# dongzhuoyao/self-guided-diffusion-models

Measured on AMD Instinct MI355X. Metric: cfg_sampled_images_per_sec_64x64_1000step_ddpm, higher is better.
Workload: dtype f32 as 3xf16 split MFMA products, f32 accumulate; 1 GPU; IN64 unet_fast ch128 cluster-k5000 cond_scale=2 bs=40/GPU (UNet batch 80), 1000-step native DDPM; batch_per_gpu=40, unet_batch=80, precision_mode=f16x3, launch=hipGraph-captured step

## Files before the change

include/sgdm_hip.h:

```cpp
#ifndef SGDM_HIP_H
#define SGDM_HIP_H
#include <stdint.h>

#ifdef __cplusplus
extern "C" {
#endif

#define SGD_ABI_VERSION 22
int sgd_abi_version(void);
const char* sgd_build_id(void);

enum { SGD_MODE_FLAT = 0, SGD_MODE_CONV3 = 1 };
enum { SGD_RS_NONE = 0, SGD_RS_AVGPOOL2 = 1, SGD_RS_UP2 = 2,
       SGD_RS_ZEROUP2 = 3  };
enum { SGD_PRO_NONE = 0, SGD_PRO_AFFINE_NC = 1, SGD_PRO_LN_ROW = 2 };
enum { SGD_PREC_F32 = 0, SGD_PREC_F16X3 = 1, SGD_PREC_BF16X3 = 2 };

typedef struct sgd_igemm_args {
    const float* x0;
    const float* x1;
    int32_t c0, c1;
    int32_t mode;
    int32_t n, hi, wi;
    int32_t ho, wo;
    int32_t m;
    int32_t rows_per_n;
    int32_t stride;
    int32_t resample;
    int32_t pro;
    int32_t pro_silu;
    const float* pa;
    const float* pb;
    const float* pc;
    const void* w;
    int32_t cin_p, cout_p;
    const float* bias;
    const float* res;
    int32_t res_mode;
    float* y;
    int32_t cout;
    int32_t y_ld;
    int32_t orows_in, orows_out, orow_off;
    int32_t prec;
    float drop_p;
    uint32_t drop_seed;
    float* stats;
    const float* w_scale_inv;
    void* work;
    int64_t work_bytes;
    int32_t grid_cap;
    int32_t tune;
} sgd_igemm_args;
enum {
    SGD_TUNE_BN128 = 1,
    SGD_TUNE_BN256 = 2,
    SGD_TUNE_FLAT2 = 4,
    SGD_TUNE_DEFER = 8,
    SGD_TUNE_PLAIN_SCHEDULE = 16,
    SGD_TUNE_NO_SMALL = 64,
    SGD_TUNE_LN_PACKED = 32,
    SGD_TUNE_WGRAD_GENERIC_NARROW = 256,
    SGD_TUNE_WGRAD_NO_POOLED_PLANES = 512,
    SGD_TUNE_WGRAD_F32 = 1024,
    SGD_TUNE_WGRAD_NO_WS = 2048,
    SGD_TUNE_WGRAD_NO_PLANES = 4096,
    SGD_TUNE_WGRAD_NO_PIPE = 8192,
    SGD_TUNE_WGRAD_PLANES_ALWAYS = 16384
};
int64_t sgd_igemm_work_bytes(void);
int64_t sgd_igemm_work_status_offset(void);
int sgd_igemm_tail_layout(int32_t total_tiles, int32_t nchunks, int32_t taps, int32_t grid, int32_t* out);


int sgd_igemm(const sgd_igemm_args* args , void* stream);
int sgd_igemm_stats_parts(const sgd_igemm_args* args );

int64_t sgd_packed_weight_bytes(int32_t cout, int32_t cin, int32_t ksize, int32_t prec);
int sgd_pack_weight(const float* w_src, void* w_dst, int32_t cout, int32_t cin, int32_t ksize,
                    int32_t prec, int32_t* cin_p, int32_t* cout_p , void* stream);

int sgd_weight_amax(const float* w, int64_t count, uint32_t* amax_bits, void* stream);
int sgd_pack_weight_scaled(const float* w_src, void* w_dst, int32_t cout, int32_t cin, int32_t ksize, int32_t prec,
                           int32_t transpose ,
                           const uint32_t* amax_bits, float* scale_inv_out, int32_t* cin_p, int32_t* cout_p ,
                           void* stream);

typedef struct sgd_pack_job {
    const float* src;
    void* dst;
    uint32_t* amax_bits;
    float* scale_inv;
    int32_t cout, cin, ksize, transpose;
    int32_t own_amax, reserved0;
} sgd_pack_job;
int sgd_pack_job_blocks(int32_t cout, int32_t cin, int32_t ksize, int32_t prec, int32_t transpose, int32_t* amax_blocks,
                        int32_t* pack_blocks, int32_t* cin_p, int32_t* cout_p );
int sgd_pack_weights_batched(const sgd_pack_job* jobs, int32_t n_jobs, const int32_t* amax_block_job, const int32_t* amax_first,
                             int32_t n_amax_blocks, const int32_t* pack_block_job, const int32_t* pack_first,
                             int32_t n_pack_blocks, int32_t prec, void* stream);

int sgd_linear_splitk(const float* x, int32_t x_ld, const float* w, const float* bias, int32_t m, int32_t n, int32_t k,
                      float* work, int32_t ksplit, float* y, int32_t y_ld, void* stream);
int sgd_linear_splitk_t(const float* x, int32_t x_ld, const float* w, int32_t w_ld, int32_t m, int32_t n, int32_t k,
                        float* work, int32_t ksplit, float* y, int32_t y_ld, void* stream);

int sgd_chan_stats(const float* x, int32_t n, int32_t hw, int32_t c,
                   float* sums , int32_t c_total, int32_t c_off, void* stream);
int sgd_add_rows_nc(float* x, const float* e, int32_t e_ld, int32_t n, int64_t hw, int32_t c, void* stream);
int sgd_stats_reduce(const float* partial, int32_t n, int32_t parts, int32_t c,
                     float* sums , int32_t c_total, int32_t c_off, void* stream);
int sgd_gn_coef_parts(const float* partial0, int32_t parts0, int32_t c0, const float* partial1, int32_t parts1, int32_t c1,
                      float* sums, const float* gamma, const float* beta, const float* film, int32_t film_ld,
                      int32_t n, int32_t groups, int32_t hw, float eps, float* a, float* b, void* stream);
int sgd_gn_coef(const float* sums, const float* gamma, const float* beta,
                const float* film , int32_t film_ld,
                int32_t n, int32_t c, int32_t groups, int32_t hw, float eps,
                float* a, float* b, void* stream);

int sgd_ln_stats(const float* x, int32_t rows, int32_t c, float eps, float* stats , void* stream);
int sgd_ln_apply(const float* x, const float* gamma, const float* beta, const float* res,
                 int32_t rows, int32_t c, float eps, float* out, void* stream);

int sgd_attention(const float* q, int32_t q_ld, int32_t q_hs,
                  const float* k, const float* v, int32_t kv_ld, int32_t kv_hs,
                  int32_t batch, int32_t heads, int32_t tq, int32_t tk, int32_t d, float scale,
                  float* out, int32_t out_ld,
                  float* lse ,
                  void* stream);
int sgd_attention_split(const float* q, int32_t q_ld, int32_t q_hs,
                        const float* k, const float* v, int32_t kv_ld, int32_t kv_hs,
                        int32_t batch, int32_t heads, int32_t tq, int32_t tk, int32_t d, float scale,
                        float* out, int32_t out_ld, float* lse, void* stream);

int sgd_timestep_embedding(const int64_t* t, const float* freqs, int32_t n_src, int32_t n, int32_t dim,
                           float* out, void* stream);
int sgd_cond_select(const void* cond, int32_t is_i64, const uint8_t* mask, const float* null_row,
                    int32_t n_src, int32_t n, int32_t k, float* out, void* stream);
int sgd_pack_input(const float* x, const float* layout, const uint8_t* mask, const float* null_layout,
                   int32_t n_src, int32_t n, int32_t cx, int32_t cl, int32_t h, int32_t w,
                   float* out, void* stream);
int sgd_pack_input_compact(const float* x, const void* layout, int32_t layout_fmt, const uint8_t* mask,
                           const float* null_layout, int32_t n_src, int32_t n, int32_t cx, int32_t cl, int32_t h,
                           int32_t w, float* out, void* stream);
int sgd_labelmap_nhot(const uint8_t* labels, int32_t b, int32_t hw, int32_t k, float* out, void* stream);
int sgd_linear_gather(const int64_t* ids, const uint8_t* mask, const float* w, const float* bias, const float* nullproj,
                      int32_t n_src, int32_t n, int32_t nout, int32_t k, float* out, int32_t ldo, void* stream);
int sgd_linear_sparse_rows(const int64_t* cond, const uint8_t* mask, const float* w, const float* bias, const float* nullproj,
                           int32_t n_src, int32_t n, int32_t nout, int32_t k, float* out, int32_t ldo, void* stream);

int sgd_nhwc_to_nchw(const float* x, int32_t n, int32_t h, int32_t w, int32_t c, float* out, void* stream);
int sgd_fill_null_kv(const float* null_kv, int32_t batch, int32_t rows_per_b, int32_t row, int32_t d,
                     float* kv, void* stream);

int sgd_ddpm_step(const float* x, const float* eps_nhwc, const float* z, int32_t cfg_mode, float w,
                  const float* coef , int32_t clip, int32_t b, int32_t c, int32_t hw,
                  float* x_out, float* x0_out, void* stream);
int sgd_ddim_step(const float* x, const float* eps_nhwc, const float* z, int32_t cfg_mode, float w,
                  const float* coef , float temperature,
                  int32_t clip, int32_t b, int32_t c, int32_t hw, float* x_out, float* x0_out, void* stream);
int sgd_ddpm_step_dev(const float* x, const float* eps_nhwc, const float* z, int32_t cfg_mode, float w,
                      const float* coef_dev, int32_t clip, int32_t b, int32_t c, int32_t hw,
                      float* x_out, float* x0_out, void* stream);
int sgd_ddim_step_dev(const float* x, const float* eps_nhwc, const float* z, int32_t cfg_mode, float w,
                      const float* coef_dev, float temperature, int32_t clip, int32_t b, int32_t c, int32_t hw,
                      float* x_out, float* x0_out, void* stream);
#define SGD_PNDM_RK0 0
#define SGD_PNDM_RK12 1
#define SGD_PNDM_RK3 2
#define SGD_PNDM_PLMS 3
typedef struct sgd_pndm_row {
    float d, c1, c2, reserved;
    int32_t phase, slot1, slot2, slot3;
} sgd_pndm_row;
int sgd_pndm_step(const float* x, const float* eps_nhwc, int32_t cfg_mode, float w, const sgd_pndm_row* row_dev,
                  float* acc, float* base, float* ring, int32_t b, int32_t c, int32_t hw, float* x_out, void* stream);
int sgd_x0_quantile(int32_t kind, const float* x, const float* eps_nhwc, int32_t cfg_mode, float w,
                    const float* coef , int32_t b, int32_t c, int32_t hw, int32_t lo, int32_t hi, float frac,
                    float* s_out , void* stream);
int sgd_ddpm_step_dyn(const float* x, const float* eps_nhwc, const float* z, int32_t cfg_mode, float w,
                      const float* coef , const float* dyn_s, int32_t b, int32_t c, int32_t hw,
                      float* x_out, float* x0_out, void* stream);
int sgd_ddim_step_dyn(const float* x, const float* eps_nhwc, const float* z, int32_t cfg_mode, float w,
                      const float* coef , float temperature, const float* dyn_s, int32_t b, int32_t c,
                      int32_t hw, float* x_out, float* x0_out, void* stream);

int sgd_token_pool(const float* cond, int32_t n, int32_t tokens, int32_t c, int32_t cls, float* out, void* stream);

int sgd_geglu(const float* in, int64_t rows, int32_t inner, float* out, void* stream);

int sgd_to_uint8(const float* x, int64_t count, uint8_t* out, void* stream);
int sgd_cfg_combine(const float* eps_nhwc, int32_t cfg_mode, float w, int32_t b, int32_t c, int32_t hw,
                    float* out_nchw, void* stream);


int sgd_pack_weight_dgrad(const float* w_src, void* w_dst, int32_t cout_fwd, int32_t cin_fwd, int32_t ksize,
                          int32_t prec, int32_t* cin_p, int32_t* cout_p , void* stream);

int sgd_wgrad(const sgd_igemm_args* fwd , const float* gy, int32_t gy_ld, int32_t cout,
              float* slabs, int32_t ksplit, float* bias_slabs, void* stream);
int64_t sgd_wgrad_scratch_bytes(const sgd_igemm_args* fwd , int32_t cout);
int sgd_wgrad_bias_rows(const sgd_igemm_args* fwd , int32_t cout, int32_t gy_ld, int32_t ksplit,
                            int64_t scratch_bytes);
int sgd_wgrad_scratch(const sgd_igemm_args* fwd , const float* gy, int32_t gy_ld, int32_t cout,
                      float* slabs, int32_t ksplit, float* bias_slabs, void* scratch, int64_t scratch_bytes, void* stream);
int sgd_colsum_fold(const float* partial, int32_t chunks, int32_t c, float* out, int32_t accumulate, float scale,
                    void* stream);
int sgd_wgrad_reduce(const float* slabs, int32_t ksplit, int32_t taps, int32_t cout, int32_t cin,
                     float* dw, int32_t accumulate, float scale, void* stream);
int sgd_wgrad_reduce_bias(const float* slabs, int32_t ksplit, int32_t taps, int32_t cout, int32_t cin, float* dw,
                          int32_t accumulate, float scale, const float* bias_slabs, int32_t bias_rows, float* dbias,
                          void* stream);
int sgd_colsum_pair(const float* g1, const float* g2, int32_t rows, int32_t c, int32_t ld, float* out1, float* out2,
                    int32_t accumulate, float scale, void* stream);
int sgd_colsum(const float* g, int32_t rows, int32_t c, int32_t ld, float* out, int32_t accumulate, float scale,
               float* work, int32_t work_chunks, void* stream);

int sgd_gn_bwd_reduce(const float* x, int32_t n, int32_t h, int32_t w, int32_t c, int32_t c_total, int32_t c_off,
                      const float* a, const float* b, int32_t silu,
                      const float* gu, int32_t gu_ld, int32_t gu_mode, float drop_p, uint32_t drop_seed,
                      float* S, void* stream);
int sgd_gn_bwd_coef(const float* S, int32_t s_chunks, const float* sums, const float* gamma, const float* beta,
                    const float* film, int32_t film_ld, int32_t n, int32_t c, int32_t groups, int32_t hw, float eps,
                    float* A, float* B, float* Cc, float* dgamma_nc, float* dbeta_nc ,
                    float* dfilm, void* stream);
int sgd_gn_bwd_coef_fold(const float* S, int32_t s_chunks, const float* sums, const float* gamma, const float* beta, const float* film,
                         int32_t film_ld, int32_t n, int32_t c, int32_t groups, int32_t hw, float eps, float* A, float* B,
                         float* Cc, float* dfilm, float* dgamma, float* dbeta, int32_t accumulate, float scale, void* stream);
int sgd_gn_bwd_rows_chunks(int32_t n, int32_t h, int32_t w, int32_t c);
int sgd_gn_bwd_reduce_rows(const float* x, int32_t n, int32_t h, int32_t w, int32_t c, int32_t c_total, int32_t c_off,
                           const float* a, const float* b, int32_t silu, const float* gu, int32_t gu_ld, float drop_p,
                           uint32_t drop_seed, int32_t chunks, float* P, void* stream);
int sgd_gn_bwd_apply(const float* x, int32_t n, int32_t h, int32_t w, int32_t c, int32_t c_total, int32_t c_off,
                     const float* a, const float* b, int32_t silu,
                     const float* gu, int32_t gu_ld, int32_t gu_mode, float drop_p, uint32_t drop_seed,
                     const float* A, const float* B, const float* Cc,
                     const float* gres, int32_t gres_ld, int32_t gres_mode,
                     float* dst, int32_t dst_ld, int32_t dst_off, int32_t accumulate, void* stream);
int sgd_silu_bwd(const float* x, const float* g, int64_t count, float* gx, void* stream);

// ... 67 lines not shown
```

self-guided-diffusion-models_amd/csrc/igemm.hip:

```cpp
#include <type_traits>
#include <utility>

#include "igemm_shared.h"
#include "prologue.h"

namespace {

#ifdef SGDM_PROBE
#define DBG(bit) 0
#define SYNC() do { if (g.stamp) { const unsigned long long t0_ = __builtin_amdgcn_s_memtime(); __syncthreads(); \
                    const unsigned long long t1_ = __builtin_amdgcn_s_memtime(); \
                    if (g.trace && blockIdx.x < 16 && pr_nbar < 512 && (threadIdx.x & 63) == 0) { \
                        unsigned long long* tp_ = g.trace + (((size_t)blockIdx.x * (NTHREADS / 64) + (threadIdx.x >> 6)) * 512 + pr_nbar) * 2; \
                        tp_[0] = t0_; tp_[1] = t1_; } \
                    pr_bar += t1_ - t0_; ++pr_nbar; } else if (!DBG(64)) { __syncthreads(); } } while (0)
#define PROBE_BEGIN() unsigned long long pr_bar = 0, pr_nbar = 0, pr_epi = 0; const unsigned long long pr_t0 = __builtin_amdgcn_s_memtime()
#define PROBE_END(role) do { if (g.stamp && (threadIdx.x & 63) == 0) { \
        unsigned long long* sp_ = g.stamp + ((size_t)blockIdx.x * (NTHREADS / 64) + (threadIdx.x >> 6)) * 4; \
        sp_[0] = __builtin_amdgcn_s_memtime() - pr_t0; sp_[1] = pr_bar; sp_[2] = pr_nbar; sp_[3] = pr_epi; } } while (0)
#define PROBE_EPI(expr) do { if (g.stamp) { const unsigned long long t0_ = __builtin_amdgcn_s_memtime(); expr; pr_epi += __builtin_amdgcn_s_memtime() - t0_; } else { expr; } } while (0)
#else
#define DBG(bit) 0
#define SYNC() __syncthreads()
#define PROBE_BEGIN()
// ... 39 lines not shown

template <int PREC, int NT> struct Frag {
    typedef typename Split<PREC>::T T;
    typedef T T8 __attribute__((ext_vector_type(8)));
    static constexpr int NKS = KC / 16;
    static constexpr int NREADS = 2;
    static constexpr int NWLOADS = 2 * NT;
    static constexpr int NMMA = 3 * NT;
    struct AU {
        T8 h, l;
        __device__ __forceinline__ void load(const float* rowp, int ks, int lh) {
            const int goff = (ks * 2 + lh) * 8;
            h = *reinterpret_cast<const T8*>(rowp + goff);
            l = *reinterpret_cast<const T8*>(rowp + goff + 4);
        }
    };
    struct B {
        T8 h[NT], l[NT];
        __device__ __forceinline__ void load(const char* p, int ks) {
#pragma unroll
            for (int nt = 0; nt < NT; ++nt) {
                h[nt] = *reinterpret_cast<const T8*>(p + nt * WUNIT + ks * 2048);
                l[nt] = *reinterpret_cast<const T8*>(p + nt * WUNIT + ks * 2048 + 1024);
            }
        }
    };
    static __device__ __forceinline__ void mma(f32x16 (&acc)[NT], const AU& a, const B& b) {
#pragma unroll
        for (int nt = 0; nt < NT; ++nt) {
            if constexpr (PREC == SGD_PREC_F16X3) {
                acc[nt] = __builtin_amdgcn_mfma_f32_32x32x16_f16(b.h[nt], a.l, acc[nt], 0, 0, 0);
                acc[nt] = __builtin_amdgcn_mfma_f32_32x32x16_f16(b.l[nt], a.h, acc[nt], 0, 0, 0);
                acc[nt] = __builtin_amdgcn_mfma_f32_32x32x16_f16(b.h[nt], a.h, acc[nt], 0, 0, 0);
            } else {
                acc[nt] = __builtin_amdgcn_mfma_f32_32x32x16_bf16(b.h[nt], a.l, acc[nt], 0, 0, 0);
                acc[nt] = __builtin_amdgcn_mfma_f32_32x32x16_bf16(b.l[nt], a.h, acc[nt], 0, 0, 0);
                acc[nt] = __builtin_amdgcn_mfma_f32_32x32x16_bf16(b.h[nt], a.h, acc[nt], 0, 0, 0);
            }
        }
    }
};
template <int PREC, int NCB> struct Frag16 {
    typedef typename Split<PREC>::T T;
    typedef T T8 __attribute__((ext_vector_type(8)));
    static constexpr int NREADS = 2;
    static constexpr int NWLOADS = 2 * NCB;
    static constexpr int NMMA = 3 * NCB;
    struct AU {
        T8 h, l;
        __device__ __forceinline__ void load(const float* rowp, int kg) {
            h = *reinterpret_cast<const T8*>(rowp + kg * 8);
            l = *reinterpret_cast<const T8*>(rowp + kg * 8 + 4);
        }
    };
    struct B {
        T8 h[NCB], l[NCB];
        __device__ __forceinline__ void load(const char* p) {
#pragma unroll
            for (int cb = 0; cb < NCB; ++cb) {
                h[cb] = *reinterpret_cast<const T8*>(p + (cb >> 1) * WUNIT + (cb & 1) * 256);
                l[cb] = *reinterpret_cast<const T8*>(p + (cb >> 1) * WUNIT + (cb & 1) * 256 + 1024);
            }
        }
    };
    static __device__ __forceinline__ f32x4 mma1(f32x4 acc, const AU& a, const B& b) {
        if constexpr (PREC == SGD_PREC_F16X3) {
            acc = __builtin_amdgcn_mfma_f32_16x16x32_f16(b.h[0], a.l, acc, 0, 0, 0);
            acc = __builtin_amdgcn_mfma_f32_16x16x32_f16(b.l[0], a.h, acc, 0, 0, 0);
            acc = __builtin_amdgcn_mfma_f32_16x16x32_f16(b.h[0], a.h, acc, 0, 0, 0);
        } else {
            acc = __builtin_amdgcn_mfma_f32_16x16x32_bf16(b.h[0], a.l, acc, 0, 0, 0);
            acc = __builtin_amdgcn_mfma_f32_16x16x32_bf16(b.l[0], a.h, acc, 0, 0, 0);
            acc = __builtin_amdgcn_mfma_f32_16x16x32_bf16(b.h[0], a.h, acc, 0, 0, 0);
        }
        return acc;
    }
    static __device__ __forceinline__ void mma(f32x4 (&acc)[NCB], const AU& a, const B& b) {
#pragma unroll
        for (int cb = 0; cb < NCB; ++cb) {
            if constexpr (PREC == SGD_PREC_F16X3) {
                acc[cb] = __builtin_amdgcn_mfma_f32_16x16x32_f16(b.h[cb], a.l, acc[cb], 0, 0, 0);
                acc[cb] = __builtin_amdgcn_mfma_f32_16x16x32_f16(b.l[cb], a.h, acc[cb], 0, 0, 0);
                acc[cb] = __builtin_amdgcn_mfma_f32_16x16x32_f16(b.h[cb], a.h, acc[cb], 0, 0, 0);
            } else {
                acc[cb] = __builtin_amdgcn_mfma_f32_16x16x32_bf16(b.h[cb], a.l, acc[cb], 0, 0, 0);
                acc[cb] = __builtin_amdgcn_mfma_f32_16x16x32_bf16(b.l[cb], a.h, acc[cb], 0, 0, 0);
                acc[cb] = __builtin_amdgcn_mfma_f32_16x16x32_bf16(b.h[cb], a.h, acc[cb], 0, 0, 0);
            }
        }
    }
};
template <int NCB> struct Frag16<SGD_PREC_F32, NCB> {
    static constexpr int NREADS = 1, NWLOADS = 1, NMMA = 1;
    struct AU { __device__ __forceinline__ void load(const float*, int) {} };
    struct B { __device__ __forceinline__ void load(const char*) {} };
    static __device__ __forceinline__ void mma(f32x4 (&)[NCB], const AU&, const B&) {}
    static __device__ __forceinline__ f32x4 mma1(f32x4 acc, const AU&, const B&) { return acc; }
};
template <int NT> struct Frag<SGD_PREC_F32, NT> {
    static constexpr int NKS = KC / 8;
    static constexpr int NREADS = 1;
    static constexpr int NWLOADS = NT;
    static constexpr int NMMA = 4 * NT;
    struct AU {
        f32x4 v;
        __device__ __forceinline__ void load(const float* rowp, int ks, int lh) {
            v = *reinterpret_cast<const f32x4*>(rowp + ks * 8 + lh * 4);
        }
    };
    struct B {
        f32x4 v[NT];
        __device__ __forceinline__ void load(const char* p, int ks) {
#pragma unroll
            for (int nt = 0; nt < NT; ++nt) v[nt] = *reinterpret_cast<const f32x4*>(p + nt * WUNIT + ks * 1024);
        }
    };
    static __device__ __forceinline__ void mma(f32x16 (&acc)[NT], const AU& a, const B& b) {
#pragma unroll
        for (int j = 0; j < 4; ++j)
#pragma unroll
            for (int nt = 0; nt < NT; ++nt)
                acc[nt] = __builtin_amdgcn_mfma_f32_32x32x2f32(b.v[nt][j], a.v[j], acc[nt], 0, 0, 0);
    }
};

template <int CTRL, int ROWMASK> __device__ __forceinline__ float dpp_add(float v) {
    return v + __builtin_bit_cast(float, __builtin_amdgcn_update_dpp(0, __builtin_bit_cast(int, v), CTRL, ROWMASK, 0xF, true));
}
__device__ __forceinline__ float half_wave_sum_hi(float v) {
    v = dpp_add<0xB1, 0xF>(v);
    v = dpp_add<0x4E, 0xF>(v);
    v = dpp_add<0x141, 0xF>(v);
    v = dpp_add<0x140, 0xF>(v);
    return dpp_add<0x142, 0xA>(v);
}

template <class F, int... I> __device__ __forceinline__ void static_for_impl(F&& f, std::integer_sequence<int, I...>) {
    (f(std::integral_constant<int, I>()), ...);
}
template <int N, class F> __device__ __forceinline__ void static_for(F&& f) {
    static_for_impl(f, std::make_integer_sequence<int, N>());
}

__device__ __forceinline__ float row16_sum(float v) {
    v = dpp_add<0xB1, 0xF>(v);
    v = dpp_add<0x4E, 0xF>(v);
    v = dpp_add<0x141, 0xF>(v);
    return dpp_add<0x140, 0xF>(v);
}

struct Tile {
    int n0c;
    int img0, ty0, tx0;
    long m0;
};

__device__ __forceinline__ Tile tile_at(const Geo& g, int lin, int bn, int tw, int th) {
    Tile t;
    const int mtile = lin / g.nt, ntile = lin - mtile * g.nt;
    t.n0c = ntile * bn;
    const int per_img = g.tiles_x * g.tiles_y;
    const int it = mtile / per_img, rem = mtile - it * per_img;
    t.img0 = it * g.nb;
    t.ty0 = (rem / g.tiles_x) * th;
    t.tx0 = (rem % g.tiles_x) * tw;
    t.m0 = (long)mtile * BM;
    return t;
}


template <int BN, int PREC, bool VEC, int TAPS, bool DEFER>
struct IgemmBlock {
    static constexpr bool CONV = TAPS == 9;
    static constexpr int FG = CONV ? 1 : TAPS;
    static constexpr int KCC = KC * FG;
    static constexpr int NA = 3;
    static constexpr int WM = (BN >= 128) ? 128 : 32;
    static constexpr int WN = (BN >= 128) ? BN / 4 : 32;
    static constexpr int MT = WM / 32, NT = WN / 32;
    static constexpr int WAVES_N = BN / WN;
    typedef Frag<PREC, NT> FragT;
    static constexpr bool M16 = PREC != SGD_PREC_F32 && BN <= 128 && !DEFER;
    static constexpr int RB = M16 ? WM / 16 : MT, RBH = M16 ? 16 : 32;
    static constexpr int CBN = M16 ? WN / 16 : NT, CBW = M16 ? 16 : 32;
    static constexpr int QPB = M16 ? 1 : 4;
    typedef Frag16<PREC, CBN> Frag16T;
    typedef std::conditional_t<M16, f32x4, f32x16> AccV;
    static constexpr int NKS = FragT::NKS;

    static constexpr int STG_LD = BN + 4;
    static_assert(!DEFER || (BN == 128 && TAPS == 9 && VEC && !M16), "loader-side epilogue: 3x3, 128-column tiles");

    const sgd_igemm_args& a;
    const Geo& g;
    float* As;
    int2* pixtab;
    float* bias_s;
    float* stg;
    int a_floats;
    bool bias_lds;
    int tid, lane, wave;
    int total, xchunk, nloc, xcd, loc, xbeg, xend, cin, nchunks, xtiles, nfull, xrem, split;
    int ntiles, rem_lin, rem_part, last_c0, last_c1;
    int Q, S, s, TW, TH, M;

    __device__ __forceinline__ int lin_of(int k) const { return (rem_lin >= 0 && k == ntiles - 1) ? rem_lin : xbeg + loc + k * nloc; }
    __device__ __forceinline__ int cbeg(int k) const { return k == ntiles - 1 ? last_c0 : 0; }
    __device__ __forceinline__ int cend(int k) const { return k == ntiles - 1 ? last_c1 : nchunks; }

    __device__ __forceinline__ bool init(float* smem) {
        a_floats = g.pix * LDA;
        As = smem;
        pixtab = reinterpret_cast<int2*>(smem + (size_t)NA * a_floats);
        bias_s = smem + (size_t)NA * a_floats + (size_t)g.pix * 8;
        bias_lds = a.cout_p <= BIAS_LDS_MAX;
        stg = bias_s + a.cout_p;

        tid = threadIdx.x; lane = tid & 63;
        wave = __builtin_amdgcn_readfirstlane(tid >> 6);

        total = g.mt * g.nt;
        xchunk = (total + 7) >> 3;
        nloc = gridDim.x >> 3;
        xcd = blockIdx.x & 7; loc = blockIdx.x >> 3;
        xbeg = xcd * xchunk; xend = (xbeg + xchunk < total) ? xbeg + xchunk : total;
        cin = a.c0 + a.c1;
        nchunks = (cin + KCC - 1) / KCC;
        xtiles = xend > xbeg ? xend - xbeg : 0;
        nfull = xtiles / nloc; xrem = xtiles - nfull * nloc;
        split = (a.work && !ABL(2048)) ? tail_split(xrem, nloc, nchunks, TAPS) : 0;
        rem_lin = -1; rem_part = 0; last_c0 = 0; last_c1 = nchunks;
        if (!split) {
            ntiles = loc < xtiles ? (xtiles - loc + nloc - 1) / nloc : 0;
        } else {
            ntiles = nfull;
            if (loc < xrem * split) {
                rem_lin = xbeg + nfull * nloc + loc / split;
                rem_part = loc % split;
                last_c0 = rem_part * nchunks / split;
                last_c1 = (rem_part + 1) * nchunks / split;
                ++ntiles;
            }
        }
        if (ntiles == 0) return false;

        Q = (ntiles - 1) * nchunks + (last_c1 - last_c0);
        S = Q * TAPS;
        s = CONV ? a.stride : 1;
        TW = 1 << g.tw_l2; TH = 1 << g.th_l2;
        M = CONV ? a.n * a.ho * a.wo : a.m;

        return true;
    }

    __device__ __forceinline__ void build_pixtab(int k, int t0, int nthr) const {
        if (k >= ntiles) return;
        const Tile T = tile_at(g, lin_of(k), BN, TW, TH);
        int2* tab = pixtab + (size_t)(k & 3) * g.pix;
        for (int pix = t0; pix < g.pix; pix += nthr) {
            int2 e;
            e.x = -1;
            e.y = 0;
            if (CONV) {
                int hx = pix % g.hw, t = pix / g.hw;
                int hy = t % g.hh, nb = t / g.hh;
                int n = T.img0 + nb, y = T.ty0 * s - 1 + hy, x = T.tx0 * s - 1 + hx;
                if (n < a.n && y >= 0 && y < g.hc && x >= 0 && x < g.wc) {
                    if (a.resample == SGD_RS_UP2) e.x = (n * a.hi + (y >> 1)) * a.wi + (x >> 1);
                    else if (a.resample == SGD_RS_AVGPOOL2) e.x = (n * a.hi + 2 * y) * a.wi + 2 * x;
                    else if (a.resample == SGD_RS_ZEROUP2) e.x = ((y | x) & 1) ? -1 : (n * a.hi + (y >> 1)) * a.wi + (x >> 1);
                    else e.x = (n * a.hi + y) * a.wi + x;
                    e.y = n;
                }
            } else {
                long row = T.m0 + pix;
                if (row < M) {
                    e.x = (int)row;
                    e.y = (a.pro == SGD_PRO_AFFINE_NC) ? (int)(row / a.rows_per_n) : 0;
                }
            }
            tab[pix] = e;
        }
    }

    static constexpr size_t SLAB = (size_t)RB * CBN * QPB * NCOMP * 16;
    static __device__ __forceinline__ f32x4 accq(const AccV (&acc)[RB][CBN], int mt, int nt, int q) {
        f32x4 v;
#pragma unroll
        for (int j = 0; j < 4; ++j) v[j] = acc[mt][nt][(M16 ? 0 : q * 4) + j];
        return v;
    }
    __device__ __forceinline__ int pixel_of_lane(int ln) const {
    const int l5 = ln & 31;
        int px = l5;
        if (CONV && g.tw_l2 == 4 && s == 1) {
            if (l5 < 4) px = l5;
            else if (l5 < 12) px = l5 + 4;
            else if (l5 < 16) px = l5 - 8;
            else if (l5 < 20) px = l5;
            else if (l5 < 28) px = l5 + 2;
            else px = l5 < 30 ? l5 - 8 : l5;
        }
        if constexpr (M16) {
            const int i16 = ln & 15;
            px = i16 < 4 ? 2 * i16 : (i16 < 12 ? 2 * (i16 - 4) + 1 : 2 * i16 - 16);
        }
        return px;
    }
    template <int RES, bool PART>
    __device__ __forceinline__ void epilogue(const AccV (&acc)[RB][CBN], const Tile& T, int wm, int wn, int lane_e, int cb, float wsk,
                                             const char* part_base, int nparts) const;
    __device__ __forceinline__ void loader_role();
    __device__ __forceinline__ void compute_role();
};

template <int BN, int PREC, bool VEC, int TAPS, bool DEFER>
__device__ __forceinline__ void IgemmBlock<BN, PREC, VEC, TAPS, DEFER>::loader_role() {
    PROBE_BEGIN();
    __builtin_amdgcn_s_setprio(2);
    const int dlt = tid - NCOMP;
    const int dcq = (dlt >> 6) * 8 + (dlt & 7), drg = (dlt & 63) >> 3;
    int dk = 0, dqs = 0, dnck = cend(0) - cbeg(0);
    Tile dT = tile_at(g, lin_of(0), BN, TW, TH);
    int dcol = 0;
    unsigned dsoff = 0xFFFFFFFFu;
    f32x4 dres[8], ds1 = {0.f, 0.f, 0.f, 0.f}, ds2 = ds1;
    unsigned dyoff[8];
    int di0 = 0;
#pragma unroll
    for (int j = 0; j < 8; ++j) { dres[j] = f32x4{0.f, 0.f, 0.f, 0.f}; dyoff[j] = 0xFFFFFFFFu; }
    const float dwsi = (DEFER && a.w_scale_inv) ? *a.w_scale_inv : 1.f;
    const long drows = (long)a.n * a.ho * a.wo;
    const __amdgpu_buffer_rsrc_t dy_rs = __builtin_amdgcn_make_buffer_rsrc(a.y, 0, (int)(drows * a.y_ld * 4), 0x00020000);
    const __amdgpu_buffer_rsrc_t dr_rs = __builtin_amdgcn_make_buffer_rsrc(a.res ? const_cast<float*>(a.res) : a.y, 0,
                                                                           a.res ? (int)(drows * a.cout * 4) : 0, 0x00020000);
    const __amdgpu_buffer_rsrc_t ds_rs = __builtin_amdgcn_make_buffer_rsrc(a.stats ? a.stats : a.y, 0,
                                             a.stats ? (int)((long)a.n * g.sparts * 2 * a.cout * 4) : 0, 0x00020000);
    const int dnq = !DEFER ? 0 : (nchunks - 1 >= 8 && cend(ntiles - 1) - cbeg(ntiles - 1) - 1 >= 8) ? 2
                               : (nchunks - 1 >= 4 && cend(ntiles - 1) - cbeg(ntiles - 1) - 1 >= 4) ? 4 : 8;
    auto with_nq = [&](auto&& f) __attribute__((always_inline)) {
        if (dnq == 2) f(std::integral_constant<int, 2>());
        else if (dnq == 4) f(std::integral_constant<int, 4>());
        else if (dnq == 8) f(std::integral_constant<int, 8>());
        else f(std::integral_constant<int, 0>());
    };
    auto drain = [&](int q, auto nqc) __attribute__((always_inline)) {
        constexpr int NQ = decltype(nqc)::value;
        if constexpr (DEFER && NQ > 0) {
            if (q >= dqs + dnck) {
                dqs += dnck;
                ++dk;
                dnck = cend(dk) - cbeg(dk);
            }
            const int j = q - dqs, nsl = dnck - 1;
            const f32x4 bq = *reinterpret_cast<const f32x4*>(bias_s + (dcol < a.cout_p ? dcol : 0));
#pragma unroll
            for (int jj = 0; jj < NQ; ++jj) {
                const int frow = drg + 8 * (di0 + jj < 16 ? di0 + jj : 15);
                f32x4 v = *reinterpret_cast<const f32x4*>(stg + (size_t)frow * STG_LD + dcq * 4);
                v = v * dwsi + bq + dres[jj];
                __builtin_amdgcn_raw_buffer_store_b128(__builtin_bit_cast(u32x4_t, v), dy_rs, dyoff[jj], 0, 0);
                if (dyoff[jj] != 0xFFFFFFFFu) {
                    ds1 += v;
                    ds2 += v * v;
                }
            }
            const bool last = dk > 0 && j == nsl;
            f32x4 t1 = ds1, t2 = ds2;
            if (last) {
#pragma unroll
                for (int o = 8; o < 64; o <<= 1)
#pragma unroll
                    for (int e = 0; e < 4; ++e) {
                        t1[e] += __shfl_xor(t1[e], o, 64);
                        t2[e] += __shfl_xor(t2[e], o, 64);
                    }
                ds1 = ds2 = f32x4{0.f, 0.f, 0.f, 0.f};
            }
            const unsigned so = (last && drg == 0) ? dsoff : 0xFFFFFFFFu;
            __builtin_amdgcn_raw_buffer_store_b128(__builtin_bit_cast(u32x4_t, t1), ds_rs, so, 0, 0);
            __builtin_amdgcn_raw_buffer_store_b128(__builtin_bit_cast(u32x4_t, t2), ds_rs,
                                                   so == 0xFFFFFFFFu ? so : so + (unsigned)a.cout * 4u, 0, 0);
            const bool req = dk > 0 && j < nsl;
            int i0 = 0, i1 = 0;
            if (req) { i0 = (16 * j) / nsl; i1 = (16 * (j + 1)) / nsl; }
            di0 = i0;
            if (dk > 0 && j == 0) {
                dT = tile_at(g, lin_of(dk - 1), BN, TW, TH);
                const Tile& T = dT;
                dcol = T.n0c + dcq * 4;
                const int part = (T.ty0 >> g.th_l2) * g.tiles_x + (T.tx0 >> g.tw_l2);
                dsoff = (a.stats && dcol < a.cout) ? (unsigned)((((long)T.img0 * g.sparts + part) * 2 * a.cout + dcol) * 4) : 0xFFFFFFFFu;
            }
            const Tile& T = dT;
#pragma unroll
            for (int jj = 0; jj < NQ; ++jj) {
                const int i = i0 + jj;
                const int row = drg + 8 * (i < 16 ? i : 15);
                const int tx = row & (TW - 1), ty = (row >> g.tw_l2) & (TH - 1), nb = row >> (g.tw_l2 + g.th_l2);
                const int n = T.img0 + nb;
                const bool ok = i < i1 && nb < g.nb && n < a.n && dcol < a.cout;
                const int orow = (n * a.ho + T.ty0 + ty) * a.wo + T.tx0 + tx;
                dyoff[jj] = ok ? (unsigned)(((long)orow * a.y_ld + dcol) * 4) : 0xFFFFFFFFu;
                const unsigned ro = ok ? (unsigned)(((long)orow * a.cout + dcol) * 4) : 0xFFFFFFFFu;
                dres[jj] = __builtin_bit_cast(f32x4, __builtin_amdgcn_raw_buffer_load_b128(dr_rs, ro, 0, 0));
            }
        }
        (void)q;
    };
    if constexpr (CONV) {
        const bool uni_rt = VEC && g.nb == 1 && a.pro == SGD_PRO_AFFINE_NC;
        const bool drop_rt = a.drop_p > 0.f;
        const bool lean2 = g.fast_a && VEC && ((uni_rt && a.pro_silu) || (a.pro == SGD_PRO_NONE && !a.pro_silu))
                           && (!drop_rt || (uni_rt && a.pro_silu && a.resample != SGD_RS_AVGPOOL2))
                           && cin % KC == 0 && (a.c1 == 0 || a.c0 % KC == 0) && !DBG(3);
        if (lean2) {
            constexpr int LT = A_THREADS;
            constexpr int AJ = (FAST_PIX * 8 + LT - 1) / LT;
            const int lt = tid - NCOMP;
            const int c4 = lt & 7;
            const int items = g.pix * 8;
            auto go = [&](auto unic, auto poolc, auto dropc) __attribute__((always_inline)) {
                constexpr bool uni = decltype(unic)::value;
                constexpr bool DROP = decltype(dropc)::value;
                constexpr bool LATE = false;
                constexpr int NS = decltype(poolc)::value ? 4 : 1;
                constexpr int T0 = LATE ? 5 : 1;
                typedef std::integral_constant<int, 0> R0;
                typedef std::integral_constant<int, 1> R1;
                typedef std::integral_constant<int, 2> R2;
                int pixj[AJ], rows2[AJ];
                bool live[AJ];
#pragma unroll
                for (int j = 0; j < AJ; ++j) {
                    const int idx = lt + j * LT;
                    live[j] = idx < items;
                    pixj[j] = (live[j] ? idx : items - 1) >> 3;
                }
                unsigned valid1 = 0, valid2 = 0;
                auto load_rows = [&](int k) __attribute__((always_inline)) {
                    const int2* tab = pixtab + (size_t)(k & 3) * g.pix;
                    valid2 = 0;
#pragma unroll
                    for (int j = 0; j < AJ; ++j) {
                        const int ex = tab[pixj[j]].x;
                        rows2[j] = ex < 0 ? 0 : ex;
                        if (ex >= 0) valid2 |= 1u << j;
                    }
                };
                struct S { int k, chunk, img0; const float* src; int stride; const float* ka; const float* kb; };
                auto fill = [&](S& c) __attribute__((always_inline)) {
                    const int ch = c.chunk * KC;
                    if (ch < a.c0) { c.src = a.x0 + ch; c.stride = a.c0; }
                    else { c.src = a.x1 + (ch - a.c0); c.stride = a.c1; }
                    const long ko = (long)c.img0 * cin + ch;
                    c.ka = uni ? a.pa + ko : a.x0;
                    c.kb = uni ? a.pb + ko : a.x0;
                };
                auto advance = [&](S c) __attribute__((always_inline)) {
                    if (++c.chunk == cend(c.k)) {
                        if (c.k + 1 < ntiles) {
                            ++c.k; c.chunk = cbeg(c.k);
                            c.img0 = tile_at(g, lin_of(c.k), BN, TW, TH).img0;
                        }
                        else c.chunk = cend(c.k) - 1;
                    }
                    fill(c);
                    return c;
                };
                f32x4 araw[AJ][NS];
                Coef kq;
                auto transform = [&](f32x4 v, bool ok) __attribute__((always_inline)) {
                    if (ABL(256)) return v;
                    if constexpr (uni) {
                        const float den = ok ? 1.0f : __builtin_inff();
                        v = v * kq.p + kq.q;
#pragma unroll
                        for (int e = 0; e < 4; ++e) v[e] = v[e] * __builtin_amdgcn_rcpf(den + __expf(-v[e]));
                    } else {
                        if (!ok) v = f32x4{0.f, 0.f, 0.f, 0.f};
                    }
                    return v;
                };
                auto issue_item = [&](const S& c, int j) __attribute__((always_inline)) {
                    const float* p0 = c.src + (long)rows2[j] * c.stride + c4 * 4;
                    if (ABL(512)) { KEEP_LIVE(p0); return; }
                    araw[j][0] = ld4(p0);
                    if constexpr (NS == 4) {
                        araw[j][1] = ld4(p0 + c.stride);
                        araw[j][2] = ld4(p0 + (long)a.wi * c.stride);
                        araw[j][3] = ld4(p0 + (long)(a.wi + 1) * c.stride);
                    }
                };
                auto issue_coef = [&](const S& c) __attribute__((always_inline)) {
                    if constexpr (uni) { kq.p = ld4(c.ka + c4 * 4); kq.q = ld4(c.kb + c4 * 4); }
                };
                S s2;
                auto finish = [&](int slot, int j) __attribute__((always_inline)) {
                    const bool ok = (valid1 >> j) & 1u;
                    f32x4 v = transform(araw[j][0], ok);
                    if constexpr (NS == 4)
                        v = 0.25f * (v + transform(araw[j][1], ok) + transform(araw[j][2], ok) + transform(araw[j][3], ok));
                    if constexpr (DROP)
                        v = sgd_drop4(v, a.drop_p, a.drop_seed, (long)rows2[j] * cin + s2.chunk * KC + c4 * 4);
                    if (!ABL(1024)) lds_store_act<PREC>(As + (size_t)(slot % NA) * a_floats + (size_t)pixj[j] * LDA, c4, v);
                    else KEEP_LIVE(v);
                };
                auto stage = [&](int slot) __attribute__((always_inline)) {
                    valid1 = valid2;
                    auto finish_all = [&]() {
#pragma unroll
                        for (int j = 0; j < AJ; ++j) finish(slot, j);
                    };
                    PROBE_EPI(finish_all());
                    const int kprev = s2.k;
                    s2 = advance(s2);
                    if (s2.k != kprev) load_rows(s2.k);
                    issue_coef(s2);
#pragma unroll
                    for (int j = 0; j < AJ; ++j) issue_item(s2, j);
                };
                s2.k = 0; s2.chunk = cbeg(0); s2.img0 = tile_at(g, lin_of(0), BN, TW, TH).img0; fill(s2);
                load_rows(0);
                issue_coef(s2);
#pragma unroll
                for (int j = 0; j < AJ; ++j) issue_item(s2, j);
                stage(0);
                stage(1);
                SYNC();
                auto periods = [&](auto nqc) __attribute__((always_inline)) {
                    for (int q = 0; q < Q; ++q) {
                        drain(q, nqc);
                        stage((q + 2) % NA);
                        if (q + 4 < Q && (q + 4) % nchunks == 0) build_pixtab((q + 4) / nchunks, lt, LT);
                        SYNC();
                    }
                };
                if constexpr (NS == 4) periods(std::integral_constant<int, 0>());
                else with_nq(periods);
            };
            if (uni_rt) {
                if (a.resample == SGD_RS_AVGPOOL2) go(std::true_type(), std::true_type(), std::false_type());
                else if (drop_rt) go(std::true_type(), std::false_type(), std::true_type());
                else go(std::true_type(), std::false_type(), std::false_type());
            } else {
                if (a.resample == SGD_RS_AVGPOOL2) go(std::false_type(), std::true_type(), std::false_type());
                else go(std::false_type(), std::false_type(), std::false_type());
            }
            PROBE_END(1);
            return;
        }
    } else {
        const bool tile_uni_rt = a.pro == SGD_PRO_AFFINE_NC && a.rows_per_n % BM == 0;
        const bool ln_rt = a.pro == SGD_PRO_LN_ROW;
        const bool leanf = VEC && (a.pro == SGD_PRO_NONE || tile_uni_rt || ln_rt) && a.drop_p == 0.f && cin % KC == 0
                           && (a.c1 == 0 || a.c0 % KC == 0) && !DBG(3);
        auto flat_loader = [&](auto modec, auto siluc) {
            constexpr int MODE = decltype(modec)::value;
            constexpr bool SILU = decltype(siluc)::value;
            constexpr bool tile_uni = MODE == 1, ln = MODE == 2;
            constexpr int AI = BM * 8 / A_THREADS;
            constexpr int AROWS = A_THREADS / 8;
            const int lt = tid - NCOMP;
            const int c4 = lt & 7;
            const int arow = lt >> 3;
            typedef std::integral_constant<int, 0> R0;
            typedef std::integral_constant<int, 1> R1;
            typedef std::integral_constant<int, 2> R2;
            f32x4 araw[NB_RING][AI];
            Coef kq[NB_RING];
            float2 rst[NB_RING][AI];
            struct Cur { int k, chunk; int m0; const float* ka; const float* kb; };
            auto open_tile = [&](Cur& c) {
                const Tile T = tile_at(g, lin_of(c.k), BN, TW, TH);
                c.m0 = (int)T.m0;
                const long ko = tile_uni ? (long)(c.m0 / a.rows_per_n) * cin : 0;
                c.ka = tile_uni ? a.pa + ko + c4 * 4 : (ln ? a.pb + c4 * 4 : a.x0);
                c.kb = tile_uni ? a.pb + ko + c4 * 4 : ((ln && a.pc) ? a.pc + c4 * 4 : a.x0);
            };
            auto advance = [&](Cur& c) {
                if (++c.chunk == cend(c.k) * FG) {
                    if (c.k + 1 < ntiles) { ++c.k; c.chunk = cbeg(c.k) * FG; open_tile(c); }
                    else c.chunk = cend(c.k) * FG - 1;
                }
            };
            Cur ci, cf;
            ci.k = 0; ci.chunk = cbeg(0) * FG; open_tile(ci);
            cf = ci;
            auto issue = [&](auto rc) {
                constexpr int R = decltype(rc)::value;
                const int ch = ci.chunk * KC;
                const float* src;
                int stride;
                if (ch < a.c0) { src = a.x0 + ch; stride = a.c0; }
                else { src = a.x1 + (ch - a.c0); stride = a.c1; }
                if constexpr (MODE != 0) {
                    kq[R].p = ld4(ci.ka + ch);
                    kq[R].q = ld4(ci.kb + ((tile_uni || a.pc) ? ch : 0));
                }
#pragma unroll
                for (int j = 0; j < AI; ++j) {
                    int row = ci.m0 + arow + j * AROWS;
                    row = row < M ? row : M - 1;
                    araw[R][j] = ld4(src + (long)row * stride + c4 * 4);
                    if constexpr (ln) rst[R][j] = *reinterpret_cast<const float2*>(a.pa + (long)row * 2);
                }
                advance(ci);
            };
            auto finish = [&](int slot, auto rc, int sub = 0) {
                constexpr int R = decltype(rc)::value;
#pragma unroll
                for (int j = 0; j < AI; ++j) {
                    f32x4 v = araw[R][j];
                    if constexpr (tile_uni) v = v * kq[R].p + kq[R].q;
                    if constexpr (ln) {
                        v = (v - rst[R][j].x) * rst[R][j].y * kq[R].p;
                        if (a.pc) v += kq[R].q;
                    }
                    if constexpr (SILU) {
#pragma unroll
                        for (int e = 0; e < 4; ++e) v[e] = sgd_silu(v[e]);
                    }
                    if (cf.m0 + arow + j * AROWS >= M) v = f32x4{0.f, 0.f, 0.f, 0.f};
                    lds_store_act<PREC>(As + (size_t)slot * a_floats + (size_t)(sub * BM + arow + j * AROWS) * LDA, c4, v);
                }
                advance(cf);
            };
            if constexpr (FG == 1) {
                issue(R0());
                issue(R1());
                finish(0, R0());
                finish(1, R1());
                issue(R2());
                issue(R0());
                issue(R1());
                SYNC();
                auto body = [&](int slot, auto rc) {
                    finish(slot, rc);
                    issue(rc);
                    SYNC();
                };
                int step = 0;
                for (; step + 3 <= S; step += 3) {
                    body(2, R2());
                    body(0, R0());
                    body(1, R1());
                }
                if (step < S) {
                    body(2, R2());
                    if (step + 1 < S) body(0, R0());
                }
            } else {
                static_assert(FG <= 2, "two planes per chunk");
                issue(R0());
                issue(R1());
                issue(R2());
                finish(0, R0(), 0); issue(R0());
                finish(0, R1(), 1); issue(R1());
                finish(1, R2(), 0); issue(R2());
                finish(1, R0(), 1); issue(R0());
                SYNC();
                auto period = [&](int slot, auto ra, auto rb) {
                    finish(slot, ra, 0); issue(ra);
                    finish(slot, rb, 1); issue(rb);
                    SYNC();
                };
                int q = 0;
                for (; q + 3 <= Q; q += 3) {
                    period(2, R1(), R2());
                    period(0, R0(), R1());
                    period(1, R2(), R0());
                }
                if (q < Q) {
                    period(2, R1(), R2());
                    if (q + 1 < Q) period(0, R0(), R1());
                }
            }
        };
        if (FG > 1 && !leanf) __builtin_trap();
        if (leanf) {
            typedef std::integral_constant<int, 0> M0;
            typedef std::integral_constant<int, 1> M1;
            typedef std::integral_constant<int, 2> M2;
            if (tile_uni_rt) { if (a.pro_silu) flat_loader(M1(), std::true_type()); else flat_loader(M1(), std::false_type()); }
            else if (ln_rt) { if (a.pro_silu) flat_loader(M2(), std::true_type()); else flat_loader(M2(), std::false_type()); }
            else { if (a.pro_silu) flat_loader(M0(), std::true_type()); else flat_loader(M0(), std::false_type()); }
            PROBE_END(1);
            return;
        }
    }
    const int lt = tid - NCOMP;
    const int c4 = lt & 7;
    const int items = g.pix * 8;
    struct TabRef { const int2* tab; long m0; };
    auto tabref = [&](int k) {
        TabRef t;
        t.tab = pixtab + (size_t)(k & 3) * g.pix;
        t.m0 = CONV ? 0 : tile_at(g, lin_of(k), BN, TW, TH).m0;
        return t;
    };
    auto entry = [&](const TabRef& t, int pix) -> int2 {
        if (CONV) return t.tab[pix];
        int2 e;
        const long row = t.m0 + pix;
        e.x = row < M ? (int)row : -1;
        e.y = (a.pro == SGD_PRO_AFFINE_NC) ? (int)(row / a.rows_per_n) : 0;
        return e;
    };
    auto item_sync = [&](float* abuf, const TabRef& tab, int idx, int kc0) {
        const int pix = idx >> 3;
        const int c = kc0 + c4 * 4;
        const int2 e = entry(tab, pix);
        f32x4 v = {0.f, 0.f, 0.f, 0.f};
        if (e.x >= 0 && c < cin) {
            if (CONV && a.resample == SGD_RS_AVGPOOL2) {
#pragma unroll
                for (int dy = 0; dy < 2; ++dy)
#pragma unroll
                    for (int dx = 0; dx < 2; ++dx) {
                        long r = (long)e.x + dy * a.wi + dx;
                        v += apply_pro(a, load_raw<VEC>(a, r, c), load_coef<VEC>(a, e.y, r, c), c, r);
                    }
                v = v * 0.25f;
            } else {
                v = apply_pro(a, load_raw<VEC>(a, e.x, c), load_coef<VEC>(a, e.y, e.x, c), c, e.x);
            }
        }
        lds_store_act<PREC>(abuf + (size_t)pix * LDA, c4, v);
    };
    auto stage_A_sync = [&](int slot, int q) __attribute__((always_inline)) {
        q = q < Q ? q : Q - 1;
        const int k = q / nchunks, chunk = q - k * nchunks + cbeg(k);
        float* abuf = As + (size_t)(slot % NA) * a_floats;
        const TabRef tab = tabref(k);
        for (int idx = lt; idx < items; idx += A_THREADS) item_sync(abuf, tab, idx, chunk * KC);
    };
    auto finish_item = [&](int slot, const TabRef& tab, int chunk, int idx, f32x4 raw, bool kuse, const Coef& kuni) __attribute__((always_inline)) {
        float* abuf = As + (size_t)(slot % NA) * a_floats;
        const int c = chunk * KC + c4 * 4;
        if (idx < items) {
            const int pix = idx >> 3;
            const int2 e = entry(tab, pix);
            f32x4 v = {0.f, 0.f, 0.f, 0.f};
            if (c < cin && e.x >= 0) v = apply_pro(a, raw, kuse ? kuni : load_coef<VEC>(a, e.y, e.x, c), c, e.x);
            lds_store_act<PREC>(abuf + (size_t)pix * LDA, c4, v);
        }
    };
    auto raw_item = [&](const TabRef& tab, int idx, int c) -> f32x4 {
        const int ii = idx < items ? idx : items - 1;
        const int2 e = entry(tab, ii >> 3);
        return load_raw<VEC>(a, e.x >= 0 ? e.x : 0, c < cin ? c : 0);
    };

    if (CONV) {
        constexpr int AJ = (FAST_PIX * 8 + A_THREADS - 1) / A_THREADS;
        stage_A_sync(0, 0);
        if (DBG(1)) {
            for (int q = 0; q <= Q; ++q) SYNC();
        } else if (g.fast_a && a.resample != SGD_RS_AVGPOOL2) {
            const bool uni = VEC && g.nb == 1 && a.pro == SGD_PRO_AFFINE_NC;
            const bool kshared = uni || a.pro == SGD_PRO_NONE;
            f32x4 araw[AJ];
            Coef kq;
            struct Ctx { const int2* tab; int c; int chunk; long ko; };
            auto ctx_of = [&](int q) {
                q = q < Q ? q : Q - 1;
                Ctx cx;
                const int k = q / nchunks;
                cx.chunk = q - k * nchunks + cbeg(k);
                cx.tab = pixtab + (size_t)(k & 3) * g.pix;
                cx.c = cx.chunk * KC + c4 * 4;
                cx.ko = (long)tile_at(g, lin_of(k), BN, TW, TH).img0 * cin + (cx.c < cin ? cx.c : 0);
                return cx;
            };
            Ctx cx = ctx_of(1);
            auto request = [&]() __attribute__((always_inline)) {
                TabRef tr;
                tr.tab = cx.tab;
                tr.m0 = 0;
                kq.p = ld4(uni ? a.pa + cx.ko : a.x0);
                kq.q = ld4(uni ? a.pb + cx.ko : a.x0);
#pragma unroll
                for (int j = 0; j < AJ; ++j) araw[j] = raw_item(tr, lt + j * A_THREADS, cx.c);
            };
            auto stage = [&](int slot, int qnext) __attribute__((always_inline)) {
                TabRef tr;
                tr.tab = cx.tab;
                tr.m0 = 0;
#pragma unroll
                for (int j = 0; j < AJ; ++j)
                    finish_item(slot, tr, cx.chunk, lt + j * A_THREADS, araw[j], kshared, kq);
                cx = ctx_of(qnext);
                request();
            };
            request();
            stage(1, 2);
            SYNC();
            with_nq([&](auto nqc) __attribute__((always_inline)) {
                for (int q = 0; q < Q; ++q) {
                    drain(q, nqc);
                    stage(q + 2, q + 3);
                    if (q + 4 < Q && (q + 4) % nchunks == 0) build_pixtab((q + 4) / nchunks, lt, A_THREADS);
                    SYNC();
                }
            });
        } else {
            stage_A_sync(1, 1);
            SYNC();
            with_nq([&](auto nqc) __attribute__((always_inline)) {
                for (int q = 0; q < Q; ++q) {
                    drain(q, nqc);
                    stage_A_sync(q + 2, q + 2);
                    if (q + 4 < Q && (q + 4) % nchunks == 0) build_pixtab((q + 4) / nchunks, lt, A_THREADS);
                    SYNC();
                }
            });
        }
        PROBE_END(1);
        return;
    } else {
        constexpr int AJ = (BM * 8 + A_THREADS - 1) / A_THREADS;
        f32x4 araw[NB_RING][AJ];
        stage_A_sync(0, 0);
        if (Q > 1) stage_A_sync(1, 1);
        auto issue = [&](int q, auto rc) {
            constexpr int R = decltype(rc)::value;
            q = q < Q ? q : Q - 1;
            const int k = q / nchunks, chunk = q - k * nchunks + cbeg(k);
            const TabRef tab = tabref(k);
            const int c = chunk * KC + c4 * 4;
#pragma unroll
            for (int j = 0; j < AJ; ++j) araw[R][j] = raw_item(tab, lt + j * A_THREADS, c);
        };
        auto finish = [&](int slot, auto rc) {
            constexpr int R = decltype(rc)::value;
            const int q = slot < Q ? slot : Q - 1;
            const int k = q / nchunks, chunk = q - k * nchunks + cbeg(k);
            const TabRef tab = tabref(k);
            Coef knone;
            knone.p = f32x4{0.f, 0.f, 0.f, 0.f};
            knone.q = knone.p;
#pragma unroll
            for (int j = 0; j < AJ; ++j)
                finish_item(slot, tab, chunk, lt + j * A_THREADS, araw[R][j], a.pro == SGD_PRO_NONE, knone);
        };
        typedef std::integral_constant<int, 0> R0;
        typedef std::integral_constant<int, 1> R1;
        typedef std::integral_constant<int, 2> R2;
        issue(2, R2());
        issue(3, R0());
        issue(4, R1());
        SYNC();
        auto body = [&](int step, auto rc) {
            finish(step + 2, rc);
            issue(step + 5, rc);
            SYNC();
        };
        int step = 0;
        for (; step + 3 <= S; step += 3) {
            body(step, R2());
            body(step + 1, R0());
            body(step + 2, R1());
        }
        if (step < S) {
            body(step, R2());
            if (step + 1 < S) body(step + 1, R0());
        }
        PROBE_END(1);
        return;
    }
}

template <int BN, int PREC, bool VEC, int TAPS, bool DEFER>
template <int RES, bool PART>
__device__ __forceinline__ void IgemmBlock<BN, PREC, VEC, TAPS, DEFER>::epilogue(const AccV (&acc)[RB][CBN], const Tile& T, int wm, int wn,
                                                                                 int lane_e, int cb, float wsk, const char* part_base,
                                                                                 int nparts) const {
    const int li = lane & 31;
    bool okm[RB];
    int orw[RB], rrw[RB];
    const int plie = pixel_of_lane(lane_e);
#pragma unroll
    for (int mt = 0; mt < RB; ++mt) {
        const int row = wm * WM + mt * RBH + plie;
        int orow, n = 0, oy = 0, ox = 0;
        if (CONV) {
            const int tx = row & (TW - 1), ty = (row >> g.tw_l2) & (TH - 1), nb = row >> (g.tw_l2 + g.th_l2);
            n = T.img0 + nb; oy = T.ty0 + ty; ox = T.tx0 + tx;
            okm[mt] = nb < g.nb && n < a.n;
            orow = (n * a.ho + oy) * a.wo + ox;
        } else {
            orow = (int)T.m0 + row;
            okm[mt] = orow < M;
        }
        if (!okm[mt]) orow = 0;
        int rrow = orow;
        if (RES == 2) rrow = (n * a.ho * 2 + 2 * oy) * (a.wo * 2) + 2 * ox;
        if (RES == 3) rrow = (n * (a.ho >> 1) + (oy >> 1)) * (a.wo >> 1) + (ox >> 1);
        if (!okm[mt]) rrow = 0;
        if (!CONV && a.orows_in > 0)
            orow = (int)((unsigned)orow / (unsigned)a.orows_in) * a.orows_out + a.orow_off
                   + (int)((unsigned)orow % (unsigned)a.orows_in);
        orw[mt] = orow;
        rrw[mt] = rrow;
    }
    const bool vec = ((a.cout | a.y_ld) & 3) == 0;
    if (vec) {
        float* sp = nullptr;
        if (a.stats) {
            int n_img, part;
            if (CONV) {
                n_img = T.img0;
                part = ((T.ty0 >> g.th_l2) * g.tiles_x + (T.tx0 >> g.tw_l2)) * (BM / WM) + wm;
            } else {
                n_img = (int)(T.m0 / a.rows_per_n);
                part = (int)((T.m0 % a.rows_per_n) / BM) * (BM / WM) + wm;
            }
            sp = a.stats + ((long)n_img * g.sparts + part) * 2 * a.cout;
        }
        {
            constexpr int CS = CBN * QPB;
            constexpr int QB = M16 ? ((RES == 2 || PART) ? 1 : (CBN > 2 ? 2 : CBN)) : ((RES == 2 || NT > 1) ? 1 : 2);
            constexpr int RBB = M16 ? (RES == 2 || RB < 4 ? 2 : ((PART || CBN > 2) ? 4 : RB)) : RB;
            static_assert(RB % RBB == 0 && CS % QB == 0, "batches must tile the wave's rows and columns");
#pragma unroll
            for (int q0 = 0; q0 < CS; q0 += QB) {
            f32x4 s1[QB], s2[QB];
#pragma unroll
            for (int i = 0; i < QB; ++i) s1[i] = s2[i] = f32x4{0.f, 0.f, 0.f, 0.f};
#pragma unroll
            for (int mb0 = 0; mb0 < RB; mb0 += RBB) {
#pragma unroll
            for (int mt = mb0; mt < mb0 + RBB; ++mt) asm volatile("" : "+v"(orw[mt]), "+v"(rrw[mt]));
            f32x4 rv[QB][RBB];
            f32x4 pv[QB][RBB];
            if constexpr (PART) {
#pragma unroll
                for (int cs = q0; cs < q0 + QB; ++cs)
#pragma unroll
                    for (int mt = mb0; mt < mb0 + RBB; ++mt) {
                        const char* pp = part_base + (size_t)((mt * CS + cs) * NCOMP) * 16;
                        f32x4 sum = *reinterpret_cast<const f32x4*>(pp);
                        for (int pi = 1; pi < nparts; ++pi) sum += *reinterpret_cast<const f32x4*>(pp + pi * SLAB);
                        pv[cs - q0][mt - mb0] = sum;
                    }
            }
#pragma unroll
            for (int cs = q0; cs < q0 + QB; ++cs) {
                const int c = cb + (cs / QPB) * CBW + (cs % QPB) * 8;
                const int cl = c < a.cout ? c : 0;
                f32x4 bv = {0.f, 0.f, 0.f, 0.f};
                if (bias_lds) bv = *reinterpret_cast<const f32x4*>(bias_s + cl);
                else if (a.bias && !ABL(2)) bv = ld4(a.bias + cl);
#pragma unroll
                for (int mt = mb0; mt < mb0 + RBB; ++mt) {
                    f32x4& r = rv[cs - q0][mt - mb0];
                    r = bv;
                    if ((RES == 1 || RES == 3) && !ABL(2)) r += ld4(a.res + (long)rrw[mt] * a.cout + cl);
                    if (RES == 2 && !ABL(2)) {
                        const long rw = (long)a.wo * 2 * a.cout;
                        const float* rp = a.res + (long)rrw[mt] * a.cout;
                        r += 0.25f * (ld4(rp + cl) + ld4(rp + a.cout + cl) + ld4(rp + rw + cl) + ld4(rp + rw + a.cout + cl));
                    }
                }
            }
#pragma unroll
            for (int cs = q0; cs < q0 + QB; ++cs) {
                const int c = cb + (cs / QPB) * CBW + (cs % QPB) * 8;
                if (c >= a.cout) continue;
#pragma unroll
                for (int mt = mb0; mt < mb0 + RBB; ++mt) {
                    f32x4 v = accq(acc, mt, cs / QPB, cs % QPB);
                    if constexpr (PART) v += pv[cs - q0][mt - mb0];
                    v = v * wsk + rv[cs - q0][mt - mb0];
                    if (okm[mt]) {
                        if (!(DBG(8)) && !ABL(1)) *reinterpret_cast<f32x4*>(a.y + (long)orw[mt] * a.y_ld + c) = v;
                        else KEEP_LIVE(v);
                        s1[cs - q0] += v;
                        s2[cs - q0] += v * v;
                    }
                }
            }
            }
            if (sp && !DBG(256) && !ABL(4)) {
#pragma unroll
                for (int cs = q0; cs < q0 + QB; ++cs) {
                    const int c = cb + (cs / QPB) * CBW + (cs % QPB) * 8;
                    if (c >= a.cout) continue;
                    f32x4 t1 = s1[cs - q0], t2 = s2[cs - q0];
#pragma unroll
                    for (int j = 0; j < 4; ++j) {
                        t1[j] = M16 ? row16_sum(t1[j]) : half_wave_sum_hi(t1[j]);
                        t2[j] = M16 ? row16_sum(t2[j]) : half_wave_sum_hi(t2[j]);
                    }
                    if (M16 ? (lane & 15) == 0 : li == 16) {
                        *reinterpret_cast<f32x4*>(sp + c) = t1;
                        *reinterpret_cast<f32x4*>(sp + a.cout + c) = t2;
                    }
                }
            }
            }
        }
    } else {
#pragma unroll
        for (int mt = 0; mt < RB; ++mt) {
            if (!okm[mt]) continue;
            float* yp = a.y + (long)orw[mt] * a.y_ld;
            const float* rp = RES ? a.res + (long)rrw[mt] * a.cout : nullptr;
#pragma unroll
            for (int nt = 0; nt < CBN; ++nt)
#pragma unroll
                for (int gq = 0; gq < QPB; ++gq)
#pragma unroll
                    for (int j = 0; j < 4; ++j) {
                        const int c = cb + nt * CBW + gq * 8 + j;
                        if (c >= a.cout) continue;
                        float x = acc[mt][nt][(M16 ? 0 : gq * 4) + j];
                        if constexpr (PART) {
                            const float* pp = reinterpret_cast<const float*>(part_base + (size_t)(((mt * CBN + nt) * QPB + gq) * NCOMP) * 16) + j;
                            for (int pi = 0; pi < nparts; ++pi) x += pp[pi * (SLAB / 4)];
                        }
                        x = x * wsk + (bias_lds ? bias_s[c] : (a.bias ? a.bias[c] : 0.f));
                        if (RES == 1 || RES == 3) x += rp[c];
                        if (RES == 2) {
                            const long rw = (long)a.wo * 2 * a.cout;
                            x += 0.25f * (rp[c] + rp[a.cout + c] + rp[rw + c] + rp[rw + a.cout + c]);
                        }
                        yp[c] = x;
                    }
        }
    }
}

template <int BN, int PREC, bool VEC, int TAPS, bool DEFER>
__device__ __forceinline__ void IgemmBlock<BN, PREC, VEC, TAPS, DEFER>::compute_role() {
    PROBE_BEGIN();
    const int li = lane & 31, lh = lane >> 5;
    const int wm = wave / WAVES_N, wn = wave % WAVES_N;

    const int pli = pixel_of_lane(lane);
    int aoff[RB];
#pragma unroll
    for (int mt = 0; mt < RB; ++mt) {
        int r = wm * WM + mt * RBH + pli;
        int p;
        if (CONV) {
            int tx = r & (TW - 1), ty = (r >> g.tw_l2) & (TH - 1), nb = r >> (g.tw_l2 + g.th_l2);
            p = (nb * g.hh + ty * s) * g.hw + tx * s;
        } else {
            p = r;
        }
        aoff[mt] = p * LDA;
    }
    const size_t wstep = (size_t)(a.cout_p >> 5) * WUNIT;
    auto wtile_of = [&](int k) __attribute__((always_inline)) {
        int l;
        asm volatile("v_mbcnt_lo_u32_b32 %0, -1, 0\n\tv_mbcnt_hi_u32_b32 %0, -1, %0" : "=v"(l));
        const int loff = M16 ? (l >> 5) * 2048 + (((l >> 4) & 1) * 32 + (l & 15)) * 16 : l * 16;
        return reinterpret_cast<const char*>(a.w) + (size_t)(wn * NT + (tile_at(g, lin_of(k), BN, TW, TH).n0c >> 5)) * WUNIT + loff;
    };

    AccV acc[RB][CBN];
    const float wsi = __builtin_bit_cast(float, __builtin_amdgcn_readfirstlane(
        __builtin_bit_cast(int, a.w_scale_inv ? *a.w_scale_inv : 1.f)));

    constexpr int STAGES = M16 ? RB * CBN : NKS * MT;
    constexpr int RING = M16 ? RB : (STAGES >= 4 ? 4 : 2);
    constexpr int DEPTH = RING - 1;
    static_assert(STAGES % RING == 0, "ring position must be a compile-time constant inside a K step");
    std::conditional_t<M16, typename Frag16<PREC, 1>::AU, typename FragT::AU> ring[RING];
    typename FragT::B fb[NKS];
    typename Frag16<PREC, 1>::B fb16[CBN];
    const int rowstep = g.hw * LDA;

    auto tap_off = [&](int tap) { return CONV ? (tap / 3) * rowstep + (tap % 3) * LDA : tap * (BM * LDA); };
    auto do_step = [&](const float* acur, const float* anext, auto tapc, auto parc, const char* wnext) {
        constexpr int tap = decltype(tapc)::value;
        constexpr int PAR = decltype(parc)::value;
        constexpr bool seam = tap + 1 == TAPS;
        static_for<STAGES>([&](auto stc) {
            constexpr int st = decltype(stc)::value;
            constexpr int ks = M16 ? 0 : st / MT, mt = M16 ? st % RB : st % MT;
            constexpr int pst = (st + DEPTH) % STAGES;
            constexpr bool wrap = st + DEPTH >= STAGES;
            const float* pbase = (wrap && seam) ? anext : acur;
            constexpr int ptap = wrap ? (seam ? 0 : tap + 1) : tap;
            if constexpr (M16) {
                constexpr int cbi = st / RB;
                const float* nbase = seam ? anext : acur;
                constexpr int ntap = seam ? 0 : tap + 1;
                if (!ABL(16)) acc[mt][cbi] = Frag16<PREC, 1>::mma1(acc[mt][cbi], ring[mt], fb16[cbi]);
                if (cbi == CBN - 1 && !ABL(64)) ring[mt].load(nbase + tap_off(ntap) + aoff[mt], lane >> 4);
                if (mt == RB - 1 && !ABL(32)) fb16[cbi].load(wnext + (cbi >> 1) * WUNIT + (cbi & 1) * 256);
                (void)pbase; (void)ptap; (void)pst; (void)wrap;
            } else {
                if (!ABL(64)) ring[(st + DEPTH) % RING].load(pbase + tap_off(ptap) + aoff[pst % MT], pst / MT, lh);
                if (!ABL(16)) FragT::mma(acc[mt], ring[st % RING], fb[ks]);
                if (mt == MT - 1 && !ABL(32)) fb[ks].load(wnext, ks);
            }
            {
                constexpr int NM = M16 ? 3 : FragT::NMMA;
                constexpr int NR = M16 ? (st / RB == CBN - 1 ? 2 : 0) : FragT::NREADS;
                constexpr int P1 = NR < NM ? NR : NM;
                constexpr int nw = M16 ? (st % RB == RB - 1 ? 2 : 0) : ((mt == MT - 1) ? FragT::NWLOADS : 0);
                constexpr int P2 = nw < NM - P1 ? nw : NM - P1;
#pragma unroll
                for (int i = 0; i < P1; ++i) {
                    __builtin_amdgcn_sched_group_barrier(0x008, 1, 0);
                    __builtin_amdgcn_sched_group_barrier(0x100, 1, 0);
                }
#pragma unroll
                for (int i = 0; i < P2; ++i) {
                    __builtin_amdgcn_sched_group_barrier(0x008, 1, 0);
                    __builtin_amdgcn_sched_group_barrier(0x020, 1, 0);
                }
                if constexpr (NM - P1 - P2 > 0) __builtin_amdgcn_sched_group_barrier(0x008, NM - P1 - P2, 0);
            }
            __builtin_amdgcn_sched_barrier(0);
        });
        if constexpr (seam) SYNC();
    };

    auto wstart_of = [&](int k) { return wtile_of(k) + (size_t)cbeg(k) * TAPS * wstep; };
    const char* wp = wstart_of(0);
    if constexpr (M16) {
#pragma unroll
        for (int cb = 0; cb < CBN; ++cb) fb16[cb].load(wp + (cb >> 1) * WUNIT + (cb & 1) * 256);
    } else {
#pragma unroll
        for (int ks = 0; ks < NKS; ++ks) fb[ks].load(wp, ks);
    }
    SYNC();
#pragma unroll
    for (int st = 0; st < (M16 ? RB : DEPTH); ++st) {
        if constexpr (M16) ring[st].load(As + aoff[st % RB], lane >> 4);
        else ring[st].load(As + aoff[st % MT], st / MT, lh);
    }
    int aslot = 0;
    for (int k = 0; k < ntiles; ++k) {
#pragma unroll
        for (int i = 0; i < RB; ++i)
#pragma unroll
            for (int j = 0; j < CBN; ++j)
#pragma unroll
                for (int r = 0; r < (M16 ? 4 : 16); ++r) acc[i][j][r] = 0.f;
        const char* const wseam = k + 1 < ntiles ? wstart_of(k + 1) : nullptr;
        const int c_end = cend(k);
        for (int chunk = cbeg(k); chunk < c_end; ++chunk) {
            const int naslot = aslot + 1 == NA ? 0 : aslot + 1;
            const float* acur = As + (size_t)aslot * a_floats;
            const float* anext = As + (size_t)naslot * a_floats;
            const char* const wlast = chunk + 1 == c_end ? (wseam ? wseam : wp + (TAPS - 1) * wstep) : nullptr;
            static_for<TAPS>([&](auto tapc) {
                constexpr int tap = decltype(tapc)::value;
                const char* wnext = wp + wstep;
                if (tap + 1 == TAPS && wlast) wnext = wlast;
                do_step(acur, anext, tapc, std::integral_constant<int, tap & 1>(), wnext);
                wp = wnext;
            });
            aslot = naslot;
        }
        if constexpr (DEFER) {
            if (k + 1 < ntiles) {
                int plie = pli;
                asm volatile("" : "+v"(plie));
#pragma unroll
                for (int mt = 0; mt < RB; ++mt) {
                    float* sp = stg + (size_t)(wm * WM + mt * RBH + plie) * STG_LD + wn * WN + 4 * lh;
#pragma unroll
                    for (int q = 0; q < QPB; ++q) {
                        f32x4 v;
#pragma unroll
                        for (int j = 0; j < 4; ++j) v[j] = acc[mt][0][q * 4 + j];
                        *reinterpret_cast<f32x4*>(sp + q * 8) = v;
                    }
                }
                continue;
            }
        }

        const char* part_base = nullptr;
        int nparts = 0;
        float wsk = wsi;
        int* part_cnt = nullptr;
        if (rem_lin >= 0 && k == ntiles - 1) {
            const int gi = tail_counter(xcd, loc, nloc, split);
            int* const cnt = reinterpret_cast<int*>(a.work) + gi * 2;
            char* const slab0 = reinterpret_cast<char*>(a.work) + WORK_HEAD + (size_t)tail_slab(xcd, loc, nloc, split) * SLAB;
            if (rem_part + 1 < split) {
                __amdgpu_buffer_rsrc_t rs = __builtin_amdgcn_make_buffer_rsrc(slab0 + (size_t)rem_part * SLAB, 0, (int)SLAB, 0x00020000);
#pragma unroll
                for (int mt = 0; mt < RB; ++mt)
#pragma unroll
                    for (int nt = 0; nt < CBN; ++nt)
#pragma unroll
                        for (int q = 0; q < QPB; ++q)
                            __builtin_amdgcn_raw_buffer_store_b128(__builtin_bit_cast(u32x4_t, accq(acc, mt, nt, q)), rs,
                                                                   (((mt * CBN + nt) * QPB + q) * NCOMP + tid) * 16, 0, 16 );
                asm volatile("s_waitcnt vmcnt(0)" ::: "memory");
                if (lane == 0) __hip_atomic_fetch_add(cnt, 1, __ATOMIC_RELAXED, __HIP_MEMORY_SCOPE_AGENT);
                break;
            }
            int late = 0;
            if (lane == 0) {
                const int need = (split - 1) * (NCOMP / 64);
                int polls = 0;
                while (__hip_atomic_load(cnt, __ATOMIC_RELAXED, __HIP_MEMORY_SCOPE_AGENT) < need) {
                    __builtin_amdgcn_s_sleep(16);
                    if (++polls >= FINISH_POLL_MAX) { late = 1; break; }
                }
                int* const status = reinterpret_cast<int*>(a.work) + WORK_STATUS_INT;
                if (late) __hip_atomic_store(status, 1, __ATOMIC_RELAXED, __HIP_MEMORY_SCOPE_AGENT);
                else if (__hip_atomic_load(status, __ATOMIC_RELAXED, __HIP_MEMORY_SCOPE_AGENT) != 0) late = 2;
            }
            if (__builtin_amdgcn_readfirstlane(late)) wsk = __builtin_nanf("");
            __builtin_amdgcn_fence(__ATOMIC_ACQUIRE, "agent");
            asm volatile("s_waitcnt vmcnt(0)" ::: "memory");
            {
                int lane_p;
                asm volatile("v_mbcnt_lo_u32_b32 %0, -1, 0\n\tv_mbcnt_hi_u32_b32 %0, -1, %0" : "=v"(lane_p));
                part_base = slab0 + (size_t)(wave * 64 + lane_p) * 16;
            }
            nparts = split - 1;
            part_cnt = cnt;
        }

        const Tile T = tile_at(g, lin_of(k), BN, TW, TH);
        int lane_e;
        asm volatile("v_mbcnt_lo_u32_b32 %0, -1, 0\n\tv_mbcnt_hi_u32_b32 %0, -1, %0" : "=v"(lane_e));
        const int cb = T.n0c + wn * WN + 4 * (M16 ? lane_e >> 4 : lane_e >> 5);
        auto keep_acc = [&]() {
#pragma unroll
            for (int i = 0; i < RB; ++i)
#pragma unroll
                for (int j = 0; j < CBN; ++j) KEEP_LIVE(acc[i][j]);
        };
        auto run_epilogue = [&](auto partc) {
            constexpr bool PARTV = decltype(partc)::value;
            if (DBG(16) || ABL(8)) keep_acc();
            else if (!a.res) epilogue<0, PARTV>(acc, T, wm, wn, lane_e, cb, wsk, part_base, nparts);
            else if (a.res_mode == SGD_RS_NONE) epilogue<1, PARTV>(acc, T, wm, wn, lane_e, cb, wsk, part_base, nparts);
            else if (NT > 1) __builtin_trap();
            else if (a.res_mode == SGD_RS_AVGPOOL2) epilogue<2, PARTV>(acc, T, wm, wn, lane_e, cb, wsk, part_base, nparts);
            else epilogue<3, PARTV>(acc, T, wm, wn, lane_e, cb, wsk, part_base, nparts);
        };
        if (nparts) {
            run_epilogue(std::true_type());
            if (lane == 0) {
                if (__hip_atomic_fetch_add(part_cnt + 1, 1, __ATOMIC_RELAXED, __HIP_MEMORY_SCOPE_AGENT) == NCOMP / 64 - 1) {
                    __hip_atomic_store(part_cnt, 0, __ATOMIC_RELAXED, __HIP_MEMORY_SCOPE_AGENT);
                    __hip_atomic_store(part_cnt + 1, 0, __ATOMIC_RELAXED, __HIP_MEMORY_SCOPE_AGENT);
                }
            }
        } else {
            PROBE_EPI(run_epilogue(std::false_type()));
        }
        if constexpr (NT > 1 || M16) {
            if (k + 1 < ntiles) {
                const float* a0 = As + (size_t)aslot * a_floats;
                if constexpr (M16) {
#pragma unroll
                    for (int st = 0; st < RB; ++st) ring[st].load(a0 + aoff[st % RB], lane >> 4);
                } else {
#pragma unroll
                    for (int ks = 0; ks < NKS; ++ks) fb[ks].load(wp, ks);
#pragma unroll
                    for (int st = 0; st < DEPTH; ++st) ring[st].load(a0 + aoff[st % MT], st / MT, lh);
                }
            }
        }
    }
    PROBE_END(0);
}

template <int BN, int PREC, bool VEC, int TAPS, bool DEFER = false>
__global__ __launch_bounds__(NTHREADS) void igemm_kernel(const KArgs ka) {
    extern __shared__ __attribute__((aligned(16))) float smem[];
    IgemmBlock<BN, PREC, VEC, TAPS, DEFER> blk{ka.a, ka.g};
    if (!blk.init(smem)) return;
    blk.build_pixtab(0, blk.tid, NTHREADS);
    blk.build_pixtab(1, blk.tid, NTHREADS);
    blk.build_pixtab(2, blk.tid, NTHREADS);
    blk.build_pixtab(3, blk.tid, NTHREADS);
    if (blk.bias_lds)
        for (int i = blk.tid; i < ka.a.cout_p; i += NTHREADS) blk.bias_s[i] = (ka.a.bias && i < ka.a.cout && !ABL(2)) ? ka.a.bias[i] : 0.f;
    __syncthreads();
    if (blk.tid >= NCOMP) blk.loader_role();
    else blk.compute_role();
}

template <int BN, int PREC, bool VEC, int TAPS, bool DEFER = false>
int launch1(const KArgs& ka, size_t smem, hipStream_t st) {
    static bool attr = false;
    if (!attr) {
        (void)hipFuncSetAttribute((const void*)igemm_kernel<BN, PREC, VEC, TAPS, DEFER>,
                                  hipFuncAttributeMaxDynamicSharedMemorySize, 160 * 1024);
        attr = true;
    }
    const int total = ka.g.mt * ka.g.nt;
    int full = device_cus();
    if (ka.a.grid_cap > 0 && ka.a.grid_cap < full) full = ka.a.grid_cap >= 8 ? (ka.a.grid_cap & ~7) : 8;
    int grid = ((total + 7) / 8) * 8;
    if (grid > full) grid = full;
    if (ka.a.work && total >= 8) grid = full;
    hipLaunchKernelGGL((igemm_kernel<BN, PREC, VEC, TAPS, DEFER>), dim3(grid), dim3(NTHREADS), smem, st, ka);
    const int rc = sgd_check_launch();
    if (rc != SGD_OK && ka.a.work) (void)hipMemsetAsync(ka.a.work, 0, WORK_HEAD, st);
    return rc;
}

template <int BN, int PREC>
int launch(const KArgs& ka, int vec, int taps, size_t smem, hipStream_t st) {
    const bool conv = taps == 9;
#ifdef SGDM_IGEMM_NOPK
    if (conv) return SGD_ERR_ARG;
    if constexpr (BN == 256) {
        return taps == 2 ? launch1<BN, PREC, true, 2>(ka, smem, st) : launch1<BN, PREC, true, 1>(ka, smem, st);
    } else {
        if constexpr (BN == 128) {
            if (taps == 2) return launch1<BN, PREC, true, 2>(ka, smem, st);
        }
        return vec ? launch1<BN, PREC, true, 1>(ka, smem, st) : launch1<BN, PREC, false, 1>(ka, smem, st);
    }
#else
    if constexpr (BN == 256) {
        if (conv) return launch1<BN, PREC, true, 9>(ka, smem, st);
        return taps == 2 ? launch1<BN, PREC, true, 2>(ka, smem, st) : launch1<BN, PREC, true, 1>(ka, smem, st);
    } else {
        if constexpr (BN == 128 && PREC != SGD_PREC_F32) {
            if (conv && vec == 2) return launch1<BN, PREC, true, 9, true>(ka, smem, st);
        }
        if (conv) return vec ? launch1<BN, PREC, true, 9>(ka, smem, st) : launch1<BN, PREC, false, 9>(ka, smem, st);
        if constexpr (BN == 128) {
            if (taps == 2) return launch1<BN, PREC, true, 2>(ka, smem, st);
        }
        return vec ? launch1<BN, PREC, true, 1>(ka, smem, st) : launch1<BN, PREC, false, 1>(ka, smem, st);
    }
#endif
}

}

#ifndef SGDM_IGEMM_PREC
#error "igemm.hip is compiled once per arithmetic mode: -DSGDM_IGEMM_PREC=0|1|2 (build.py); geometry and entry points: igemm_host.hip"
#endif
#ifdef SGDM_DEV_ONE
#define SGD_DISPATCH_BODY(P)                                                                                        \
    const KArgs& ka = *reinterpret_cast<const KArgs*>(kap); (void)bn; (void)vec; (void)taps;                         \
    return launch1<SGDM_DEV_BN, P, true, SGDM_DEV_ONE, SGDM_DEV_DEFER>(ka, smem, st);
#else
#define SGD_DISPATCH_BODY(P)                                                                                        \
    const KArgs& ka = *reinterpret_cast<const KArgs*>(kap);                                                         \
    return bn == 256 ? launch<256, P>(ka, 1, taps, smem, st)                                                         \
                     : (bn == 128 ? launch<128, P>(ka, vec, taps, smem, st) : launch<32, P>(ka, vec, taps, smem, st));
#endif
#if SGDM_IGEMM_PREC == 0
int sgd_igemm_dispatch_f32(const void* kap, int bn, int vec, int taps, size_t smem, hipStream_t st) { SGD_DISPATCH_BODY(SGD_PREC_F32) }
#elif SGDM_IGEMM_PREC == 1 && defined(SGDM_IGEMM_NOPK)
int sgd_igemm_dispatch_f16x3_nopk(const void* kap, int bn, int vec, int taps, size_t smem, hipStream_t st) { SGD_DISPATCH_BODY(SGD_PREC_F16X3) }
#elif SGDM_IGEMM_PREC == 1
int sgd_igemm_dispatch_f16x3(const void* kap, int bn, int vec, int taps, size_t smem, hipStream_t st) { SGD_DISPATCH_BODY(SGD_PREC_F16X3) }
#elif defined(SGDM_IGEMM_NOPK)
int sgd_igemm_dispatch_bf16x3_nopk(const void* kap, int bn, int vec, int taps, size_t smem, hipStream_t st) { SGD_DISPATCH_BODY(SGD_PREC_BF16X3) }
#else
int sgd_igemm_dispatch_bf16x3(const void* kap, int bn, int vec, int taps, size_t smem, hipStream_t st) { SGD_DISPATCH_BODY(SGD_PREC_BF16X3) }
#endif
```

self-guided-diffusion-models_amd/csrc/igemm_host.hip:

```cpp
#include <stdint.h>

#include "igemm_shared.h"

extern "C" int sgd_abi_version(void) { return SGD_ABI_VERSION; }

static inline int pick_bn(int cout) { return (cout % 128 == 0) ? 128 : 32; }

static inline int column_tile(const sgd_igemm_args& a) {
    const int bn = pick_bn(a.cout);
    if (bn != 128 || (a.tune & (SGD_TUNE_NO_SMALL | SGD_TUNE_BN128 | SGD_TUNE_BN256))) return bn;
    const long rows = a.mode == SGD_MODE_CONV3 ? (long)a.n * a.ho * a.wo : (long)a.m;
    const long t128 = ((rows + BM - 1) / BM) * ((a.cout + 127) / 128);
    return t128 * 4 <= device_cus() ? 32 : 128;
}

static int make_geo(const sgd_igemm_args& a, Geo& g, int bn, int& na, int fg = 1) {
    if (a.c0 <= 0 || a.c1 < 0 || a.cout <= 0 || a.y_ld < a.cout) return SGD_ERR_ARG;
    if (a.mode == SGD_MODE_CONV3) {
        if (a.n <= 0 || a.hi <= 0 || a.wi <= 0 || (a.stride != 1 && a.stride != 2)) return SGD_ERR_ARG;
        if (a.stride == 2 && a.resample != SGD_RS_NONE) return SGD_ERR_ARG;
        const bool up = a.resample == SGD_RS_UP2 || a.resample == SGD_RS_ZEROUP2;
        g.hc = a.resample == SGD_RS_AVGPOOL2 ? a.hi / 2 : (up ? a.hi * 2 : a.hi);
        g.wc = a.resample == SGD_RS_AVGPOOL2 ? a.wi / 2 : (up ? a.wi * 2 : a.wi);
        if (a.resample == SGD_RS_AVGPOOL2 && ((a.hi | a.wi) & 1)) return SGD_ERR_ARG;
        const int ho = a.stride == 2 ? (g.hc + 1) / 2 : g.hc, wo = a.stride == 2 ? (g.wc + 1) / 2 : g.wc;
        if (a.ho != ho || a.wo != wo) return SGD_ERR_ARG;
        if (!is_pow2(a.ho) || !is_pow2(a.wo) || a.ho < 2 || a.wo < 2) return SGD_ERR_ARG;
        if (a.res && a.res_mode == SGD_RS_UP2 && ((a.ho | a.wo) & 1)) return SGD_ERR_ARG;
        if ((long)a.n * a.hi * a.wi >= (1L << 31)) return SGD_ERR_ARG;
        int tw = a.wo < 16 ? a.wo : 16;
        int th = BM / tw; if (th > a.ho) th = a.ho;
        while (th * tw > BM) th >>= 1;
        if (a.stride == 2) { if (tw > 8) tw = 8; if (th > 8) th = 8; }
        int nb = BM / (th * tw);
        g.hh = a.stride == 2 ? 2 * th + 1 : th + 2;
        g.hw = a.stride == 2 ? 2 * tw + 1 : tw + 2;
        while (nb > 1 && 3 * (size_t)nb * g.hh * g.hw * LDA * 4 + (size_t)nb * g.hh * g.hw * 32 > 150 * 1024)
            nb >>= 1;
        g.tw_l2 = ilog2(tw); g.th_l2 = ilog2(th); g.nb = nb;
        g.tiles_x = a.wo / tw; g.tiles_y = a.ho / th;
        g.pix = nb * g.hh * g.hw;
        g.mt = ((a.n + nb - 1) / nb) * g.tiles_x * g.tiles_y;
        g.fast_a = g.pix <= FAST_PIX ? 1 : 0;
        na = 3;
    } else if (a.mode == SGD_MODE_FLAT) {
        if (a.m <= 0) return SGD_ERR_ARG;
        if (a.pro == SGD_PRO_AFFINE_NC && a.rows_per_n <= 0) return SGD_ERR_ARG;
        if (a.res && a.res_mode != SGD_RS_NONE) return SGD_ERR_ARG;
        g.tw_l2 = g.th_l2 = 0; g.nb = 1; g.tiles_x = g.tiles_y = 1; g.hh = g.hw = 1; g.hc = g.wc = 1;
        g.pix = BM * fg;
        g.mt = (a.m + BM - 1) / BM;
        g.fast_a = 1;
        na = 3;
    } else {
        return SGD_ERR_ARG;
    }
    g.sparts = 0;
    const int ppt = bn >= 128 ? 1 : 4;
    if (((a.cout | a.y_ld) & 3) == 0 && a.orows_in == 0) {
        if (a.mode == SGD_MODE_CONV3) {
            if (g.nb == 1 && (1 << (g.tw_l2 + g.th_l2)) == BM) g.sparts = g.tiles_x * g.tiles_y * ppt;
        } else if (a.rows_per_n > 0 && a.rows_per_n % BM == 0 && a.m % a.rows_per_n == 0) {
            g.sparts = a.rows_per_n / BM * ppt;
        }
    }
    return SGD_OK;
}

static bool want_bn256(const sgd_igemm_args& a) {
    if (a.tune & SGD_TUNE_BN128) return false;
    if (a.tune & SGD_TUNE_BN256) return true;
    const long rows = a.mode == SGD_MODE_CONV3 ? (long)a.n * a.ho * a.wo : (long)a.m;
    const long mt = (rows + BM - 1) / BM;
    const long t256 = mt * (a.cout_p / 256), t128 = mt * (a.cout_p / 128);
    if (a.mode == SGD_MODE_CONV3 && a.prec != SGD_PREC_F32) return t128 <= 256 && a.ho * a.wo <= 64 && a.c0 + a.c1 >= 512;
    if (t256 <= 256 && t128 > 256) return true;
    const long r256 = (t256 + 255) / 256, r128 = (t128 + 255) / 256;
    return r256 * 2.0 < r128 * 1.07;
}

extern "C" int sgd_igemm_tail_layout(int32_t total_tiles, int32_t nchunks, int32_t taps, int32_t grid, int32_t* out) {
    if (!out || grid < 8 || (grid & 7) || total_tiles < 0) return SGD_ERR_ARG;
    const int xchunk = (total_tiles + 7) >> 3, nloc = grid >> 3;
    for (int b = 0; b < grid; ++b) {
        const int xcd = b & 7, loc = b >> 3;
        const int xbeg = xcd * xchunk, xend = (xbeg + xchunk < total_tiles) ? xbeg + xchunk : total_tiles;
        const int xtiles = xend > xbeg ? xend - xbeg : 0;
        const int nfull = xtiles / nloc, xrem = xtiles - nfull * nloc;
        const int split = tail_split(xrem, nloc, nchunks, taps);
        int32_t* o = out + 4 * b;
        o[0] = o[1] = o[2] = o[3] = 0;
        if (split && loc < xrem * split) {
            o[0] = split;
            o[1] = tail_counter(xcd, loc, nloc, split);
            o[2] = tail_slab(xcd, loc, nloc, split);
            o[3] = split - 1;
        }
    }
    return SGD_OK;
}

extern "C" int64_t sgd_igemm_work_bytes(void) {
    return (int64_t)WORK_HEAD + 192 * (int64_t)(BM * 256 * 4);
}

extern "C" int64_t sgd_igemm_work_status_offset(void) { return (int64_t)WORK_STATUS_INT * 4; }

extern "C" int sgd_igemm_stats_parts(const sgd_igemm_args* args) {
    if (!args) return 0;
    Geo g;
    int na;
    if (make_geo(*args, g, column_tile(*args), na) != SGD_OK) return 0;
    return g.sparts;
}

extern "C" int sgd_igemm(const sgd_igemm_args* args, void* stream) {
    SGD_CLEAR_ERR();
    if (!args) return SGD_ERR_ARG;
    KArgs ka;
    ka.a = *args;
    sgd_igemm_args& a = ka.a;
    Geo& g = ka.g;
    if (!a.x0 || !a.w || !a.y || a.c0 <= 0 || a.c1 < 0 || a.cout <= 0) return SGD_ERR_ARG;
    if (a.c1 > 0 && (!a.x1 || a.c0 % KC != 0)) return SGD_ERR_ARG;
    if (a.y_ld < a.cout) return SGD_ERR_ARG;
    if (a.pro != SGD_PRO_NONE && (!a.pa || !a.pb)) return SGD_ERR_ARG;
    const int cin = a.c0 + a.c1;
    int bn = column_tile(a);
    if (a.cout_p % pick_bn(a.cout) != 0 || a.cout_p < a.cout || a.cin_p % KC != 0 || a.cin_p < cin) return SGD_ERR_ARG;
    const bool vec = (a.c0 % 4 == 0) && (a.c1 % 4 == 0);
    if (bn == 128 && a.cout_p % 256 == 0 && vec && (!a.res || a.res_mode == SGD_RS_NONE) && want_bn256(a)) bn = 256;
    int na;
    const bool conv = a.mode == SGD_MODE_CONV3;
    int taps = conv ? 9 : 1;
    const bool ln_nopk = !conv && a.pro == SGD_PRO_LN_ROW && a.prec != SGD_PREC_F32 && !(a.tune & SGD_TUNE_LN_PACKED);
    const bool ln_any = !conv && a.pro == SGD_PRO_LN_ROW && (ln_nopk || (a.tune & SGD_TUNE_LN_PACKED));
    if (!conv && vec && bn >= 128 && a.drop_p == 0.f && cin % (2 * KC) == 0 && (a.c1 == 0 || a.c0 % KC == 0)
        && (a.pro == SGD_PRO_NONE || (a.pro == SGD_PRO_AFFINE_NC && a.rows_per_n > 0 && a.rows_per_n % BM == 0) || ln_any)
        && (a.tune & SGD_TUNE_FLAT2))
        taps = 2;
    {
        const int rc = make_geo(a, g, bn, na, conv ? 1 : taps);
        if (rc != SGD_OK) return rc;
    }
    if (a.stats && g.sparts == 0) return SGD_ERR_ARG;
    g.nt = a.cout_p / bn;
    if ((a.work && a.work_bytes < sgd_igemm_work_bytes()) || (a.tune & SGD_TUNE_PLAIN_SCHEDULE)) a.work = nullptr;
    {
        const long rows_out = a.mode == SGD_MODE_CONV3 ? (long)a.n * a.ho * a.wo : (long)a.m;
        const long rows_res = a.res_mode == SGD_RS_AVGPOOL2 ? rows_out * 4 : rows_out;
        if (rows_out >= (1L << 31) || rows_res >= (1L << 31)) return SGD_ERR_ARG;
    }
#ifdef SGDM_PROBE
    {
        const char* e = getenv("SGDM_DBG");
        g.dbg = e ? atoi(e) : 0;
        const char* sp = getenv("SGDM_STAMP_PTR");
        g.stamp = sp ? reinterpret_cast<unsigned long long*>(strtoull(sp, nullptr, 0)) : nullptr;
        const char* tp = getenv("SGDM_TRACE_PTR");
        g.trace = tp ? reinterpret_cast<unsigned long long*>(strtoull(tp, nullptr, 0)) : nullptr;
    }
#endif
    const size_t smem = (size_t)na * g.pix * LDA * sizeof(float) + (size_t)g.pix * 32
                        + (a.cout_p <= BIAS_LDS_MAX ? (size_t)a.cout_p * sizeof(float) : 0);
    if (smem > 160 * 1024) return SGD_ERR_ARG;
    hipStream_t st = (hipStream_t)stream;
    int variant = vec ? 1 : 0;
    size_t smem_launch = smem;
    {
        const int nchunks = (cin + KC - 1) / KC;
        const long rows_out = (long)a.n * a.ho * a.wo;
        const size_t smem_defer = smem + (size_t)BM * (128 + 4) * sizeof(float);
        if (conv && vec && bn == 128 && a.prec != SGD_PREC_F32 && ((a.cout | a.y_ld) & 3) == 0
            && (!a.res || a.res_mode == SGD_RS_NONE) && a.resample != SGD_RS_AVGPOOL2 && a.cout_p <= BIAS_LDS_MAX && nchunks >= 3
            && rows_out * a.y_ld * 4 < (1L << 32) && (!a.stats || (long)a.n * g.sparts * 2 * a.cout * 4 < (1L << 32))
            && smem_defer <= 160 * 1024 && (a.tune & SGD_TUNE_DEFER)) {
            variant = 2;
            smem_launch = smem_defer;
        }
    }
    switch (a.prec) {
        case SGD_PREC_F32: return sgd_igemm_dispatch_f32(&ka, bn, variant, taps, smem_launch, st);
        case SGD_PREC_F16X3: return ln_nopk ? sgd_igemm_dispatch_f16x3_nopk(&ka, bn, variant, taps, smem_launch, st)
                                            : sgd_igemm_dispatch_f16x3(&ka, bn, variant, taps, smem_launch, st);
        case SGD_PREC_BF16X3: return ln_nopk ? sgd_igemm_dispatch_bf16x3_nopk(&ka, bn, variant, taps, smem_launch, st)
                                             : sgd_igemm_dispatch_bf16x3(&ka, bn, variant, taps, smem_launch, st);
        default: return SGD_ERR_ARG;
    }
}
```

self-guided-diffusion-models_amd/csrc/pack.hip:

```cpp
#include "igemm_shared.h"
#include "prologue.h"

namespace {

__device__ __forceinline__ float pow2_scale_of(uint32_t amax_bits) {
    const float amax = __uint_as_float(amax_bits);
    if (!(amax >= 1.17549435e-38f) || !(amax < 3.0e38f)) return 1.f;
    int e;
    frexpf(amax, &e);
    return ldexpf(1.f, 1 - e);
}

__device__ __forceinline__ void weight_amax_body(const float* __restrict__ w, long count, uint32_t* __restrict__ amax_bits, int vec,
                                                 int blk, int nblk) {
    float m = 0.f;
    if (vec) {
        const long nq = count >> 2;
        const long q0 = (blk * (long)blockDim.x + threadIdx.x) * 4;
        const long step = (long)nblk * blockDim.x * 4;
        for (long q = q0; q < nq; q += step) {
            f32x4 v[4];
#pragma unroll
            for (int j = 0; j < 4; ++j) {
                const long qq = q + j < nq ? q + j : nq - 1;
                v[j] = *reinterpret_cast<const f32x4*>(w + qq * 4);
            }
#pragma unroll
            for (int j = 0; j < 4; ++j)
#pragma unroll
                for (int e = 0; e < 4; ++e) m = fmaxf(m, fabsf(v[j][e]));
        }
        for (long i = (nq << 2) + blk * (long)blockDim.x + threadIdx.x; i < count; i += (long)nblk * blockDim.x)
            m = fmaxf(m, fabsf(w[i]));
    } else {
        for (long i = blk * (long)blockDim.x + threadIdx.x; i < count; i += (long)nblk * blockDim.x) m = fmaxf(m, fabsf(w[i]));
    }
    m = wave_max(m);
    __shared__ float wm[4];
    if ((threadIdx.x & 63) == 0) wm[threadIdx.x >> 6] = m;
    __syncthreads();
    if (threadIdx.x == 0) atomicMax(amax_bits, __float_as_uint(fmaxf(fmaxf(wm[0], wm[1]), fmaxf(wm[2], wm[3]))));
}
__global__ void weight_amax_kernel(const float* __restrict__ w, long count, uint32_t* __restrict__ amax_bits, int vec) {
    weight_amax_body(w, count, amax_bits, vec, blockIdx.x, gridDim.x);
}

template <int PREC>
__device__ __forceinline__ void pack_weight_body(const float* __restrict__ src, float* __restrict__ dst, int cout, int cin,
                                                 int ks, int cout_p, int cin_p, int transpose, const uint32_t* __restrict__ amax_bits,
                                                 float* __restrict__ scale_inv_out, int blk, int grid_blocks) {
    const float wscale = amax_bits ? pow2_scale_of(*amax_bits) : 1.f;
    if (scale_inv_out && blk == 0 && threadIdx.x == 0) *scale_inv_out = 1.f / wscale;
    constexpr int NKS = PREC == SGD_PREC_F32 ? 4 : 2;
    constexpr int CPL = PREC == SGD_PREC_F32 ? 4 : 8;
    const int kk = ks * ks, nblk = cout_p >> 5;
    const long total = (long)(cin_p >> 5) * kk * nblk * NKS * 64;
    for (long i = blk * (long)blockDim.x + threadIdx.x; i < total; i += (long)grid_blocks * blockDim.x) {
        const int lane = i & 63;
        long t = i >> 6;
        const int sub = t % NKS; t /= NKS;
        const long unit = t;
        const int nb = t % nblk; t /= nblk;
        const int tap = t % kk;
        const int chunk = t / kk;
        const int co = nb * 32 + (lane & 31);
        const int ci0 = chunk * 32 + sub * (2 * CPL) + (lane >> 5) * CPL;
        float v[CPL];
#pragma unroll
        for (int j = 0; j < CPL; ++j) {
            const int ci = ci0 + j;
            float x = 0.f;
            if (ci < cin && co < cout) {
                if (!transpose) x = src[((long)co * cin + ci) * kk + tap];
                else x = src[((long)ci * cout + co) * kk + (kk - 1 - tap)];
            }
            v[j] = x * wscale;
        }
        if constexpr (PREC == SGD_PREC_F32) {
            *reinterpret_cast<f32x4*>(dst + unit * 1024 + sub * 256 + lane * 4) = f32x4{v[0], v[1], v[2], v[3]};
        } else {
            typedef typename Split<PREC>::T T;
            typedef T T8 __attribute__((ext_vector_type(8)));
            T8 h, l;
#pragma unroll
            for (int j = 0; j < 8; ++j) {
                T hj, lj;
                Split<PREC>::split(v[j], hj, lj);
                h[j] = hj;
                l[j] = lj;
            }
            T* up = reinterpret_cast<T*>(dst + unit * 1024) + sub * 1024 + lane * 8;
            *reinterpret_cast<T8*>(up) = h;
            *reinterpret_cast<T8*>(up + 512) = l;
        }
    }
}
template <int PREC>
__global__ void pack_weight_kernel(const float* __restrict__ src, float* __restrict__ dst, int cout, int cin,
                                   int ks, int cout_p, int cin_p, int transpose, const uint32_t* __restrict__ amax_bits,
                                   float* __restrict__ scale_inv_out) {
    pack_weight_body<PREC>(src, dst, cout, cin, ks, cout_p, cin_p, transpose, amax_bits, scale_inv_out, blockIdx.x, gridDim.x);
}

__global__ void pack_zero_amax_kernel(const sgd_pack_job* __restrict__ jobs, int n) {
    const int i = blockIdx.x * blockDim.x + threadIdx.x;
    if (i < n && jobs[i].own_amax && jobs[i].amax_bits) *jobs[i].amax_bits = 0u;
}
__global__ void weight_amax_batched_kernel(const sgd_pack_job* __restrict__ jobs, const int32_t* __restrict__ block_job,
                                           const int32_t* __restrict__ first) {
    const int j = block_job[blockIdx.x];
    const sgd_pack_job jb = jobs[j];
    const long count = (long)jb.cout * jb.cin * jb.ksize * jb.ksize;
    weight_amax_body(jb.src, count, jb.amax_bits, (((uintptr_t)jb.src) & 15) == 0 && count >= 4, blockIdx.x - first[j], first[j + 1] - first[j]);
}
template <int PREC>
__global__ void pack_weight_batched_kernel(const sgd_pack_job* __restrict__ jobs, const int32_t* __restrict__ block_job,
                                           const int32_t* __restrict__ first) {
    const int j = block_job[blockIdx.x];
    const sgd_pack_job jb = jobs[j];
    const int co = jb.transpose ? jb.cin : jb.cout, ci = jb.transpose ? jb.cout : jb.cin;
    const int bn = (co % 128 == 0) ? 128 : 32;
    const int cout_p = ((co + bn - 1) / bn) * bn, cin_p = ((ci + KC - 1) / KC) * KC;
    pack_weight_body<PREC>(jb.src, reinterpret_cast<float*>(jb.dst), co, ci, jb.ksize, cout_p, cin_p, jb.transpose, jb.amax_bits,
                           jb.scale_inv, blockIdx.x - first[j], first[j + 1] - first[j]);
}

}

static inline int pick_bn(int cout) { return (cout % 128 == 0) ? 128 : 32; }

extern "C" int64_t sgd_packed_weight_bytes(int32_t cout, int32_t cin, int32_t ksize, int32_t prec) {
    (void)prec;
    const int bn = pick_bn(cout);
    const int64_t cout_p = (int64_t)((cout + bn - 1) / bn) * bn;
    const int64_t cin_p = (int64_t)((cin + KC - 1) / KC) * KC;
    return (int64_t)ksize * ksize * cout_p * cin_p * 4;
}

static int pack_weight_impl(const float* w_src, void* w_dst, int32_t cout, int32_t cin, int32_t ksize, int32_t prec,
                            int32_t* cin_p_out, int32_t* cout_p_out, int transpose, void* stream,
                            const uint32_t* amax_bits = nullptr, float* scale_inv_out = nullptr) {
    SGD_CLEAR_ERR();
    if (!w_src || !w_dst || cout <= 0 || cin <= 0 || (ksize != 1 && ksize != 3)) return SGD_ERR_ARG;
    const int bn = pick_bn(cout);
    const int cout_p = ((cout + bn - 1) / bn) * bn;
    const int cin_p = ((cin + KC - 1) / KC) * KC;
    if (cin_p_out) *cin_p_out = cin_p;
    if (cout_p_out) *cout_p_out = cout_p;
    const long total = (long)ksize * ksize * cout_p * cin_p / (prec == SGD_PREC_F32 ? 4 : 8);
    int grid = (int)((total + 255) / 256);
    if (grid > 4096) grid = 4096;
    hipStream_t st = (hipStream_t)stream;
    float* dst = reinterpret_cast<float*>(w_dst);
    if (prec == SGD_PREC_F32) hipLaunchKernelGGL((pack_weight_kernel<SGD_PREC_F32>), dim3(grid), dim3(256), 0, st, w_src, dst, cout, cin, ksize, cout_p, cin_p, transpose, amax_bits, scale_inv_out);
    else if (prec == SGD_PREC_F16X3) hipLaunchKernelGGL((pack_weight_kernel<SGD_PREC_F16X3>), dim3(grid), dim3(256), 0, st, w_src, dst, cout, cin, ksize, cout_p, cin_p, transpose, amax_bits, scale_inv_out);
    else if (prec == SGD_PREC_BF16X3) hipLaunchKernelGGL((pack_weight_kernel<SGD_PREC_BF16X3>), dim3(grid), dim3(256), 0, st, w_src, dst, cout, cin, ksize, cout_p, cin_p, transpose, amax_bits, scale_inv_out);
    else return SGD_ERR_ARG;
    return sgd_check_launch();
}

extern "C" int sgd_pack_weight(const float* w_src, void* w_dst, int32_t cout, int32_t cin, int32_t ksize,
                               int32_t prec, int32_t* cin_p_out, int32_t* cout_p_out, void* stream) {
    return pack_weight_impl(w_src, w_dst, cout, cin, ksize, prec, cin_p_out, cout_p_out, 0, stream);
}

extern "C" int sgd_pack_weight_dgrad(const float* w_src, void* w_dst, int32_t cout_fwd, int32_t cin_fwd, int32_t ksize,
                                     int32_t prec, int32_t* cin_p_out, int32_t* cout_p_out, void* stream) {
    return pack_weight_impl(w_src, w_dst, cin_fwd, cout_fwd, ksize, prec, cin_p_out, cout_p_out, 1, stream);
}

extern "C" int sgd_weight_amax(const float* w, int64_t count, uint32_t* amax_bits, void* stream) {
    SGD_CLEAR_ERR();
    if (!w || !amax_bits || count <= 0) return SGD_ERR_ARG;
    const int vec = (((uintptr_t)w) & 15) == 0 && count >= 4;
    long grid = vec ? (count + 4095) / 4096 : (count + 1023) / 1024;
    if (grid > 256) grid = 256;
    hipLaunchKernelGGL(weight_amax_kernel, dim3((unsigned)grid), dim3(256), 0, (hipStream_t)stream, w, (long)count, amax_bits, vec);
    return sgd_check_launch();
}

extern "C" int sgd_pack_weight_scaled(const float* w_src, void* w_dst, int32_t cout, int32_t cin, int32_t ksize, int32_t prec,
                                      int32_t transpose, const uint32_t* amax_bits, float* scale_inv_out, int32_t* cin_p_out,
                                      int32_t* cout_p_out, void* stream) {
    if (!amax_bits || !scale_inv_out) return SGD_ERR_ARG;
    if (transpose) return pack_weight_impl(w_src, w_dst, cin, cout, ksize, prec, cin_p_out, cout_p_out, 1, stream, amax_bits, scale_inv_out);
    return pack_weight_impl(w_src, w_dst, cout, cin, ksize, prec, cin_p_out, cout_p_out, 0, stream, amax_bits, scale_inv_out);
}

extern "C" int sgd_pack_job_blocks(int32_t cout, int32_t cin, int32_t ksize, int32_t prec, int32_t transpose, int32_t* amax_blocks,
                                   int32_t* pack_blocks, int32_t* cin_p_out, int32_t* cout_p_out) {
    if (cout <= 0 || cin <= 0 || (ksize != 1 && ksize != 3)) return SGD_ERR_ARG;
    const int co = transpose ? cin : cout, ci = transpose ? cout : cin;
    const int bn = pick_bn(co);
    const int cout_p = ((co + bn - 1) / bn) * bn, cin_p = ((ci + KC - 1) / KC) * KC;
    const long count = (long)cout * cin * ksize * ksize;
    long ab = (count + 4095) / 4096;
    if (ab > 256) ab = 256;
    const long total = (long)ksize * ksize * cout_p * cin_p / (prec == SGD_PREC_F32 ? 4 : 8);
    long pb = (total + 255) / 256;
    if (pb > 4096) pb = 4096;
    if (amax_blocks) *amax_blocks = (int32_t)ab;
    if (pack_blocks) *pack_blocks = (int32_t)pb;
    if (cin_p_out) *cin_p_out = cin_p;
    if (cout_p_out) *cout_p_out = cout_p;
    return SGD_OK;
}

extern "C" int sgd_pack_weights_batched(const sgd_pack_job* jobs, int32_t n_jobs, const int32_t* amax_block_job,
                                        const int32_t* amax_first, int32_t n_amax_blocks, const int32_t* pack_block_job,
                                        const int32_t* pack_first, int32_t n_pack_blocks, int32_t prec, void* stream) {
    SGD_CLEAR_ERR();
    if (!jobs || n_jobs <= 0 || !pack_block_job || !pack_first || n_pack_blocks <= 0) return SGD_ERR_ARG;
    hipStream_t st = (hipStream_t)stream;
    if (prec != SGD_PREC_F32 && n_amax_blocks > 0) {
        if (!amax_block_job || !amax_first) return SGD_ERR_ARG;
        hipLaunchKernelGGL(pack_zero_amax_kernel, dim3((n_jobs + 255) / 256), dim3(256), 0, st, jobs, n_jobs);
        hipLaunchKernelGGL(weight_amax_batched_kernel, dim3(n_amax_blocks), dim3(256), 0, st, jobs, amax_block_job, amax_first);
    }
    if (prec == SGD_PREC_F32) hipLaunchKernelGGL((pack_weight_batched_kernel<SGD_PREC_F32>), dim3(n_pack_blocks), dim3(256), 0, st, jobs, pack_block_job, pack_first);
    else if (prec == SGD_PREC_F16X3) hipLaunchKernelGGL((pack_weight_batched_kernel<SGD_PREC_F16X3>), dim3(n_pack_blocks), dim3(256), 0, st, jobs, pack_block_job, pack_first);
    else if (prec == SGD_PREC_BF16X3) hipLaunchKernelGGL((pack_weight_batched_kernel<SGD_PREC_BF16X3>), dim3(n_pack_blocks), dim3(256), 0, st, jobs, pack_block_job, pack_first);
    else return SGD_ERR_ARG;
    return sgd_check_launch();
}
```

self-guided-diffusion-models_amd/sgdm_amd/_lib.py:

```python
import ctypes as C
import os

import torch

_HERE = os.path.dirname(os.path.abspath(__file__))
LIB_PATH = os.environ.get("SGDM_LIB_PATH") or os.path.join(_HERE, "lib", "libsgdm_hip.so")

MODE_FLAT, MODE_CONV3 = 0, 1
RS_NONE, RS_AVGPOOL2, RS_UP2, RS_ZEROUP2 = 0, 1, 2, 3
PRO_NONE, PRO_AFFINE_NC, PRO_LN_ROW = 0, 1, 2
PREC_F32, PREC_F16X3, PREC_BF16X3 = 0, 1, 2
PREC_BY_NAME = {"f32": PREC_F32, "f16x3": PREC_F16X3, "bf16x3": PREC_BF16X3}
ABI_VERSION = 22

TUNE_BN128, TUNE_BN256, TUNE_FLAT2, TUNE_DEFER, TUNE_PLAIN_SCHEDULE, TUNE_LN_PACKED, TUNE_NO_SMALL = 1, 2, 4, 8, 16, 32, 64
TUNE_WGRAD_GENERIC_NARROW, TUNE_WGRAD_NO_POOLED_PLANES, TUNE_WGRAD_F32 = 256, 512, 1024
TUNE_WGRAD_NO_WS, TUNE_WGRAD_NO_PLANES, TUNE_WGRAD_NO_PIPE, TUNE_WGRAD_PLANES_ALWAYS = 2048, 4096, 8192, 16384

vp, i32, i64, f32 = C.c_void_p, C.c_int32, C.c_int64, C.c_float


class IgemmArgs(C.Structure):
    _fields_ = [
        ("x0", vp), ("x1", vp), ("c0", i32), ("c1", i32), ("mode", i32),
        ("n", i32), ("hi", i32), ("wi", i32), ("ho", i32), ("wo", i32), ("m", i32),
        ("rows_per_n", i32), ("stride", i32), ("resample", i32), ("pro", i32), ("pro_silu", i32),
        ("pa", vp), ("pb", vp), ("pc", vp), ("w", vp), ("cin_p", i32), ("cout_p", i32),
        ("bias", vp), ("res", vp), ("res_mode", i32), ("y", vp), ("cout", i32), ("y_ld", i32),
        ("orows_in", i32), ("orows_out", i32), ("orow_off", i32), ("prec", i32),
        ("drop_p", f32), ("drop_seed", C.c_uint32), ("stats", vp), ("w_scale_inv", vp),
        ("work", vp), ("work_bytes", i64), ("grid_cap", i32), ("tune", i32),
    ]


class PackJob(C.Structure):
    _fields_ = [("src", vp), ("dst", vp), ("amax_bits", vp), ("scale_inv", vp), ("cout", i32), ("cin", i32), ("ksize", i32),
                ("transpose", i32), ("own_amax", i32), ("reserved0", i32)]


SIGNATURES = {
    "sgd_abi_version": (i32, []),
    "sgd_build_id": (C.c_char_p, []),
    "sgd_igemm": (i32, [C.POINTER(IgemmArgs), vp]),
    "sgd_igemm_stats_parts": (i32, [C.POINTER(IgemmArgs)]),
    "sgd_igemm_work_bytes": (i64, []),
    "sgd_igemm_work_status_offset": (i64, []),
    "sgd_igemm_tail_layout": (i32, [i32, i32, i32, i32, C.POINTER(i32)]),
    "sgd_stats_reduce": (i32, [vp, i32, i32, i32, vp, i32, i32, vp]),
    "sgd_packed_weight_bytes": (i64, [i32, i32, i32, i32]),
    "sgd_pack_weight": (i32, [vp, vp, i32, i32, i32, i32, C.POINTER(i32), C.POINTER(i32), vp]),
    "sgd_weight_amax": (i32, [vp, i64, vp, vp]),
    "sgd_pack_weight_scaled": (i32, [vp, vp, i32, i32, i32, i32, i32, vp, vp, C.POINTER(i32), C.POINTER(i32), vp]),
    "sgd_pack_job_blocks": (i32, [i32, i32, i32, i32, i32, C.POINTER(i32), C.POINTER(i32), C.POINTER(i32), C.POINTER(i32)]),
    "sgd_pack_weights_batched": (i32, [vp, i32, vp, vp, i32, vp, vp, i32, i32, vp]),
    "sgd_linear_splitk": (i32, [vp, i32, vp, vp, i32, i32, i32, vp, i32, vp, i32, vp]),
    "sgd_linear_splitk_t": (i32, [vp, i32, vp, i32, i32, i32, i32, vp, i32, vp, i32, vp]),
    "sgd_conv3_narrow_in_parts": (i32, [i32, i32]),
    "sgd_conv3_narrow_in": (i32, [vp, vp, vp, vp, vp, i32, i32, i32, i32, i32, i32, i32, vp]),
    "sgd_conv3_narrow_out": (i32, [vp, vp, vp, i32, vp, vp, vp, i32, i32, i32, i32, i32, i32, vp]),
    "sgd_chan_stats": (i32, [vp, i32, i32, i32, vp, i32, i32, vp]),
    "sgd_gn_coef_parts": (i32, [vp, i32, i32, vp, i32, i32, vp, vp, vp, vp, i32, i32, i32, i32, f32, vp, vp, vp]),
    "sgd_gn_coef": (i32, [vp, vp, vp, vp, i32, i32, i32, i32, i32, f32, vp, vp, vp]),
    "sgd_add_rows_nc": (i32, [vp, vp, i32, i32, i64, i32, vp]),
    "sgd_ln_stats": (i32, [vp, i32, i32, f32, vp, vp]),
    "sgd_ln_apply": (i32, [vp, vp, vp, vp, i32, i32, f32, vp, vp]),
    "sgd_attention": (i32, [vp, i32, i32, vp, vp, i32, i32, i32, i32, i32, i32, i32, f32, vp, i32, vp, vp]),
    "sgd_attention_split": (i32, [vp, i32, i32, vp, vp, i32, i32, i32, i32, i32, i32, i32, f32, vp, i32, vp, vp]),
    "sgd_attention_masked": (i32, [vp, i32, i32, vp, vp, i32, i32, vp, i32, i32, i32, i32, i32, f32, vp, i32, vp, vp]),
    "sgd_linear_attention": (i32, [vp, i32, i32, vp, vp, i32, i32, vp, i32, i32, i32, i32, i32, f32, vp, i32, vp]),
    "sgd_attention_bwd": (i32, [vp, i32, i32, vp, vp, i32, i32, vp, i32, vp, i32, vp, vp, i32, i32, i32, i32, i32, f32,
                              vp, vp, vp, vp]),
    "sgd_attention_bwd_split": (i32, [vp, i32, i32, vp, vp, i32, i32, vp, i32, vp, i32, vp, vp, i32, i32, i32, i32, i32, f32,
                                    vp, vp, vp, vp]),
    "sgd_attention_masked_bwd": (i32, [vp, i32, i32, vp, vp, i32, i32, vp, vp, i32, vp, i32, vp, vp, i32, i32, i32, i32, i32,
                                     f32, vp, vp, vp, vp]),
    "sgd_linear_attention_bwd": (i32, [vp, i32, i32, vp, vp, i32, i32, vp, vp, i32, i32, i32, i32, i32, i32, f32, vp, vp, vp,
                                     vp]),
    "sgd_pack_weight_dgrad": (i32, [vp, vp, i32, i32, i32, i32, C.POINTER(i32), C.POINTER(i32), vp]),
    "sgd_wgrad": (i32, [C.POINTER(IgemmArgs), vp, i32, i32, vp, i32, vp, vp]),
    "sgd_wgrad_scratch_bytes": (i64, [C.POINTER(IgemmArgs), i32]),
    "sgd_wgrad_scratch": (i32, [C.POINTER(IgemmArgs), vp, i32, i32, vp, i32, vp, vp, i64, vp]),
    "sgd_colsum_fold": (i32, [vp, i32, i32, vp, i32, f32, vp]),
    "sgd_wgrad_reduce": (i32, [vp, i32, i32, i32, i32, vp, i32, f32, vp]),
    "sgd_wgrad_reduce_bias": (i32, [vp, i32, i32, i32, i32, vp, i32, f32, vp, i32, vp, vp]),
    "sgd_wgrad_bias_rows": (i32, [C.POINTER(IgemmArgs), i32, i32, i32, i64]),
    "sgd_colsum_pair": (i32, [vp, vp, i32, i32, i32, vp, vp, i32, f32, vp]),
    "sgd_colsum": (i32, [vp, i32, i32, i32, vp, i32, f32, vp, i32, vp]),
    "sgd_gn_bwd_reduce": (i32, [vp, i32, i32, i32, i32, i32, i32, vp, vp, i32, vp, i32, i32, f32, C.c_uint32, vp, vp]),
    "sgd_gn_bwd_coef": (i32, [vp, i32, vp, vp, vp, vp, i32, i32, i32, i32, i32, f32, vp, vp, vp, vp, vp, vp, vp]),
    "sgd_gn_bwd_coef_fold": (i32, [vp, i32, vp, vp, vp, vp, i32, i32, i32, i32, i32, f32, vp, vp, vp, vp, vp, vp, i32, f32, vp]),
    "sgd_gn_bwd_rows_chunks": (i32, [i32, i32, i32, i32]),
    "sgd_gn_bwd_reduce_rows": (i32, [vp, i32, i32, i32, i32, i32, i32, vp, vp, i32, vp, i32, f32, C.c_uint32, i32, vp, vp]),
    "sgd_gn_bwd_apply": (i32, [vp, i32, i32, i32, i32, i32, i32, vp, vp, i32, vp, i32, i32, f32, C.c_uint32, vp, vp, vp, vp, i32, i32,
                             vp, i32, i32, i32, vp]),
    "sgd_silu_bwd": (i32, [vp, vp, i64, vp, vp]),
    "sgd_ln_bwd": (i32, [vp, vp, vp, i32, i32, f32, vp, i32, vp, vp, vp]),
    "sgd_resample_bwd": (i32, [vp, i32, i32, i32, i32, i32, vp, i32, vp]),
    "sgd_q_sample": (i32, [vp, vp, vp, vp, vp, i32, i64, vp, vp]),
    "sgd_mse_loss": (i32, [vp, vp, i32, i32, i32, vp, vp, vp]),
    "sgd_adamw_ema_step": (i32, [vp, vp, i32, i32, f32, f32, f32, f32, f32, f32, f32, f32, f32, vp, vp]),
    "sgd_exchange_bind": (i32, [C.c_char_p]),
    "sgd_allreduce_bucket": (i32, [vp, vp, i64, vp]),
    "sgd_timestep_embedding": (i32, [vp, vp, i32, i32, i32, vp, vp]),
    "sgd_cond_select": (i32, [vp, i32, vp, vp, i32, i32, i32, vp, vp]),
    "sgd_pack_input": (i32, [vp, vp, vp, vp, i32, i32, i32, i32, i32, i32, vp, vp]),
    "sgd_pack_input_compact": (i32, [vp, vp, i32, vp, vp, i32, i32, i32, i32, i32, i32, vp, vp]),
    "sgd_labelmap_nhot": (i32, [vp, i32, i32, i32, vp, vp]),
    "sgd_linear_gather": (i32, [vp, vp, vp, vp, vp, i32, i32, i32, i32, vp, i32, vp]),
    "sgd_linear_sparse_rows": (i32, [vp, vp, vp, vp, vp, i32, i32, i32, i32, vp, i32, vp]),
    "sgd_nhwc_to_nchw": (i32, [vp, i32, i32, i32, i32, vp, vp]),
    "sgd_fill_null_kv": (i32, [vp, i32, i32, i32, i32, vp, vp]),
    "sgd_ddpm_step": (i32, [vp, vp, vp, i32, f32, C.POINTER(f32), i32, i32, i32, i32, vp, vp, vp]),
    "sgd_ddim_step": (i32, [vp, vp, vp, i32, f32, C.POINTER(f32), f32, i32, i32, i32, i32, vp, vp, vp]),
    "sgd_ddpm_step_dev": (i32, [vp, vp, vp, i32, f32, vp, i32, i32, i32, i32, vp, vp, vp]),
    "sgd_ddim_step_dev": (i32, [vp, vp, vp, i32, f32, vp, f32, i32, i32, i32, i32, vp, vp, vp]),
    "sgd_x0_quantile": (i32, [i32, vp, vp, i32, f32, C.POINTER(f32), i32, i32, i32, i32, i32, f32, vp, vp]),
    "sgd_ddpm_step_dyn": (i32, [vp, vp, vp, i32, f32, C.POINTER(f32), vp, i32, i32, i32, vp, vp, vp]),
    "sgd_ddim_step_dyn": (i32, [vp, vp, vp, i32, f32, C.POINTER(f32), f32, vp, i32, i32, i32, vp, vp, vp]),
    "sgd_token_pool": (i32, [vp, i32, i32, i32, i32, vp, vp]),
    "sgd_geglu": (i32, [vp, i64, i32, vp, vp]),
    "sgd_to_uint8": (i32, [vp, i64, vp, vp]),
    "sgd_cfg_combine": (i32, [vp, i32, f32, i32, i32, i32, vp, vp]),
    "sgd_pndm_step": (i32, [vp, vp, i32, f32, vp, vp, vp, vp, i32, i32, i32, vp, vp]),
}

TOOLS_LIB_PATH = os.path.join(_HERE, "lib", "libsgdm_hip_tools.so")
TOOLS_SIGNATURES = {
    "sgd_debug_occupy": (i32, [i32, f32, vp]),
    "sgd_debug_mfma_probe": (i32, [i32, i64, C.c_uint32, i32, vp, vp]),
    "sgd_debug_mfma_probe_flops": (i64, [i32, i64, i32]),
    "sgd_debug_copy_probe": (i32, [vp, vp, i64, i32, i32, vp]),
    "sgd_debug_mfma_lds_probe": (i32, [i32, i64, C.c_uint32, i32, i32, vp, vp]),
    "sgd_debug_mfma_stream_probe": (i32, [i32, i64, C.c_uint32, i32, vp, vp, i64, vp, vp]),
}

_lib = None
_tools = None


class HipLibraryError(RuntimeError):
    pass


def load():
    global _lib
    if _lib is not None:
        return _lib
    if not os.path.exists(LIB_PATH):
        raise HipLibraryError(
            f"{LIB_PATH} not found: the HIP extension is not built "
            "(run `python self-guided-diffusion-models_amd/build.py`). There is no CPU fallback.")
    lib = C.CDLL(LIB_PATH)
    for name, (res, args) in SIGNATURES.items():
        try:
            fn = getattr(lib, name)
        except AttributeError as e:
            raise HipLibraryError(f"{LIB_PATH} does not export {name}") from e
        fn.restype = res
        fn.argtypes = args
    if lib.sgd_abi_version() != ABI_VERSION:
        raise HipLibraryError(f"ABI mismatch: library {lib.sgd_abi_version()} != binding {ABI_VERSION}")
    _lib = lib
    return lib


def load_tools():
    global _tools
    if _tools is not None:
        return _tools
    if not os.path.exists(TOOLS_LIB_PATH):
        raise HipLibraryError(f"{TOOLS_LIB_PATH} not found (run `python self-guided-diffusion-models_amd/build.py`)")
    lib = C.CDLL(TOOLS_LIB_PATH)
    for name, (res, args) in TOOLS_SIGNATURES.items():
        try:
            fn = getattr(lib, name)
        except AttributeError as e:
            raise HipLibraryError(f"{TOOLS_LIB_PATH} does not export {name}") from e
        fn.restype = res
        fn.argtypes = args
    _tools = lib
    return lib


def check(rc, what):
    if rc != 0:
        raise RuntimeError(f"{what} failed with code {rc} "
                           f"({'invalid argument' if rc == 1 else 'launch failure'})")
```

self-guided-diffusion-models_amd/sgdm_amd/unet.py:

```python
import ctypes as C
import weakref
import math
import os

import torch
import torch.nn as nn

from . import _lib as L

GN_GROUPS, GN_EPS, LN_EPS = 32, 1e-5, 1e-5
NUM_TIME_TOKENS = NUM_COND_TOKENS = 8


def _ptr(t):
    return C.c_void_p(t.data_ptr()) if t is not None else C.c_void_p(0)


def timestep_freqs(dim, max_period=10000):
    half = dim // 2
    return torch.exp(-math.log(max_period) * torch.arange(start=0, end=half, dtype=torch.float32) / half)


def default_precision():
    return os.environ.get("SGDM_PREC", "f32")


class _Node(nn.Module):
    pass


def _register(root, name, shape, kind, init):
    parts = name.split(".")
    node = root
    for p in parts[:-1]:
        if p not in node._modules:
            node.add_module(p, _Node())
        node = node._modules[p]
    t = init(shape)
    if kind == "buffer":
        node.register_buffer(parts[-1], t)
    else:
        node.register_parameter(parts[-1], nn.Parameter(t, requires_grad=(kind == "param")))


def _get(root, name):
    obj = root
    for p in name.split("."):
        obj = getattr(obj, p) if not p.isdigit() else obj._modules[p]
    return obj


def _init_weight(shape):
    w = torch.empty(shape)
    nn.init.kaiming_uniform_(w, a=math.sqrt(5))
    return w


def _init_bias_for(fan_in):
    def f(shape):
        b = torch.empty(shape)
        bound = 1 / math.sqrt(fan_in) if fan_in > 0 else 0
        nn.init.uniform_(b, -bound, bound)
        return b
    return f


_zeros = lambda s: torch.zeros(s)
_ones = lambda s: torch.ones(s)
_randn = lambda s: torch.randn(s)


class _Spec:

    def __init__(self):
        self.items = []

    def linear(self, p, i, o, bias=True, zero=False):
        self.items.append((p + ".weight", (o, i), "param", _zeros if zero else _init_weight))
        if bias:
            self.items.append((p + ".bias", (o,), "param", _zeros if zero else _init_bias_for(i)))

    def conv(self, p, i, o, k, dims=2, zero=False):
        self.items.append((p + ".weight", (o, i) + (k,) * dims, "param", _zeros if zero else _init_weight))
        self.items.append((p + ".bias", (o,), "param", _zeros if zero else _init_bias_for(i * k ** dims)))

    def norm(self, p, c):
        self.items.append((p + ".weight", (c,), "param", _ones))
        self.items.append((p + ".bias", (c,), "param", _zeros))


AMAX_OF = {}


HEAD_DIMS = (16, 32, 64, 128)


def padded_head_dim(d):
    for dp in HEAD_DIMS:
        if dp >= d:
            return dp
    raise ValueError(f"attention head width {d} > {HEAD_DIMS[-1]} is not supported")


class _Pad:

    def __init__(self, rows=None, n_rows=None, cols=None, n_cols=None):
        self.rows = None if rows is None else torch.as_tensor(rows, dtype=torch.int64)
        self.cols = None if cols is None else torch.as_tensor(cols, dtype=torch.int64)
        self.n_rows, self.n_cols = n_rows, n_cols

    def _idx(self, dev):
        if self.rows is not None and self.rows.device != dev:
            self.rows = self.rows.to(dev)
        if self.cols is not None and self.cols.device != dev:
            self.cols = self.cols.to(dev)

    def apply(self, w):
        self._idx(w.device)
        w2 = w.reshape(w.shape[0], -1)
        out = w2.new_zeros(self.n_rows if self.rows is not None else w2.shape[0],
                           self.n_cols if self.cols is not None else w2.shape[1])
        if self.rows is not None and self.cols is not None:
            out[self.rows[:, None], self.cols[None, :]] = w2
        elif self.rows is not None:
            out[self.rows] = w2
        else:
            out[:, self.cols] = w2
        return out

    def gather(self, wp):
        self._idx(wp.device)
        if self.rows is not None:
            wp = wp[self.rows]
        if self.cols is not None:
            wp = wp[:, self.cols]
        return wp


class _Packed:

    def __init__(self, srcs, ksize, prec, pad=None):
        self.srcs = srcs
        self.ksize = ksize
        self.prec = prec
        self.pad = pad
        self.cout = sum(s.shape[0] for s in srcs)
        self.cin = srcs[0].shape[1]
        if pad is not None:
            assert ksize == 1
            self.cout = pad.n_rows if pad.rows is not None else self.cout
            self.cin = pad.n_cols if pad.cols is not None else self.cin
        lib = L.load()
        nbytes = lib.sgd_packed_weight_bytes(self.cout, self.cin, ksize, prec)
        self.buf = torch.empty(nbytes // 4, dtype=torch.float32, device=srcs[0].device)
        self.cin_p = self.cout_p = 0
        self.sig = None
        self.scaled = prec != L.PREC_F32
        if self.scaled:
            self.amax = torch.zeros(1, dtype=torch.int32, device=srcs[0].device)
            self.scale_inv = torch.ones(1, dtype=torch.float32, device=srcs[0].device)

    @property
    def scale_ptr(self):
        return self.scale_inv.data_ptr() if self.scaled else 0

    def refresh(self, stream):
        sig = tuple((s.data_ptr(), s._version) for s in self.srcs)
        if sig == self.sig:
            return
        lib = L.load()
        src = self.srcs[0].detach() if len(self.srcs) == 1 else torch.cat([s.detach() for s in self.srcs], 0)
        src = src.contiguous().float()
        if self.pad is not None:
            src = self.pad.apply(src).contiguous()
        cin_p, cout_p = C.c_int32(0), C.c_int32(0)
        if self.scaled:
            self.amax.zero_()
            L.check(lib.sgd_weight_amax(_ptr(src), src.numel(), _ptr(self.amax), stream), "sgd_weight_amax")
            if len(self.srcs) == 1 and self.pad is None:
                AMAX_OF[self.srcs[0].data_ptr()] = (self.srcs[0]._version, self.amax, weakref.ref(self.srcs[0]))
            L.check(lib.sgd_pack_weight_scaled(_ptr(src), _ptr(self.buf), self.cout, self.cin, self.ksize, self.prec, 0,
                                               _ptr(self.amax), _ptr(self.scale_inv), C.byref(cin_p), C.byref(cout_p),
                                               stream), "sgd_pack_weight_scaled")
        else:
            L.check(lib.sgd_pack_weight(_ptr(src), _ptr(self.buf), self.cout, self.cin, self.ksize, self.prec,
                                        C.byref(cin_p), C.byref(cout_p), stream), "sgd_pack_weight")
        self.cin_p, self.cout_p = cin_p.value, cout_p.value
        self._keep = src
        self.sig = sig


class _PackBatch:

    MIN_STALE = 8

    def __init__(self, packs, prec, dev):
        self.packs, self.prec, self.dev = list(packs), prec, dev
        self.lib = L.load()
        self.members, self.table_sig = None, None

    @staticmethod
    def _source(pk):
        if hasattr(pk, "srcs"):
            if len(pk.srcs) != 1 or pk.pad is not None:
                return None
            p, t = pk.srcs[0], 0
            cout, cin = pk.cout, pk.cin
        else:
            if len(pk.deps) != 1:
                return None
            p, t = pk.deps[0], 1
            src = pk.src_fn()
            if src.data_ptr() != p.data_ptr() or src.numel() != p.numel():
                return None
            cout, cin = pk.cout_fwd, pk.cin_fwd
        if p.dtype != torch.float32 or not p.is_contiguous() or p.numel() != cout * cin * pk.ksize * pk.ksize:
            return None
        return p, cout, cin, t

    def _build(self):
        members, jobs = [], []
        ab, pb = C.c_int32(), C.c_int32()
        cp, op = C.c_int32(), C.c_int32()
        a_job, a_first, p_job, p_first = [], [0], [], [0]
        scaled = self.prec != L.PREC_F32
        for pk in self.packs:
            srcd = self._source(pk)
            if srcd is None:
                continue
            p, cout, cin, t = srcd
            L.check(self.lib.sgd_pack_job_blocks(cout, cin, pk.ksize, self.prec, t, C.byref(ab), C.byref(pb), C.byref(cp),
                                                 C.byref(op)), "sgd_pack_job_blocks")
            j = len(members)
            jobs.append(L.PackJob(src=p.data_ptr(), dst=pk.buf.data_ptr(), amax_bits=pk.amax.data_ptr() if scaled else 0,
                                  scale_inv=pk.scale_inv.data_ptr() if scaled else 0, cout=cout, cin=cin, ksize=pk.ksize,
                                  transpose=t, own_amax=1 if scaled else 0))
            members.append((pk, p, cp.value, op.value))
            a_job += [j] * (ab.value if scaled else 0)
            a_first.append(len(a_job))
            p_job += [j] * pb.value
            p_first.append(len(p_job))
        self.members = members
        self.table_sig = tuple(p.data_ptr() for _, p, _, _ in members)
        if not members:
            return
        arr = (L.PackJob * len(jobs))(*jobs)
        self.jobs = torch.frombuffer(bytearray(C.string_at(C.addressof(arr), C.sizeof(arr))), dtype=torch.uint8).to(self.dev)
        i32t = lambda v: torch.tensor(v if v else [0], dtype=torch.int32, device=self.dev)
        self.a_job, self.a_first, self.p_job, self.p_first = i32t(a_job), i32t(a_first), i32t(p_job), i32t(p_first)
        self.n_a, self.n_p = len(a_job), len(p_job)
        self.batched = {id(pk) for pk, _, _, _ in members}

    def refresh(self, stream):
        if self.members is None or self.table_sig != tuple(p.data_ptr() for _, p, _, _ in self.members):
            self._build()
        stale = [(pk, p, cp, op) for pk, p, cp, op in self.members if pk.sig != ((p.data_ptr(), p._version),)]
        if len(stale) >= self.MIN_STALE and os.environ.get("SGDM_BATCHED_PACK", "1") != "0":
            L.check(self.lib.sgd_pack_weights_batched(_ptr(self.jobs), len(self.members), _ptr(self.a_job), _ptr(self.a_first),
                                                      self.n_a, _ptr(self.p_job), _ptr(self.p_first), self.n_p, self.prec,
                                                      stream), "sgd_pack_weights_batched")
            for pk, p, cp, op in self.members:
                pk.cin_p, pk.cout_p = cp, op
                pk.sig = ((p.data_ptr(), p._version),)
                if hasattr(pk, "srcs") and pk.scaled:
                    AMAX_OF[p.data_ptr()] = (p._version, pk.amax, weakref.ref(p))
        for pk in self.packs:
            pk.refresh(stream)


class _Program:
    def __init__(self):
        self.ops = []
        self.meta = []
        self.keep = []

    def add(self, name, fn, *args, flops=0.0, nbytes=0.0):
        self.ops.append((name, fn, args))
        self.meta.append((getattr(fn, "__name__", "op"), flops, nbytes))

    def run(self, stream):
        for name, fn, args in self.ops:
            rc = fn(*args, stream)
            if rc:
                L.check(rc, name)

    def run_profiled(self, stream):
        evs = []
        for name, fn, args in self.ops:
            e0, e1 = torch.cuda.Event(enable_timing=True), torch.cuda.Event(enable_timing=True)
            e0.record()
            rc = fn(*args, stream)
            e1.record()
            if rc:
                L.check(rc, name)
            evs.append((e0, e1))
        torch.cuda.synchronize()
        return [(op[0], mt[0], e0.elapsed_time(e1), mt[1], mt[2])
                for op, mt, (e0, e1) in zip(self.ops, self.meta, evs)]


class UNetModelBase(nn.Module):
    KIND = None

    def _setup(self, image_size, in_channels, model_channels, out_channels, num_res_blocks,
               attention_resolutions, dropout, channel_mult, conv_resample, dims, use_checkpoint, use_fp16,
               num_heads, num_head_channels, num_heads_upsample, use_scale_shift_norm, resblock_updown,
               cond_dim, condition, condition_method):
        if dims != 2:
            raise NotImplementedError("HIP path implements dims=2 only")
        if use_fp16:
            raise NotImplementedError("use_fp16=True is not supported (reference configs use fp32)")
        if num_heads == -1 and num_head_channels == -1:
            raise AssertionError("Either num_heads or num_head_channels has to be set")
        if not conv_resample:
            raise NotImplementedError("HIP path implements conv_resample=True (ctor default)")
        self.image_size = image_size
        self.in_channels = in_channels
        self.model_channels = model_channels
        self.out_channels = out_channels
        self.num_res_blocks = num_res_blocks
        self.attention_resolutions = tuple(attention_resolutions)
        self.dropout = dropout
        self.channel_mult = tuple(channel_mult)
        self.conv_resample = conv_resample
        self.use_checkpoint = use_checkpoint
        self.dtype = torch.float32
        self.num_heads = num_heads
        self.num_head_channels = num_head_channels
        self.num_heads_upsample = num_heads if num_heads_upsample == -1 else num_heads_upsample
        self.use_scale_shift_norm = use_scale_shift_norm
        self._film_mult = 2 if use_scale_shift_norm else 1
        self.resblock_updown = resblock_updown
        self.cond_dim = 0 if cond_dim is None else cond_dim
        self.condition = condition
        self.condition_method = condition_method
        self.hip_precision = default_precision()
        self._engines = {}

    def _heads_for(self, ch, up=False):
        if self.num_head_channels == -1:
            return self.num_heads_upsample if up else self.num_heads
        return ch // self.num_head_channels

    def _walk(self):
        mc, cm, nrb = self.model_channels, self.channel_mult, self.num_res_blocks
        inp = [[("conv", self._in_ch_total, mc)]]
        chans = [mc]
        ch, ds = mc, 1
        for level, mult in enumerate(cm):
            for _ in range(nrb):
                layers = [("res", ch, mult * mc, None)]
                ch = mult * mc
                if ds in self.attention_resolutions:
                    layers.append(("attn", ch, self._heads_for(ch)))
                inp.append(layers)
                chans.append(ch)
            if level != len(cm) - 1:
                inp.append([("res", ch, ch, "down")] if self.resblock_updown else [("down", ch)])
                chans.append(ch)
                ds *= 2
        mid = [("res", ch, ch, None), ("attn", ch, self._heads_for(ch)), ("res", ch, ch, None)]
        out = []
        for level, mult in list(enumerate(cm))[::-1]:
            for i in range(nrb + 1):
                ich = chans.pop()
                layers = [("res", ch + ich, mc * mult, None)]
                ch = mc * mult
                if ds in self.attention_resolutions:
                    layers.append(("attn", ch, self._heads_for(ch, up=True)))
                if level and i == nrb:
                    layers.append(("res", ch, ch, "up") if self.resblock_updown else ("up", ch))
                    ds //= 2
                out.append(layers)
        return inp, mid, out

    def _layer_spec(self, sp, p, layer):
        kind = layer[0]
        if kind == "conv":
            sp.conv(p, layer[1], layer[2], 3)
        elif kind == "res":
            _, cin, cout, _ud = layer
            sp.norm(p + ".in_layers.0", cin)
            sp.conv(p + ".in_layers.2", cin, cout, 3)
            sp.linear(p + ".emb_layers.1", self._emb_ch, self._film_mult * cout)
            sp.norm(p + ".out_layers.0", cout)
            sp.conv(p + ".out_layers.3", cout, cout, 3, zero=True)
            if cin != cout:
                sp.conv(p + ".skip_connection", cin, cout, 1)
        elif kind == "attn":
            self._attn_spec(sp, p, layer[1], layer[2])
        elif kind == "down":
            sp.conv(p + ".op", layer[1], layer[1], 3)
        elif kind == "up":
            sp.conv(p + ".conv", layer[1], layer[1], 3)

    def _register_all(self, sp_head):
        sp = sp_head
        inp, mid, out = self._walk()
        self._plan = (inp, mid, out)
        for i, blk in enumerate(inp):
            for j, layer in enumerate(blk):
                self._layer_spec(sp, f"input_blocks.{i}.{j}", layer)
        for j, layer in enumerate(mid):
            self._layer_spec(sp, f"middle_block.{j}", layer)
        for i, blk in enumerate(out):
            for j, layer in enumerate(blk):
                self._layer_spec(sp, f"output_blocks.{i}.{j}", layer)
        sp.norm("out.0", self.model_channels)
        sp.conv("out.2", self.model_channels, self.out_channels, 3, zero=True)
        for name, shape, kind, init in sp.items:
            _register(self, name, shape, kind, init)
        self._manifest = [(n, tuple(s), k) for n, s, k, _ in sp.items]

    def P(self, name):
        return _get(self, name)

    def get_guided_score(self, z, zc, w):
        st = self.condition["scale_type"] if isinstance(self.condition, dict) else self.condition.scale_type
        if st == "imagen":
            return (1 - w) * z + w * zc
        elif st == "cfg":
            return (1 + w) * zc - w * z
        raise ValueError(st)

    def _scale_mode(self):
        st = self.condition["scale_type"] if isinstance(self.condition, dict) else self.condition.scale_type
        if st == "imagen":
            return 1
        if st == "cfg":
            return 2
        raise ValueError(st)

    def convert_to_fp16(self):
        pass

    def convert_to_fp32(self):
        pass

    def _engine(self, n, h, w, prec):
        dev = self._device()
        sig = tuple(p.data_ptr() for p in self._all_tensors())
        key = (n, h, w, prec)
        eng = self._engines.get(key)
        if eng is None or eng.sig != sig:
            eng = _Engine(self, n, h, w, prec, dev)
            eng.sig = sig
            self._engines[key] = eng
        return eng

    def _all_tensors(self):
        if not hasattr(self, "_tensor_list") or self._tensor_list_n != len(self._manifest):
            self._tensor_list = [self.P(n) for n, _, _ in self._manifest]
            self._tensor_list_n = len(self._manifest)
        return self._tensor_list

    def _device(self):
        return self.P(self._manifest[-1][0]).device

    def _check_runnable(self, x):
        if x.device.type != "cuda":
            raise RuntimeError("sgdm_amd UNet runs on the MI355X HIP path only (inputs must be on a cuda "
                               "device); there is no CPU fallback")
        L.load()

    def _draw_mask(self, n, cond_drop_prob, device):
        return torch.zeros((n,), device=device).float().uniform_(0, 1) < cond_drop_prob

    def _run(self, x, t, cond, layout, mask, n):
        self._check_runnable(x)
        if torch.is_grad_enabled() and self.training and any(p.requires_grad for p in self.parameters()):
            from .train import forward_train
            return forward_train(self, x, t, cond, layout, mask, n)
        B, cx, H, W = x.shape
        assert cx == self.in_channels
        prec = L.PREC_BY_NAME[self.hip_precision]
        eng = self._engine(n, H, W, prec)
        eng.run(x, t, cond, layout, mask)
        return eng

    def _to_nchw(self, eng):
        lib = L.load()
        n, H, W = eng.n, eng.h, eng.w
        out = torch.empty(n, self.out_channels, H, W, device=eng.dev, dtype=torch.float32)
        L.check(lib.sgd_nhwc_to_nchw(_ptr(eng.eps_nhwc), n, H, W, self.out_channels, _ptr(out),
                                     torch.cuda.current_stream().cuda_stream), "sgd_nhwc_to_nchw")
        return out

    def _cfg_combine(self, eng, w, B):
        lib = L.load()
        out = torch.empty(B, self.out_channels, eng.h, eng.w, device=eng.dev, dtype=torch.float32)
        L.check(lib.sgd_cfg_combine(_ptr(eng.eps_nhwc), self._scale_mode(), float(w), B, self.out_channels,
                                    eng.h * eng.w, _ptr(out), torch.cuda.current_stream().cuda_stream),
                "sgd_cfg_combine")
        return out


def device_cus(dev):
    return int(torch.cuda.get_device_properties(dev).multi_processor_count)


_GRAD_HEALTH = {}


def grad_health(dev):
    dev = torch.device(dev)
    key = (dev.type, dev.index if dev.index is not None else (torch.cuda.current_device() if dev.type == "cuda" else 0))
    if key not in _GRAD_HEALTH:
        _GRAD_HEALTH[key] = torch.zeros(1, dtype=torch.float32, device=dev)
    return _GRAD_HEALTH[key]


class _Engine:

    def __init__(self, model, n, h, w, prec, dev):
        self.m, self.n, self.h, self.w, self.prec, self.dev = model, n, h, w, prec, dev
        self.lib = L.load()
        self.prog = _Program()
        self.packed = []
        self.bufs = []
        self.tape = []
        self.drops = []
        self.lse = {}
        self.stats_of = {}
        self._p_drop = 0.0
        self._grid_cap = 0
        self.refresh_hooks = []
        self.work_bytes = int(self.lib.sgd_igemm_work_bytes()) if os.environ.get("SGDM_BALANCE", "1") != "0" else 0
        self.work = torch.zeros(max(1, self.work_bytes // 4), dtype=torch.float32, device=dev)
        self._build()

    def buf(self, *shape, dtype=torch.float32):
        t = torch.empty(*shape, dtype=dtype, device=self.dev)
        self.bufs.append(t)
        return t

    def attention_fn(self):
        return self.lib.sgd_attention_split if self.prec == L.PREC_F16X3 else self.lib.sgd_attention

    def pack(self, names, ksize, pad=None):
        pk = _Packed([self.m.P(nm) for nm in names], ksize, self.prec, pad)
        self.packed.append(pk)
        return pk

    def padded(self, name, pad):
        src = self.m.P(name)
        buf = self.buf(*pad.apply(src.detach().reshape(-1, src.shape[-1]) if src.dim() > 1 else src.detach().reshape(1, -1)).shape)
        box = dict(sig=None)

        def hook(stream):
            sig = (src.data_ptr(), src._version)
            if sig != box["sig"]:
                v = src.detach().float()
                buf.copy_(pad.apply(v.reshape(-1, v.shape[-1]) if v.dim() > 1 else v.reshape(1, -1)))
                box["sig"] = sig
        self.refresh_hooks.append(hook)
        return buf

    def igemm(self, tag, x0, c0, y, cout, pk, *, x1=None, c1=0, conv=None, m=0, rows_per_n=0,
              pro=L.PRO_NONE, silu=0, pa=None, pb=None, pc=None, bias=None, res=None, res_mode=L.RS_NONE,
              y_ld=None, y_off=0, orows=(0, 0, 0), stats=False, launch=True):
        a = L.IgemmArgs()
        a.x0, a.x1, a.c0, a.c1 = x0.data_ptr(), (x1.data_ptr() if x1 is not None else 0), c0, c1
        rows_n = conv[0] if conv is not None else (m // rows_per_n if rows_per_n else 0)
        if conv is not None:
            nimg, hi, wi, ho, wo, stride, resample = conv
            a.mode, a.n, a.hi, a.wi, a.ho, a.wo, a.stride, a.resample = L.MODE_CONV3, nimg, hi, wi, ho, wo, stride, resample
        else:
            a.mode, a.m, a.rows_per_n, a.stride = L.MODE_FLAT, m, rows_per_n, 1
        a.pro, a.pro_silu = pro, silu
        a.pa = pa.data_ptr() if pa is not None else 0
        a.pb = pb.data_ptr() if pb is not None else 0
        a.pc = pc.data_ptr() if pc is not None else 0
        a.w = pk.buf.data_ptr()
        a.w_scale_inv = pk.scale_ptr
        a.bias = bias.data_ptr() if bias is not None else 0
        a.res = res.data_ptr() if res is not None else 0
        a.res_mode = res_mode
        a.y = y.data_ptr() + 4 * y_off
        a.cout = cout
        a.y_ld = y_ld if y_ld is not None else cout
        a.orows_in, a.orows_out, a.orow_off = orows
        a.prec = self.prec
        if self.work_bytes:
            a.work, a.work_bytes = self.work.data_ptr(), self.work_bytes
        narrow = (conv is not None and launch and c1 == 0 and c0 in (3, 4) and pro == L.PRO_NONE and not silu and res is None
                  and conv[5] == 1 and conv[6] == 0 and cout % 4 == 0 and cout <= 1024 and y_off == 0 and orows == (0, 0, 0)
                  and len(pk.srcs) == 1 and pk.pad is None and pk.srcs[0].dtype == torch.float32 and pk.srcs[0].is_contiguous()
                  and os.environ.get("SGDM_NARROW_CONV", "1") != "0")
        narrow_out = (conv is not None and launch and not narrow and c1 == 0 and cout in (3, 4) and c0 % 32 == 0 and res is None
                      and pro in (L.PRO_NONE, L.PRO_AFFINE_NC) and conv[5] == 1 and conv[6] == 0 and y_off == 0
                      and orows == (0, 0, 0) and not stats and len(pk.srcs) == 1 and pk.pad is None
                      and pk.srcs[0].dtype == torch.float32 and os.environ.get("SGDM_NARROW_CONV", "1") != "0")
        if stats and os.environ.get("SGDM_FUSED_STATS", "1") != "0":
            parts = self.lib.sgd_conv3_narrow_in_parts(conv[3], conv[4]) if narrow else self.lib.sgd_igemm_stats_parts(C.byref(a))
            if parts > 0:
                sbuf = self.buf(rows_n, parts, 2, cout)
                a.stats = sbuf.data_ptr()
                self.stats_of[y.data_ptr()] = (sbuf, parts, cout)
        self.prog.keep.append((a, pk))
        self._late.append((a, pk))
        rows = conv[0] * conv[3] * conv[4] if conv is not None else m
        rows_in = conv[0] * conv[1] * conv[2] if conv is not None else m
        taps = 9 if conv is not None else 1
        cin = c0 + c1
        flops = 2.0 * rows * cout * taps * cin
        nbytes = 4.0 * (rows_in * cin + rows * cout * (2 if res is not None else 1) + taps * cin * cout)
        if narrow:
            wsrc, fn = pk.srcs[0], self.lib.sgd_conv3_narrow_in
            x_p, b_p, y_p, s_p = _ptr(x0), C.c_void_p(a.bias or 0), C.c_void_p(a.y), C.c_void_p(a.stats or 0)
            nimg, ho, wo, y_ld = conv[0], conv[3], conv[4], a.y_ld

            def sgd_conv3_narrow_in(stream):
                return fn(x_p, C.c_void_p(wsrc.data_ptr()), b_p, y_p, s_p, nimg, ho, wo, c0, cout, y_ld, 0, stream)
            self.prog.add(tag, sgd_conv3_narrow_in, flops=flops, nbytes=nbytes)
        elif narrow_out:
            wsrc, fn = pk.srcs[0], self.lib.sgd_conv3_narrow_out
            w9 = self.buf(9, cout, c0)
            box = dict(sig=None)

            def refresh_w9(stream, w9=w9, wsrc=wsrc, box=box):
                sig = (wsrc.data_ptr(), wsrc._version)
                if sig != box["sig"]:
                    w9.copy_(wsrc.detach().float().permute(2, 3, 0, 1).reshape(9, cout, c0))
                    box["sig"] = sig
            self.refresh_hooks.append(refresh_w9)
            x_p, y_p, b_p, w_p = _ptr(x0), C.c_void_p(a.y), C.c_void_p(a.bias or 0), _ptr(w9)
            pa_p, pb_p = C.c_void_p(a.pa or 0), C.c_void_p(a.pb or 0)
            nimg, ho, wo, y_ld = conv[0], conv[3], conv[4], a.y_ld

            def sgd_conv3_narrow_out(stream):
                return fn(x_p, pa_p, pb_p, int(silu), w_p, b_p, y_p, nimg, ho, wo, c0, cout, y_ld, stream)
            self.prog.add(tag, sgd_conv3_narrow_out, flops=flops, nbytes=nbytes)
        elif launch:
            self.prog.add(tag, self.lib.sgd_igemm, C.byref(a), flops=flops, nbytes=nbytes)
        return a

    def gn(self, tag, srcs, hw, gname, film=None, film_ld=0, eps=GN_EPS):
        n = self.n
        ct = sum(c for _, c in srcs)
        sums = self.buf(n, ct, 2)
        off = 0
        parts = []
        for t, c in srcs:
            st = self.stats_of.get(t.data_ptr())
            if st is not None and st[2] == c:
                parts.append((st[0], st[1], c))
            else:
                self.prog.add(tag + ".stats", self.lib.sgd_chan_stats, _ptr(t), n, hw, c, _ptr(sums), ct, off)
                parts.append((None, 0, c))
            off += c
        a, b = self.buf(n, ct), self.buf(n, ct)
        self._last_sums = sums
        gw, gb = self.m.P(gname + ".weight"), self.m.P(gname + ".bias")
        if len(parts) <= 2 and any(p[1] > 0 for p in parts):
            (p0, n0, c0), (p1, n1, c1) = parts[0], (parts[1] if len(parts) == 2 else (None, 0, 0))
            self.prog.add(tag + ".coef", self.lib.sgd_gn_coef_parts, _ptr(p0) if p0 is not None else None, n0, c0,
                          _ptr(p1) if p1 is not None else None, n1, c1, _ptr(sums), _ptr(gw), _ptr(gb),
                          C.c_void_p(film or 0), film_ld, n, GN_GROUPS, hw, eps, _ptr(a), _ptr(b))
        else:
            self.prog.add(tag + ".coef", self.lib.sgd_gn_coef, _ptr(sums), _ptr(gw), _ptr(gb), C.c_void_p(film or 0),
                          film_ld, n, ct, GN_GROUPS, hw, eps, _ptr(a), _ptr(b))
        return a, b

    def _build(self):
        m, n, H, W = self.m, self.n, self.h, self.w
        self._late = []
        mc = m.model_channels
        ted = 4 * mc
        P = m.P
        lib = self.lib
        self.temb = self.buf(n, mc)
        self.freqs = timestep_freqs(mc).to(self.dev)
        cin_tot = m._in_ch_total
        self.x_in = self.buf(n, H, W, cin_tot)
        self.cond_m = self.buf(n, max(1, m._cond_width)) if m._cond_width else None
        emb = self.buf(n, ted)
        e1 = self.buf(n, ted)
        a0 = self.igemm("time_embed.0", self.temb, mc, e1, ted, self.pack(["time_embed.0.weight"], 1), m=n,
                        bias=P("time_embed.0.bias"))
        a2 = self.igemm("time_embed.2", e1, ted, emb, ted, self.pack(["time_embed.2.weight"], 1), m=n, silu=1,
                        bias=P("time_embed.2.bias"))
        self.tape.append(dict(kind="mlp2", name="time_embed", x=self.temb, h=e1, y=emb, a0=a0, a2=a2, cin=mc,
                              mid=ted, cout=ted, add_to_y=False))
        self.context = None
        self.emb_c = None
        m._build_cond_path(self, emb)
        res_names = m._res_prefixes()
        fm = m._film_mult
        film_w = sum(fm * co for _, co in res_names)
        film = self.buf(n, film_w)
        fbias = self.buf(film_w)
        self._film_bias_src = [P(p + ".emb_layers.1.bias") for p, _ in res_names]
        self._film_bias = fbias
        ec = self.emb_c
        af = self.igemm("emb_layers", emb, ted, film, film_w,
                        self.pack([p + ".emb_layers.1.weight" for p, _ in res_names], 1), m=n, silu=1, bias=fbias,
                        x1=ec, c1=(m._emb_ch - ted) if ec is not None else 0)
        self.tape.append(dict(kind="film", emb_t=emb, emb_c=ec, film=film, film_w=film_w, a=af,
                              names=[p for p, _ in res_names], couts=[co for _, co in res_names]))
        self.film, self.film_ld = film, film_w
        self.film_off = {}
        off = 0
        for p, co in res_names:
            self.film_off[p] = off
            off += fm * co
        inp, mid, out = m._plan
        hs = []
        cur = (self.x_in, cin_tot, H, W)
        for i, blk in enumerate(inp):
            cur = self._block(f"input_blocks.{i}", blk, [cur])
            hs.append(cur)
        cur = self._block("middle_block", mid, [cur])
        for i, blk in enumerate(out):
            cur = self._block(f"output_blocks.{i}", blk, [cur, hs.pop()])
        t, c, hh, ww = cur
        a, b = self.gn("out.0", [(t, c)], hh * ww, "out.0")
        self.eps_nhwc = self.buf(n, hh, ww, m.out_channels)
        ah = self.igemm("out.2", t, c, self.eps_nhwc, m.out_channels, self.pack(["out.2.weight"], 3),
                        conv=(n, hh, ww, hh, ww, 1, L.RS_NONE), pro=L.PRO_AFFINE_NC, silu=1, pa=a, pb=b,
                        bias=P("out.2.bias"))
        self.tape.append(dict(kind="head", x=t, c=c, hw=(hh, ww), a=a, b=b, sums=self._last_sums, conv=ah))

    def _block(self, prefix, blk, srcs):
        for j, layer in enumerate(blk):
            p = f"{prefix}.{j}"
            kind = layer[0]
            if kind == "conv":
                (t, c, hh, ww), = srcs
                y = self.buf(self.n, hh, ww, layer[2])
                a = self.igemm(p, t, c, y, layer[2], self.pack([p + ".weight"], 3),
                               conv=(self.n, hh, ww, hh, ww, 1, L.RS_NONE), bias=self.m.P(p + ".bias"), stats=True)
                self.tape.append(dict(kind="conv_in", p=p, x=t, y=y, a=a, cin=c, cout=layer[2], hw=(hh, ww)))
                srcs = [(y, layer[2], hh, ww)]
            elif kind == "res":
                srcs = [self._res(p, layer, srcs)]
            elif kind == "attn":
                srcs = [self.m._build_attn(self, p, layer, srcs[0])]
            elif kind == "down":
                (t, c, hh, ww), = srcs
                y = self.buf(self.n, hh // 2, ww // 2, c)
                a = self.igemm(p + ".op", t, c, y, c, self.pack([p + ".op.weight"], 3),
                               conv=(self.n, hh, ww, hh // 2, ww // 2, 2, L.RS_NONE), bias=self.m.P(p + ".op.bias"),
                               stats=True)
                self.tape.append(dict(kind="down", p=p, x=t, y=y, c=c, hw_in=(hh, ww), a=a))
                srcs = [(y, c, hh // 2, ww // 2)]
            elif kind == "up":
                (t, c, hh, ww), = srcs
                y = self.buf(self.n, hh * 2, ww * 2, c)
                a = self.igemm(p + ".conv", t, c, y, c, self.pack([p + ".conv.weight"], 3),
                               conv=(self.n, hh, ww, hh * 2, ww * 2, 1, L.RS_UP2), bias=self.m.P(p + ".conv.bias"),
                               stats=True)
                self.tape.append(dict(kind="up", p=p, x=t, y=y, c=c, hw_in=(hh, ww), a=a))
                srcs = [(y, c, hh * 2, ww * 2)]
        return srcs[0]

    def _res(self, p, layer, srcs):
        _, cin, cout, ud = layer
        n, P = self.n, self.m.P
        t0, c0, hh, ww = srcs[0]
        t1, c1 = (srcs[1][0], srcs[1][1]) if len(srcs) == 2 else (None, 0)
        assert c0 + c1 == cin
        rs = {None: L.RS_NONE, "down": L.RS_AVGPOOL2, "up": L.RS_UP2}[ud]
        ho, wo = (hh // 2, ww // 2) if ud == "down" else ((hh * 2, ww * 2) if ud == "up" else (hh, ww))
        ss = self.m.use_scale_shift_norm
        a1, b1 = self.gn(p + ".in_layers.0", [(t0, c0)] + ([(t1, c1)] if t1 is not None else []), hh * ww,
                         p + ".in_layers.0")
        sums1 = self._last_sums
        h1 = self.buf(n, ho, wo, cout)
        ac1 = self.igemm(p + ".in_layers.2", t0, c0, h1, cout, self.pack([p + ".in_layers.2.weight"], 3), x1=t1,
                         c1=c1, conv=(n, hh, ww, ho, wo, 1, rs), pro=L.PRO_AFFINE_NC, silu=1, pa=a1, pb=b1,
                         bias=P(p + ".in_layers.2.bias"), stats=ss)
        film_ptr = self.film.data_ptr() + 4 * self.film_off[p]
        if ss:
            a2, b2 = self.gn(p + ".out_layers.0", [(h1, cout)], ho * wo, p + ".out_layers.0", film=film_ptr,
                             film_ld=self.film_ld)
        else:
            self.prog.add(p + ".emb_add", self.lib.sgd_add_rows_nc, _ptr(h1), C.c_void_p(film_ptr), self.film_ld, n, ho * wo, cout)
            a2, b2 = self.gn(p + ".out_layers.0", [(h1, cout)], ho * wo, p + ".out_layers.0")
        sums2 = self._last_sums
        ask = None
        if cin != cout:
            assert ud is None
            skip = self.buf(n, hh, ww, cout)
            ask = self.igemm(p + ".skip_connection", t0, c0, skip, cout,
                             self.pack([p + ".skip_connection.weight"], 1), x1=t1, c1=c1, m=n * hh * ww,
                             bias=P(p + ".skip_connection.bias"))
            res, res_mode = skip, L.RS_NONE
        else:
            assert t1 is None
            res, res_mode = t0, rs
        y = self.buf(n, ho, wo, cout)
        ac2 = self.igemm(p + ".out_layers.3", h1, cout, y, cout, self.pack([p + ".out_layers.3.weight"], 3),
                         conv=(n, ho, wo, ho, wo, 1, L.RS_NONE), pro=L.PRO_AFFINE_NC, silu=1, pa=a2, pb=b2,
                         bias=P(p + ".out_layers.3.bias"), res=res, res_mode=res_mode, stats=True)
        pbox, sbox = C.c_float(0.0), C.c_uint32(0)
        self.drops.append((ac2, pbox, sbox))
        self.tape.append(dict(kind="res", drop_p=pbox, drop_seed=sbox, p=p,
                              srcs=[(t0, c0)] + ([(t1, c1)] if t1 is not None else []), cin=cin,
                              cout=cout, hw_in=(hh, ww), hw_out=(ho, wo), rs=rs, a1=a1, b1=b1, sums1=sums1, h1=h1,
                              a2=a2, b2=b2, sums2=sums2, film_off=self.film_off[p], conv1=ac1, conv2=ac2, skip=ask,
                              y=y, ss=ss))
        return (y, cout, ho, wo)

    def refresh(self, stream):
        if getattr(self, "_pack_batch", None) is None or len(self._pack_batch.packs) != len(self.packed):
            self._pack_batch = _PackBatch(self.packed, self.prec, self.dev)
        self._pack_batch.refresh(stream)
        for a, pk in self._late:
            a.cin_p, a.cout_p = pk.cin_p, pk.cout_p
        for hook in self.refresh_hooks:
            hook(stream)
        sig = tuple((b.data_ptr(), b._version) for b in self._film_bias_src)
        if sig != getattr(self, "_film_sig", None):
            self._film_bias.copy_(torch.cat([b.detach().reshape(-1) for b in self._film_bias_src]))
            self._film_sig = sig

    def _health_fail(self, training=False):
        self.work.zero_()
        what = ("sgdm_amd: a conv launch's balanced tail timed out waiting for another block's partial sums (stale arrival "
                "counters: a faulted launch, or two streams on one engine); the affected outputs were poisoned with NaN.  The "
                "workspace has been re-zeroed")
        if not training:
            raise RuntimeError(what + ": rerun the step.")
        grad_health(self.dev).zero_()
        raise RuntimeError(what + ".  The gradients of that training iteration are invalid on every rank (the flag travels "
                           "with the gradient exchange).  sgdm_amd.optim.FusedAdamWEma skipped its step for them -- parameters, "
                           "moments and EMA shadows are untouched: repeat the iteration.  Any other optimizer has consumed "
                           "non-finite gradients: restore the last checkpoint.")

    def check_health(self):
        if self.work_bytes:
            off = int(self.lib.sgd_igemm_work_status_offset()) // 4
            if int(self.work.view(torch.int32)[off].item()) != 0:
                self._health_fail()

    def health_word(self):
        if not self.work_bytes:
            return None
        if getattr(self, "_health_off", None) is None:
            self._health_off = int(self.lib.sgd_igemm_work_status_offset()) // 4
        return self.work.view(torch.int32)[self._health_off:self._health_off + 1]

    def note_health(self, flag=None):
        if not self.work_bytes:
            return
        if getattr(self, "_health_host", None) is None:
            self._health_host = torch.zeros(1, dtype=torch.float32).pin_memory()
        self._health_host.copy_(flag if flag is not None else self.health_word(), non_blocking=True)
        self._health_training = flag is not None
        self._health_ev = torch.cuda.Event()
        self._health_ev.record()

    def poll_health(self):
        ev = getattr(self, "_health_ev", None)
        if ev is not None and ev.query():
            self._health_ev = None
            if float(self._health_host[0]) != 0:
                self._health_fail(training=getattr(self, "_health_training", False))

    def set_grid_cap(self, reserve):
        cap = 0 if reserve <= 0 else max(8, device_cus(self.dev) - int(reserve))
        if cap == getattr(self, "_grid_cap", 0):
            return
        self._grid_cap = cap
        bw = getattr(self, "backward", None)
        if bw is not None:
            bw.apply_grid_cap()

    def run(self, x, t, cond, layout, mask, train=False):
        stream = torch.cuda.current_stream().cuda_stream
        self.prepare(x, t, cond, layout, mask, train=train)
        self.launch(stream)

    def prepare(self, x, t, cond, layout, mask, train=False):
        m, n = self.m, self.n
        stream = torch.cuda.current_stream().cuda_stream
        self.poll_health()
        self.refresh(stream)
        from .ddp import reserved_cus
        self.set_grid_cap(reserved_cus(m) if train else 0)
        p_drop = float(m.dropout) if (train and m.dropout) else 0.0
        if p_drop != self._p_drop or p_drop > 0:
            seeds = torch.randint(0, 2 ** 31 - 1, (len(self.drops),)).tolist() if p_drop > 0 else [0] * len(self.drops)
            for (a, pbox, sbox), sd in zip(self.drops, seeds):
                a.drop_p, a.drop_seed = p_drop, sd
                pbox.value, sbox.value = p_drop, sd
            self._p_drop = p_drop
        B = x.shape[0]
        assert n % B == 0
        x = x.contiguous().float()
        t = t.contiguous().to(torch.int64)
        mask_u8 = mask.contiguous().view(torch.uint8) if mask is not None else None
        cl = m._in_ch_total - m.in_channels
        lfmt = 0
        if cl:
            if layout is None:
                raise ValueError(f"condition_method={m.condition_method} needs `layout`")
            if layout.dtype == torch.uint8 and layout.numel() == B * self.h * self.w:
                layout, lfmt = layout.contiguous(), 1
            elif layout.dtype in (torch.int32, torch.int64) and tuple(layout.shape) == (B, 4):
                if cl != 1:
                    raise ValueError("box-corner layouts need layout_dim == 1")
                layout, lfmt = layout.to(torch.int32).contiguous(), 2
            else:
                layout = layout.contiguous().float()
                assert layout.shape == (B, cl, self.h, self.w), (layout.shape, (B, cl, self.h, self.w))
        is_i64 = 0
        if m._cond_width:
            if cond is None:
                raise ValueError(f"condition_method={m.condition_method} needs `cond`")
            cond = cond.contiguous()
            if cond.dtype == torch.int64 and cond.numel() == B and m._cond_width > 1:
                is_i64 = 2
                cond = cond.reshape(B)
            else:
                is_i64 = int(cond.dtype == torch.int64)
                if not is_i64:
                    cond = cond.float()
                assert cond.numel() == B * m._cond_width, (cond.shape, m._cond_width)
        self._keep_inputs = (x, t, cond, layout, mask_u8, B, is_i64, lfmt)
        self._train_mode = bool(train)

    def launch(self, stream):
        m, n, lib = self.m, self.n, self.lib
# ... 520 lines not shown
```

Baseline: 2.161 images/s.

## Replace nearest-upsample-then-3x3 conv with sub-pixel 2x2 conv per output parity

Nearest 2x upsampling followed by a 3x3 conv is rewritten as four 2x2 convolutions on the low-resolution input, one per output parity, using pre-summed weights packed per parity. The implicit-GEMM kernel gains a TAPS=4 variant that selects parity from the tile index, offsets the LDS A reads and the weight base, and scatters outputs to interleaved positions. This removes redundant MACs (4 taps instead of 9) and the upsampled gather for up-blocks and up-resblock first convs. It adds a new weight pack and amax path and is restricted to cases with no residual or dropout. The per-parity pre-summed weights may also change rounding slightly under the split-f16 mode.

```diff
diff --git a/include/sgdm_hip.h b/include/sgdm_hip.h
--- a/include/sgdm_hip.h
+++ b/include/sgdm_hip.h
@@ -6,13 +6,14 @@
 extern "C" {
 #endif
 
-#define SGD_ABI_VERSION 22
+#define SGD_ABI_VERSION 23
 int sgd_abi_version(void);
 const char* sgd_build_id(void);
 
 enum { SGD_MODE_FLAT = 0, SGD_MODE_CONV3 = 1 };
 enum { SGD_RS_NONE = 0, SGD_RS_AVGPOOL2 = 1, SGD_RS_UP2 = 2,
-       SGD_RS_ZEROUP2 = 3  };
+       SGD_RS_ZEROUP2 = 3 ,
+       SGD_RS_UP2_SUBPIXEL = 4 };
 enum { SGD_PRO_NONE = 0, SGD_PRO_AFFINE_NC = 1, SGD_PRO_LN_ROW = 2 };
 enum { SGD_PREC_F32 = 0, SGD_PREC_F16X3 = 1, SGD_PREC_BF16X3 = 2 };
 
@@ -65,7 +66,8 @@
     SGD_TUNE_WGRAD_NO_WS = 2048,
     SGD_TUNE_WGRAD_NO_PLANES = 4096,
     SGD_TUNE_WGRAD_NO_PIPE = 8192,
-    SGD_TUNE_WGRAD_PLANES_ALWAYS = 16384
+    SGD_TUNE_WGRAD_PLANES_ALWAYS = 16384,
+    SGD_TUNE_NO_SUBPIXEL = 32768
 };
 int64_t sgd_igemm_work_bytes(void);
 int64_t sgd_igemm_work_status_offset(void);
@@ -74,10 +76,17 @@
 
 int sgd_igemm(const sgd_igemm_args* args , void* stream);
 int sgd_igemm_stats_parts(const sgd_igemm_args* args );
+int sgd_igemm_subpixel_ok(const sgd_igemm_args* args );
 
 int64_t sgd_packed_weight_bytes(int32_t cout, int32_t cin, int32_t ksize, int32_t prec);
 int sgd_pack_weight(const float* w_src, void* w_dst, int32_t cout, int32_t cin, int32_t ksize,
                     int32_t prec, int32_t* cin_p, int32_t* cout_p , void* stream);
+
+int64_t sgd_packed_weight_subpixel_bytes(int32_t cout, int32_t cin, int32_t prec);
+int sgd_weight_amax_subpixel(const float* w_src, int32_t cout, int32_t cin, uint32_t* amax_bits, void* stream);
+int sgd_pack_weight_subpixel_scaled(const float* w_src, void* w_dst, int32_t cout, int32_t cin, int32_t prec,
+                                    const uint32_t* amax_bits, float* scale_inv_out, int32_t* cin_p, int32_t* cout_p ,
+                                    void* stream);
 
 int sgd_weight_amax(const float* w, int64_t count, uint32_t* amax_bits, void* stream);
 int sgd_pack_weight_scaled(const float* w_src, void* w_dst, int32_t cout, int32_t cin, int32_t ksize, int32_t prec,
@@ -85,6 +94,7 @@
                            const uint32_t* amax_bits, float* scale_inv_out, int32_t* cin_p, int32_t* cout_p ,
                            void* stream);
 
+enum { SGD_PACK_FORWARD = 0, SGD_PACK_DGRAD = 1, SGD_PACK_SUBPIXEL = 2  };
 typedef struct sgd_pack_job {
     const float* src;
     void* dst;
diff --git a/self-guided-diffusion-models_amd/csrc/igemm.hip b/self-guided-diffusion-models_amd/csrc/igemm.hip
--- a/self-guided-diffusion-models_amd/csrc/igemm.hip
+++ b/self-guided-diffusion-models_amd/csrc/igemm.hip
@@ -215,12 +215,21 @@
 struct Tile {
     int n0c;
     int img0, ty0, tx0;
+    int par;
     long m0;
 };
 
+template <bool SUB>
 __device__ __forceinline__ Tile tile_at(const Geo& g, int lin, int bn, int tw, int th) {
     Tile t;
-    const int mtile = lin / g.nt, ntile = lin - mtile * g.nt;
+    int mtile = lin / g.nt;
+    const int ntile = lin - mtile * g.nt;
+    t.par = 0;
+    if constexpr (SUB) {
+        const int mq = g.mt >> 2;
+        t.par = mtile / mq;
+        mtile -= t.par * mq;
+    }
     t.n0c = ntile * bn;
     const int per_img = g.tiles_x * g.tiles_y;
     const int it = mtile / per_img, rem = mtile - it * per_img;
@@ -234,7 +243,8 @@
 
 template <int BN, int PREC, bool VEC, int TAPS, bool DEFER>
 struct IgemmBlock {
-    static constexpr bool CONV = TAPS == 9;
+    static constexpr bool SUBPIX = TAPS == 4;
+    static constexpr bool CONV = TAPS == 9 || SUBPIX;
     static constexpr int FG = CONV ? 1 : TAPS;
     static constexpr int KCC = KC * FG;
     static constexpr int NA = 3;
@@ -253,6 +263,7 @@
 
     static constexpr int STG_LD = BN + 4;
     static_assert(!DEFER || (BN == 128 && TAPS == 9 && VEC && !M16), "loader-side epilogue: 3x3, 128-column tiles");
+    static_assert(!SUBPIX || (VEC && PREC != SGD_PREC_F32 && BN >= 128), "sub-pixel conv: 16-byte inputs, split modes, 128-column tiles");
 
     const sgd_igemm_args& a;
     const Geo& g;
@@ -318,7 +329,7 @@
 
     __device__ __forceinline__ void build_pixtab(int k, int t0, int nthr) const {
         if (k >= ntiles) return;
-        const Tile T = tile_at(g, lin_of(k), BN, TW, TH);
+        const Tile T = tile_at<SUBPIX>(g, lin_of(k), BN, TW, TH);
         int2* tab = pixtab + (size_t)(k & 3) * g.pix;
         for (int pix = t0; pix < g.pix; pix += nthr) {
             int2 e;
@@ -384,7 +395,7 @@
     const int dlt = tid - NCOMP;
     const int dcq = (dlt >> 6) * 8 + (dlt & 7), drg = (dlt & 63) >> 3;
     int dk = 0, dqs = 0, dnck = cend(0) - cbeg(0);
-    Tile dT = tile_at(g, lin_of(0), BN, TW, TH);
+    Tile dT = tile_at<SUBPIX>(g, lin_of(0), BN, TW, TH);
     int dcol = 0;
     unsigned dsoff = 0xFFFFFFFFu;
     f32x4 dres[8], ds1 = {0.f, 0.f, 0.f, 0.f}, ds2 = ds1;
@@ -449,7 +460,7 @@
             if (req) { i0 = (16 * j) / nsl; i1 = (16 * (j + 1)) / nsl; }
             di0 = i0;
             if (dk > 0 && j == 0) {
-                dT = tile_at(g, lin_of(dk - 1), BN, TW, TH);
+                dT = tile_at<SUBPIX>(g, lin_of(dk - 1), BN, TW, TH);
                 const Tile& T = dT;
                 dcol = T.n0c + dcq * 4;
                 const int part = (T.ty0 >> g.th_l2) * g.tiles_x + (T.tx0 >> g.tw_l2);
@@ -524,7 +535,7 @@
                     if (++c.chunk == cend(c.k)) {
                         if (c.k + 1 < ntiles) {
                             ++c.k; c.chunk = cbeg(c.k);
-                            c.img0 = tile_at(g, lin_of(c.k), BN, TW, TH).img0;
+                            c.img0 = tile_at<SUBPIX>(g, lin_of(c.k), BN, TW, TH).img0;
                         }
                         else c.chunk = cend(c.k) - 1;
                     }
@@ -583,7 +594,7 @@
 #pragma unroll
                     for (int j = 0; j < AJ; ++j) issue_item(s2, j);
                 };
-                s2.k = 0; s2.chunk = cbeg(0); s2.img0 = tile_at(g, lin_of(0), BN, TW, TH).img0; fill(s2);
+                s2.k = 0; s2.chunk = cbeg(0); s2.img0 = tile_at<SUBPIX>(g, lin_of(0), BN, TW, TH).img0; fill(s2);
                 load_rows(0);
                 issue_coef(s2);
 #pragma unroll
@@ -635,7 +646,7 @@
             float2 rst[NB_RING][AI];
             struct Cur { int k, chunk; int m0; const float* ka; const float* kb; };
             auto open_tile = [&](Cur& c) {
-                const Tile T = tile_at(g, lin_of(c.k), BN, TW, TH);
+                const Tile T = tile_at<SUBPIX>(g, lin_of(c.k), BN, TW, TH);
                 c.m0 = (int)T.m0;
                 const long ko = tile_uni ? (long)(c.m0 / a.rows_per_n) * cin : 0;
                 c.ka = tile_uni ? a.pa + ko + c4 * 4 : (ln ? a.pb + c4 * 4 : a.x0);
@@ -759,7 +770,7 @@
     auto tabref = [&](int k) {
         TabRef t;
         t.tab = pixtab + (size_t)(k & 3) * g.pix;
-        t.m0 = CONV ? 0 : tile_at(g, lin_of(k), BN, TW, TH).m0;
+        t.m0 = CONV ? 0 : tile_at<SUBPIX>(g, lin_of(k), BN, TW, TH).m0;
         return t;
     };
     auto entry = [&](const TabRef& t, int pix) -> int2 {
@@ -833,7 +844,7 @@
                 cx.chunk = q - k * nchunks + cbeg(k);
                 cx.tab = pixtab + (size_t)(k & 3) * g.pix;
                 cx.c = cx.chunk * KC + c4 * 4;
-                cx.ko = (long)tile_at(g, lin_of(k), BN, TW, TH).img0 * cin + (cx.c < cin ? cx.c : 0);
+                cx.ko = (long)tile_at<SUBPIX>(g, lin_of(k), BN, TW, TH).img0 * cin + (cx.c < cin ? cx.c : 0);
                 return cx;
             };
             Ctx cx = ctx_of(1);
@@ -951,7 +962,8 @@
             const int tx = row & (TW - 1), ty = (row >> g.tw_l2) & (TH - 1), nb = row >> (g.tw_l2 + g.th_l2);
             n = T.img0 + nb; oy = T.ty0 + ty; ox = T.tx0 + tx;
             okm[mt] = nb < g.nb && n < a.n;
-            orow = (n * a.ho + oy) * a.wo + ox;
+            if (SUBPIX) orow = (n * a.ho + 2 * oy + (T.par >> 1)) * a.wo + 2 * ox + (T.par & 1);
+            else orow = (n * a.ho + oy) * a.wo + ox;
         } else {
             orow = (int)T.m0 + row;
             okm[mt] = orow < M;
@@ -974,7 +986,7 @@
             int n_img, part;
             if (CONV) {
                 n_img = T.img0;
-                part = ((T.ty0 >> g.th_l2) * g.tiles_x + (T.tx0 >> g.tw_l2)) * (BM / WM) + wm;
+                part = ((T.par * g.tiles_y + (T.ty0 >> g.th_l2)) * g.tiles_x + (T.tx0 >> g.tw_l2)) * (BM / WM) + wm;
             } else {
                 n_img = (int)(T.m0 / a.rows_per_n);
                 part = (int)((T.m0 % a.rows_per_n) / BM) * (BM / WM) + wm;
@@ -1120,7 +1132,18 @@
         int l;
         asm volatile("v_mbcnt_lo_u32_b32 %0, -1, 0\n\tv_mbcnt_hi_u32_b32 %0, -1, %0" : "=v"(l));
         const int loff = M16 ? (l >> 5) * 2048 + (((l >> 4) & 1) * 32 + (l & 15)) * 16 : l * 16;
-        return reinterpret_cast<const char*>(a.w) + (size_t)(wn * NT + (tile_at(g, lin_of(k), BN, TW, TH).n0c >> 5)) * WUNIT + loff;
+        const Tile T = tile_at<SUBPIX>(g, lin_of(k), BN, TW, TH);
+        const size_t pbase = SUBPIX ? (size_t)T.par * ((size_t)a.cin_p * a.cout_p * 16) : 0;
+        return reinterpret_cast<const char*>(a.w) + pbase + (size_t)(wn * NT + (T.n0c >> 5)) * WUNIT + loff;
+    };
+    auto par_off = [&](int k) __attribute__((always_inline)) {
+        if constexpr (SUBPIX) {
+            const int par = tile_at<SUBPIX>(g, lin_of(k), BN, TW, TH).par;
+            return (par >> 1) * (g.hw * LDA) + (par & 1) * LDA;
+        } else {
+            (void)k;
+            return 0;
+        }
     };
 
     AccV acc[RB][CBN];
@@ -1136,7 +1159,10 @@
     typename Frag16<PREC, 1>::B fb16[CBN];
     const int rowstep = g.hw * LDA;
 
-    auto tap_off = [&](int tap) { return CONV ? (tap / 3) * rowstep + (tap % 3) * LDA : tap * (BM * LDA); };
+    auto tap_off = [&](int tap) {
+        if constexpr (SUBPIX) return (tap >> 1) * rowstep + (tap & 1) * LDA;
+        else return CONV ? (tap / 3) * rowstep + (tap % 3) * LDA : tap * (BM * LDA);
+    };
     auto do_step = [&](const float* acur, const float* anext, auto tapc, auto parc, const char* wnext) {
         constexpr int tap = decltype(tapc)::value;
         constexpr int PAR = decltype(parc)::value;
@@ -1194,13 +1220,15 @@
         for (int ks = 0; ks < NKS; ++ks) fb[ks].load(wp, ks);
     }
     SYNC();
+    int pcur = par_off(0);
 #pragma unroll
     for (int st = 0; st < (M16 ? RB : DEPTH); ++st) {
-        if constexpr (M16) ring[st].load(As + aoff[st % RB], lane >> 4);
-        else ring[st].load(As + aoff[st % MT], st / MT, lh);
+        if constexpr (M16) ring[st].load(As + pcur + aoff[st % RB], lane >> 4);
+        else ring[st].load(As + pcur + aoff[st % MT], st / MT, lh);
     }
     int aslot = 0;
     for (int k = 0; k < ntiles; ++k) {
+        if (k > 0) pcur = par_off(k);
 #pragma unroll
         for (int i = 0; i < RB; ++i)
 #pragma unroll
@@ -1209,10 +1237,11 @@
                 for (int r = 0; r < (M16 ? 4 : 16); ++r) acc[i][j][r] = 0.f;
         const char* const wseam = k + 1 < ntiles ? wstart_of(k + 1) : nullptr;
         const int c_end = cend(k);
+        const int pnext = k + 1 < ntiles ? par_off(k + 1) : pcur;
         for (int chunk = cbeg(k); chunk < c_end; ++chunk) {
             const int naslot = aslot + 1 == NA ? 0 : aslot + 1;
-            const float* acur = As + (size_t)aslot * a_floats;
-            const float* anext = As + (size_t)naslot * a_floats;
+            const float* acur = As + (size_t)aslot * a_floats + pcur;
+            const float* anext = As + (size_t)naslot * a_floats + (chunk + 1 == c_end ? pnext : pcur);
             const char* const wlast = chunk + 1 == c_end ? (wseam ? wseam : wp + (TAPS - 1) * wstep) : nullptr;
             static_for<TAPS>([&](auto tapc) {
                 constexpr int tap = decltype(tapc)::value;
@@ -1288,7 +1317,7 @@
             part_cnt = cnt;
         }
 
-        const Tile T = tile_at(g, lin_of(k), BN, TW, TH);
+        const Tile T = tile_at<SUBPIX>(g, lin_of(k), BN, TW, TH);
         int lane_e;
         asm volatile("v_mbcnt_lo_u32_b32 %0, -1, 0\n\tv_mbcnt_hi_u32_b32 %0, -1, %0" : "=v"(lane_e));
         const int cb = T.n0c + wn * WN + 4 * (M16 ? lane_e >> 4 : lane_e >> 5);
@@ -1301,7 +1330,7 @@
         auto run_epilogue = [&](auto partc) {
             constexpr bool PARTV = decltype(partc)::value;
             if (DBG(16) || ABL(8)) keep_acc();
-            else if (!a.res) epilogue<0, PARTV>(acc, T, wm, wn, lane_e, cb, wsk, part_base, nparts);
+            else if (SUBPIX || !a.res) epilogue<0, PARTV>(acc, T, wm, wn, lane_e, cb, wsk, part_base, nparts);
             else if (a.res_mode == SGD_RS_NONE) epilogue<1, PARTV>(acc, T, wm, wn, lane_e, cb, wsk, part_base, nparts);
             else if (NT > 1) __builtin_trap();
             else if (a.res_mode == SGD_RS_AVGPOOL2) epilogue<2, PARTV>(acc, T, wm, wn, lane_e, cb, wsk, part_base, nparts);
@@ -1320,7 +1349,7 @@
         }
         if constexpr (NT > 1 || M16) {
             if (k + 1 < ntiles) {
-                const float* a0 = As + (size_t)aslot * a_floats;
+                const float* a0 = As + (size_t)aslot * a_floats + pnext;
                 if constexpr (M16) {
 #pragma unroll
                     for (int st = 0; st < RB; ++st) ring[st].load(a0 + aoff[st % RB], lane >> 4);
@@ -1376,6 +1405,7 @@
 int launch(const KArgs& ka, int vec, int taps, size_t smem, hipStream_t st) {
     const bool conv = taps == 9;
 #ifdef SGDM_IGEMM_NOPK
+    if (taps == 4) return SGD_ERR_ARG;
     if (conv) return SGD_ERR_ARG;
     if constexpr (BN == 256) {
         return taps == 2 ? launch1<BN, PREC, true, 2>(ka, smem, st) : launch1<BN, PREC, true, 1>(ka, smem, st);
@@ -1386,6 +1416,10 @@
         return vec ? launch1<BN, PREC, true, 1>(ka, smem, st) : launch1<BN, PREC, false, 1>(ka, smem, st);
     }
 #else
+    if (taps == 4) {
+        if constexpr (PREC != SGD_PREC_F32 && BN >= 128) return launch1<BN, PREC, true, 4>(ka, smem, st);
+        return SGD_ERR_ARG;
+    }
     if constexpr (BN == 256) {
         if (conv) return launch1<BN, PREC, true, 9>(ka, smem, st);
         return taps == 2 ? launch1<BN, PREC, true, 2>(ka, smem, st) : launch1<BN, PREC, true, 1>(ka, smem, st);
diff --git a/self-guided-diffusion-models_amd/csrc/igemm_host.hip b/self-guided-diffusion-models_amd/csrc/igemm_host.hip
--- a/self-guided-diffusion-models_amd/csrc/igemm_host.hip
+++ b/self-guided-diffusion-models_amd/csrc/igemm_host.hip
@@ -19,17 +19,21 @@
     if (a.mode == SGD_MODE_CONV3) {
         if (a.n <= 0 || a.hi <= 0 || a.wi <= 0 || (a.stride != 1 && a.stride != 2)) return SGD_ERR_ARG;
         if (a.stride == 2 && a.resample != SGD_RS_NONE) return SGD_ERR_ARG;
+        if (a.resample < SGD_RS_NONE || a.resample > SGD_RS_UP2_SUBPIXEL) return SGD_ERR_ARG;
+        const bool sub = a.resample == SGD_RS_UP2_SUBPIXEL;
         const bool up = a.resample == SGD_RS_UP2 || a.resample == SGD_RS_ZEROUP2;
         g.hc = a.resample == SGD_RS_AVGPOOL2 ? a.hi / 2 : (up ? a.hi * 2 : a.hi);
         g.wc = a.resample == SGD_RS_AVGPOOL2 ? a.wi / 2 : (up ? a.wi * 2 : a.wi);
         if (a.resample == SGD_RS_AVGPOOL2 && ((a.hi | a.wi) & 1)) return SGD_ERR_ARG;
-        const int ho = a.stride == 2 ? (g.hc + 1) / 2 : g.hc, wo = a.stride == 2 ? (g.wc + 1) / 2 : g.wc;
+        const int ho = a.stride == 2 ? (g.hc + 1) / 2 : g.hc * (sub ? 2 : 1), wo = a.stride == 2 ? (g.wc + 1) / 2 : g.wc * (sub ? 2 : 1);
         if (a.ho != ho || a.wo != wo) return SGD_ERR_ARG;
         if (!is_pow2(a.ho) || !is_pow2(a.wo) || a.ho < 2 || a.wo < 2) return SGD_ERR_ARG;
         if (a.res && a.res_mode == SGD_RS_UP2 && ((a.ho | a.wo) & 1)) return SGD_ERR_ARG;
+        if (sub && (a.res || a.drop_p != 0.f)) return SGD_ERR_ARG;
         if ((long)a.n * a.hi * a.wi >= (1L << 31)) return SGD_ERR_ARG;
-        int tw = a.wo < 16 ? a.wo : 16;
-        int th = BM / tw; if (th > a.ho) th = a.ho;
+        const int gho = sub ? a.hi : a.ho, gwo = sub ? a.wi : a.wo;
+        int tw = gwo < 16 ? gwo : 16;
+        int th = BM / tw; if (th > gho) th = gho;
         while (th * tw > BM) th >>= 1;
         if (a.stride == 2) { if (tw > 8) tw = 8; if (th > 8) th = 8; }
         int nb = BM / (th * tw);
@@ -38,9 +42,9 @@
         while (nb > 1 && 3 * (size_t)nb * g.hh * g.hw * LDA * 4 + (size_t)nb * g.hh * g.hw * 32 > 150 * 1024)
             nb >>= 1;
         g.tw_l2 = ilog2(tw); g.th_l2 = ilog2(th); g.nb = nb;
-        g.tiles_x = a.wo / tw; g.tiles_y = a.ho / th;
+        g.tiles_x = gwo / tw; g.tiles_y = gho / th;
         g.pix = nb * g.hh * g.hw;
-        g.mt = ((a.n + nb - 1) / nb) * g.tiles_x * g.tiles_y;
+        g.mt = ((a.n + nb - 1) / nb) * g.tiles_x * g.tiles_y * (sub ? 4 : 1);
         g.fast_a = g.pix <= FAST_PIX ? 1 : 0;
         na = 3;
     } else if (a.mode == SGD_MODE_FLAT) {
@@ -59,7 +63,8 @@
     const int ppt = bn >= 128 ? 1 : 4;
     if (((a.cout | a.y_ld) & 3) == 0 && a.orows_in == 0) {
         if (a.mode == SGD_MODE_CONV3) {
-            if (g.nb == 1 && (1 << (g.tw_l2 + g.th_l2)) == BM) g.sparts = g.tiles_x * g.tiles_y * ppt;
+            if (g.nb == 1 && (1 << (g.tw_l2 + g.th_l2)) == BM)
+                g.sparts = g.tiles_x * g.tiles_y * ppt * (a.resample == SGD_RS_UP2_SUBPIXEL ? 4 : 1);
         } else if (a.rows_per_n > 0 && a.rows_per_n % BM == 0 && a.m % a.rows_per_n == 0) {
             g.sparts = a.rows_per_n / BM * ppt;
         }
@@ -73,6 +78,7 @@
     const long rows = a.mode == SGD_MODE_CONV3 ? (long)a.n * a.ho * a.wo : (long)a.m;
     const long mt = (rows + BM - 1) / BM;
     const long t256 = mt * (a.cout_p / 256), t128 = mt * (a.cout_p / 128);
+    if (a.mode == SGD_MODE_CONV3 && a.resample == SGD_RS_UP2_SUBPIXEL) return t256 >= 256;
     if (a.mode == SGD_MODE_CONV3 && a.prec != SGD_PREC_F32) return t128 <= 256 && a.ho * a.wo <= 64 && a.c0 + a.c1 >= 512;
     if (t256 <= 256 && t128 > 256) return true;
     const long r256 = (t256 + 255) / 256, r128 = (t128 + 255) / 256;
@@ -114,6 +120,25 @@
     return g.sparts;
 }
 
+static bool subpixel_ok(const sgd_igemm_args& a0) {
+    if (a0.mode != SGD_MODE_CONV3 || (a0.resample != SGD_RS_UP2 && a0.resample != SGD_RS_UP2_SUBPIXEL)) return false;
+    if (a0.prec == SGD_PREC_F32 || (a0.tune & SGD_TUNE_NO_SUBPIXEL)) return false;
+    if (a0.stride != 1 || a0.res || a0.drop_p != 0.f) return false;
+    if ((a0.c0 & 3) || (a0.c1 & 3) || (a0.c1 > 0 && a0.c0 % KC != 0)) return false;
+    if (column_tile(a0) != 128) return false;
+    sgd_igemm_args a = a0;
+    a.resample = SGD_RS_UP2_SUBPIXEL;
+    Geo g;
+    int na;
+    if (make_geo(a, g, 128, na) != SGD_OK) return false;
+    if (a.stats && g.sparts == 0) return false;
+    const size_t smem = (size_t)na * g.pix * LDA * sizeof(float) + (size_t)g.pix * 32
+                        + (a.cout <= BIAS_LDS_MAX ? (size_t)((a.cout + 127) / 128 * 128) * sizeof(float) : 0);
+    return smem <= 160 * 1024;
+}
+
+extern "C" int sgd_igemm_subpixel_ok(const sgd_igemm_args* args) { return args && subpixel_ok(*args) ? 1 : 0; }
+
 extern "C" int sgd_igemm(const sgd_igemm_args* args, void* stream) {
     SGD_CLEAR_ERR();
     if (!args) return SGD_ERR_ARG;
@@ -129,10 +154,12 @@
     int bn = column_tile(a);
     if (a.cout_p % pick_bn(a.cout) != 0 || a.cout_p < a.cout || a.cin_p % KC != 0 || a.cin_p < cin) return SGD_ERR_ARG;
     const bool vec = (a.c0 % 4 == 0) && (a.c1 % 4 == 0);
+    const bool conv = a.mode == SGD_MODE_CONV3;
+    const bool sub = conv && a.resample == SGD_RS_UP2_SUBPIXEL;
+    if (sub && !subpixel_ok(a)) return SGD_ERR_ARG;
     if (bn == 128 && a.cout_p % 256 == 0 && vec && (!a.res || a.res_mode == SGD_RS_NONE) && want_bn256(a)) bn = 256;
     int na;
-    const bool conv = a.mode == SGD_MODE_CONV3;
-    int taps = conv ? 9 : 1;
+    int taps = conv ? (sub ? 4 : 9) : 1;
     const bool ln_nopk = !conv && a.pro == SGD_PRO_LN_ROW && a.prec != SGD_PREC_F32 && !(a.tune & SGD_TUNE_LN_PACKED);
     const bool ln_any = !conv && a.pro == SGD_PRO_LN_ROW && (ln_nopk || (a.tune & SGD_TUNE_LN_PACKED));
     if (!conv && vec && bn >= 128 && a.drop_p == 0.f && cin % (2 * KC) == 0 && (a.c1 == 0 || a.c0 % KC == 0)
@@ -174,7 +201,7 @@
         if (conv && vec && bn == 128 && a.prec != SGD_PREC_F32 && ((a.cout | a.y_ld) & 3) == 0
             && (!a.res || a.res_mode == SGD_RS_NONE) && a.resample != SGD_RS_AVGPOOL2 && a.cout_p <= BIAS_LDS_MAX && nchunks >= 3
             && rows_out * a.y_ld * 4 < (1L << 32) && (!a.stats || (long)a.n * g.sparts * 2 * a.cout * 4 < (1L << 32))
-            && smem_defer <= 160 * 1024 && (a.tune & SGD_TUNE_DEFER)) {
+            && smem_defer <= 160 * 1024 && !sub && (a.tune & SGD_TUNE_DEFER)) {
             variant = 2;
             smem_launch = smem_defer;
         }
diff --git a/self-guided-diffusion-models_amd/csrc/pack.hip b/self-guided-diffusion-models_amd/csrc/pack.hip
--- a/self-guided-diffusion-models_amd/csrc/pack.hip
+++ b/self-guided-diffusion-models_amd/csrc/pack.hip
@@ -9,6 +9,14 @@
     int e;
     frexpf(amax, &e);
     return ldexpf(1.f, 1 - e);
+}
+
+__device__ __forceinline__ void block_amax_commit(float m, uint32_t* __restrict__ amax_bits) {
+    m = wave_max(m);
+    __shared__ float wm[4];
+    if ((threadIdx.x & 63) == 0) wm[threadIdx.x >> 6] = m;
+    __syncthreads();
+    if (threadIdx.x == 0) atomicMax(amax_bits, __float_as_uint(fmaxf(fmaxf(wm[0], wm[1]), fmaxf(wm[2], wm[3]))));
 }
 
 __device__ __forceinline__ void weight_amax_body(const float* __restrict__ w, long count, uint32_t* __restrict__ amax_bits, int vec,
@@ -35,11 +43,7 @@
     } else {
         for (long i = blk * (long)blockDim.x + threadIdx.x; i < count; i += (long)nblk * blockDim.x) m = fmaxf(m, fabsf(w[i]));
     }
-    m = wave_max(m);
-    __shared__ float wm[4];
-    if ((threadIdx.x & 63) == 0) wm[threadIdx.x >> 6] = m;
-    __syncthreads();
-    if (threadIdx.x == 0) atomicMax(amax_bits, __float_as_uint(fmaxf(fmaxf(wm[0], wm[1]), fmaxf(wm[2], wm[3]))));
+    block_amax_commit(m, amax_bits);
 }
 __global__ void weight_amax_kernel(const float* __restrict__ w, long count, uint32_t* __restrict__ amax_bits, int vec) {
     weight_amax_body(w, count, amax_bits, vec, blockIdx.x, gridDim.x);
@@ -102,6 +106,86 @@
     pack_weight_body<PREC>(src, dst, cout, cin, ks, cout_p, cin_p, transpose, amax_bits, scale_inv_out, blockIdx.x, gridDim.x);
 }
 
+__device__ __forceinline__ int sp_lo(int a, int r) { return r == 0 ? 0 : a + 1; }
+__device__ __forceinline__ int sp_hi(int a, int r) { return r == 0 ? a : 2; }
+__device__ __forceinline__ float subpixel_v(const float* w9, int a, int b, int r, int s) {
+    const int y0 = sp_lo(a, r), y1 = sp_hi(a, r), x0 = sp_lo(b, s), x1 = sp_hi(b, s);
+    float v = 0.f;
+    for (int y = y0; y <= y1; ++y) {
+        float rs = w9[y * 3 + x0];
+        if (x1 != x0) rs += w9[y * 3 + x1];
+        v = y == y0 ? rs : v + rs;
+    }
+    return v;
+}
+
+__device__ __forceinline__ void weight_amax_subpixel_body(const float* __restrict__ w, int cout, int cin, uint32_t* __restrict__ amax_bits,
+                                                          int blk, int nblk) {
+    float m = 0.f;
+    const long pairs = (long)cout * cin;
+    for (long i = blk * (long)blockDim.x + threadIdx.x; i < pairs; i += (long)nblk * blockDim.x) {
+        float w9[9];
+#pragma unroll
+        for (int t = 0; t < 9; ++t) w9[t] = w[i * 9 + t];
+#pragma unroll
+        for (int p = 0; p < 16; ++p) m = fmaxf(m, fabsf(subpixel_v(w9, p >> 3, (p >> 2) & 1, (p >> 1) & 1, p & 1)));
+    }
+    block_amax_commit(m, amax_bits);
+}
+__global__ void weight_amax_subpixel_kernel(const float* __restrict__ w, int cout, int cin, uint32_t* __restrict__ amax_bits) {
+    weight_amax_subpixel_body(w, cout, cin, amax_bits, blockIdx.x, gridDim.x);
+}
+
+template <int PREC>
+__device__ __forceinline__ void pack_subpixel_body(const float* __restrict__ src, float* __restrict__ dst, int cout, int cin,
+                                                   int cout_p, int cin_p, const uint32_t* __restrict__ amax_bits,
+                                                   float* __restrict__ scale_inv_out, int blk, int grid_blocks) {
+    static_assert(PREC != SGD_PREC_F32, "the sub-pixel path is a split-mode path");
+    const float wscale = amax_bits ? pow2_scale_of(*amax_bits) : 1.f;
+    if (scale_inv_out && blk == 0 && threadIdx.x == 0) *scale_inv_out = 1.f / wscale;
+    constexpr int NKS = 2, CPL = 8;
+    const int nblk = cout_p >> 5, nch = cin_p >> 5;
+    const long total = 4L * nch * 4 * nblk * NKS * 64;
+    for (long i = blk * (long)blockDim.x + threadIdx.x; i < total; i += (long)grid_blocks * blockDim.x) {
+        const int lane = i & 63;
+        long t = i >> 6;
+        const int sub = t % NKS; t /= NKS;
+        const long unit = t;
+        const int nb = t % nblk; t /= nblk;
+        const int tap = t % 4; t /= 4;
+        const int chunk = t % nch;
+        const int par = (int)(t / nch);
+        const int co = nb * 32 + (lane & 31);
+        const int ci0 = chunk * 32 + sub * (2 * CPL) + (lane >> 5) * CPL;
+        typedef typename Split<PREC>::T T;
+        typedef T T8 __attribute__((ext_vector_type(8)));
+        T8 h, l;
+#pragma unroll
+        for (int j = 0; j < CPL; ++j) {
+            const int ci = ci0 + j;
+            float x = 0.f;
+            if (ci < cin && co < cout) {
+                float w9[9];
+#pragma unroll
+                for (int k = 0; k < 9; ++k) w9[k] = src[((long)co * cin + ci) * 9 + k];
+                x = subpixel_v(w9, par >> 1, par & 1, tap >> 1, tap & 1);
+            }
+            T hj, lj;
+            Split<PREC>::split(x * wscale, hj, lj);
+            h[j] = hj;
+            l[j] = lj;
+        }
+        T* up = reinterpret_cast<T*>(dst + unit * 1024) + sub * 1024 + lane * 8;
+        *reinterpret_cast<T8*>(up) = h;
+        *reinterpret_cast<T8*>(up + 512) = l;
+    }
+}
+template <int PREC>
+__global__ void pack_subpixel_kernel(const float* __restrict__ src, float* __restrict__ dst, int cout, int cin, int cout_p, int cin_p,
+                                     const uint32_t* __restrict__ amax_bits, float* __restrict__ scale_inv_out) {
+    pack_subpixel_body<PREC>(src, dst, cout, cin, cout_p, cin_p, amax_bits, scale_inv_out, blockIdx.x, gridDim.x);
+}
+
 __global__ void pack_zero_amax_kernel(const sgd_pack_job* __restrict__ jobs, int n) {
     const int i = blockIdx.x * blockDim.x + threadIdx.x;
     if (i < n && jobs[i].own_amax && jobs[i].amax_bits) *jobs[i].amax_bits = 0u;
@@ -110,6 +194,10 @@
                                            const int32_t* __restrict__ first) {
     const int j = block_job[blockIdx.x];
     const sgd_pack_job jb = jobs[j];
+    if (jb.transpose == SGD_PACK_SUBPIXEL) {
+        weight_amax_subpixel_body(jb.src, jb.cout, jb.cin, jb.amax_bits, blockIdx.x - first[j], first[j + 1] - first[j]);
+        return;
+    }
     const long count = (long)jb.cout * jb.cin * jb.ksize * jb.ksize;
     weight_amax_body(jb.src, count, jb.amax_bits, (((uintptr_t)jb.src) & 15) == 0 && count >= 4, blockIdx.x - first[j], first[j + 1] - first[j]);
 }
@@ -118,6 +206,15 @@
                                            const int32_t* __restrict__ first) {
     const int j = block_job[blockIdx.x];
     const sgd_pack_job jb = jobs[j];
+    if (jb.transpose == SGD_PACK_SUBPIXEL) {
+        if constexpr (PREC != SGD_PREC_F32) {
+            const int bn = (jb.cout % 128 == 0) ? 128 : 32;
+            pack_subpixel_body<PREC>(jb.src, reinterpret_cast<float*>(jb.dst), jb.cout, jb.cin, ((jb.cout + bn - 1) / bn) * bn,
+                                     ((jb.cin + KC - 1) / KC) * KC, jb.amax_bits, jb.scale_inv, blockIdx.x - first[j],
+                                     first[j + 1] - first[j]);
+        }
+        return;
+    }
     const int co = jb.transpose ? jb.cin : jb.cout, ci = jb.transpose ? jb.cout : jb.cin;
     const int bn = (co % 128 == 0) ? 128 : 32;
     const int cout_p = ((co + bn - 1) / bn) * bn, cin_p = ((ci + KC - 1) / KC) * KC;
@@ -187,16 +284,58 @@
     return pack_weight_impl(w_src, w_dst, cout, cin, ksize, prec, cin_p_out, cout_p_out, 0, stream, amax_bits, scale_inv_out);
 }
 
+static inline long subpixel_amax_blocks(int cout, int cin) {
+    const long b = ((long)cout * cin + 255) / 256;
+    return b > 256 ? 256 : b;
+}
+static inline long subpixel_pack_blocks(int cout_p, int cin_p) {
+    const long b = (16L * cout_p * cin_p / 8 + 255) / 256;
+    return b > 4096 ? 4096 : b;
+}
+
+extern "C" int64_t sgd_packed_weight_subpixel_bytes(int32_t cout, int32_t cin, int32_t prec) {
+    return 4 * sgd_packed_weight_bytes(cout, cin, 2, prec);
+}
+
+extern "C" int sgd_weight_amax_subpixel(const float* w_src, int32_t cout, int32_t cin, uint32_t* amax_bits, void* stream) {
+    SGD_CLEAR_ERR();
+    if (!w_src || !amax_bits || cout <= 0 || cin <= 0) return SGD_ERR_ARG;
+    hipLaunchKernelGGL(weight_amax_subpixel_kernel, dim3((unsigned)subpixel_amax_blocks(cout, cin)), dim3(256), 0, (hipStream_t)stream,
+                       w_src, cout, cin, amax_bits);
+    return sgd_check_launch();
+}
+
+extern "C" int sgd_pack_weight_subpixel_scaled(const float* w_src, void* w_dst, int32_t cout, int32_t cin, int32_t prec,
+                                               const uint32_t* amax_bits, float* scale_inv_out, int32_t* cin_p_out,
+                                               int32_t* cout_p_out, void* stream) {
+    SGD_CLEAR_ERR();
+    if (!w_src || !w_dst || !amax_bits || !scale_inv_out || cout <= 0 || cin <= 0) return SGD_ERR_ARG;
+    const int bn = pick_bn(cout);
+    const int cout_p = ((cout + bn - 1) / bn) * bn, cin_p = ((cin + KC - 1) / KC) * KC;
+    if (cin_p_out) *cin_p_out = cin_p;
+    if (cout_p_out) *cout_p_out = cout_p;
+    const dim3 grid((unsigned)subpixel_pack_blocks(cout_p, cin_p));
+    hipStream_t st = (hipStream_t)stream;
+    float* dst = reinterpret_cast<float*>(w_dst);
+    if (prec == SGD_PREC_F16X3) hipLaunchKernelGGL((pack_subpixel_kernel<SGD_PREC_F16X3>), grid, dim3(256), 0, st, w_src, dst, cout, cin, cout_p, cin_p, amax_bits, scale_inv_out);
+    else if (prec == SGD_PREC_BF16X3) hipLaunchKernelGGL((pack_subpixel_kernel<SGD_PREC_BF16X3>), grid, dim3(256), 0, st, w_src, dst, cout, cin, cout_p, cin_p, amax_bits, scale_inv_out);
+    else return SGD_ERR_ARG;
+    return sgd_check_launch();
+}
+
 extern "C" int sgd_pack_job_blocks(int32_t cout, int32_t cin, int32_t ksize, int32_t prec, int32_t transpose, int32_t* amax_blocks,
                                    int32_t* pack_blocks, int32_t* cin_p_out, int32_t* cout_p_out) {
     if (cout <= 0 || cin <= 0 || (ksize != 1 && ksize != 3)) return SGD_ERR_ARG;
-    const int co = transpose ? cin : cout, ci = transpose ? cout : cin;
+    if (transpose < SGD_PACK_FORWARD || transpose > SGD_PACK_SUBPIXEL) return SGD_ERR_ARG;
+    if (transpose == SGD_PACK_SUBPIXEL && (ksize != 3 || prec == SGD_PREC_F32)) return SGD_ERR_ARG;
+    const int co = transpose == SGD_PACK_DGRAD ? cin : cout, ci = transpose == SGD_PACK_DGRAD ? cout : cin;
     const int bn = pick_bn(co);
     const int cout_p = ((co + bn - 1) / bn) * bn, cin_p = ((ci + KC - 1) / KC) * KC;
     const long count = (long)cout * cin * ksize * ksize;
     long ab = (count + 4095) / 4096;
     if (ab > 256) ab = 256;
-    const long total = (long)ksize * ksize * cout_p * cin_p / (prec == SGD_PREC_F32 ? 4 : 8);
+    if (transpose == SGD_PACK_SUBPIXEL) ab = subpixel_amax_blocks(cout, cin);
+    const long total = (long)(transpose == SGD_PACK_SUBPIXEL ? 16 : ksize * ksize) * cout_p * cin_p / (prec == SGD_PREC_F32 ? 4 : 8);
     long pb = (total + 255) / 256;
     if (pb > 4096) pb = 4096;
     if (amax_blocks) *amax_blocks = (int32_t)ab;
diff --git a/self-guided-diffusion-models_amd/sgdm_amd/_lib.py b/self-guided-diffusion-models_amd/sgdm_amd/_lib.py
--- a/self-guided-diffusion-models_amd/sgdm_amd/_lib.py
+++ b/self-guided-diffusion-models_amd/sgdm_amd/_lib.py
@@ -7,15 +7,17 @@
 LIB_PATH = os.environ.get("SGDM_LIB_PATH") or os.path.join(_HERE, "lib", "libsgdm_hip.so")
 
 MODE_FLAT, MODE_CONV3 = 0, 1
-RS_NONE, RS_AVGPOOL2, RS_UP2, RS_ZEROUP2 = 0, 1, 2, 3
+RS_NONE, RS_AVGPOOL2, RS_UP2, RS_ZEROUP2, RS_UP2_SUBPIXEL = 0, 1, 2, 3, 4
 PRO_NONE, PRO_AFFINE_NC, PRO_LN_ROW = 0, 1, 2
 PREC_F32, PREC_F16X3, PREC_BF16X3 = 0, 1, 2
 PREC_BY_NAME = {"f32": PREC_F32, "f16x3": PREC_F16X3, "bf16x3": PREC_BF16X3}
-ABI_VERSION = 22
+ABI_VERSION = 23
 
 TUNE_BN128, TUNE_BN256, TUNE_FLAT2, TUNE_DEFER, TUNE_PLAIN_SCHEDULE, TUNE_LN_PACKED, TUNE_NO_SMALL = 1, 2, 4, 8, 16, 32, 64
 TUNE_WGRAD_GENERIC_NARROW, TUNE_WGRAD_NO_POOLED_PLANES, TUNE_WGRAD_F32 = 256, 512, 1024
 TUNE_WGRAD_NO_WS, TUNE_WGRAD_NO_PLANES, TUNE_WGRAD_NO_PIPE, TUNE_WGRAD_PLANES_ALWAYS = 2048, 4096, 8192, 16384
+TUNE_NO_SUBPIXEL = 32768
+PACK_FORWARD, PACK_DGRAD, PACK_SUBPIXEL = 0, 1, 2
 
 vp, i32, i64, f32 = C.c_void_p, C.c_int32, C.c_int64, C.c_float
 
@@ -43,6 +45,7 @@
     "sgd_build_id": (C.c_char_p, []),
     "sgd_igemm": (i32, [C.POINTER(IgemmArgs), vp]),
     "sgd_igemm_stats_parts": (i32, [C.POINTER(IgemmArgs)]),
+    "sgd_igemm_subpixel_ok": (i32, [C.POINTER(IgemmArgs)]),
     "sgd_igemm_work_bytes": (i64, []),
     "sgd_igemm_work_status_offset": (i64, []),
     "sgd_igemm_tail_layout": (i32, [i32, i32, i32, i32, C.POINTER(i32)]),
@@ -51,6 +54,9 @@
     "sgd_pack_weight": (i32, [vp, vp, i32, i32, i32, i32, C.POINTER(i32), C.POINTER(i32), vp]),
     "sgd_weight_amax": (i32, [vp, i64, vp, vp]),
     "sgd_pack_weight_scaled": (i32, [vp, vp, i32, i32, i32, i32, i32, vp, vp, C.POINTER(i32), C.POINTER(i32), vp]),
+    "sgd_packed_weight_subpixel_bytes": (i64, [i32, i32, i32]),
+    "sgd_weight_amax_subpixel": (i32, [vp, i32, i32, vp, vp]),
+    "sgd_pack_weight_subpixel_scaled": (i32, [vp, vp, i32, i32, i32, vp, vp, C.POINTER(i32), C.POINTER(i32), vp]),
     "sgd_pack_job_blocks": (i32, [i32, i32, i32, i32, i32, C.POINTER(i32), C.POINTER(i32), C.POINTER(i32), C.POINTER(i32)]),
     "sgd_pack_weights_batched": (i32, [vp, i32, vp, vp, i32, vp, vp, i32, i32, vp]),
     "sgd_linear_splitk": (i32, [vp, i32, vp, vp, i32, i32, i32, vp, i32, vp, i32, vp]),
diff --git a/self-guided-diffusion-models_amd/sgdm_amd/unet.py b/self-guided-diffusion-models_amd/sgdm_amd/unet.py
--- a/self-guided-diffusion-models_amd/sgdm_amd/unet.py
+++ b/self-guided-diffusion-models_amd/sgdm_amd/unet.py
@@ -139,11 +139,13 @@
 
 class _Packed:
 
-    def __init__(self, srcs, ksize, prec, pad=None):
+    def __init__(self, srcs, ksize, prec, pad=None, subpixel=False):
         self.srcs = srcs
         self.ksize = ksize
         self.prec = prec
         self.pad = pad
+        self.subpixel = subpixel
+        assert not subpixel or (ksize == 3 and pad is None and prec != L.PREC_F32)
         self.cout = sum(s.shape[0] for s in srcs)
         self.cin = srcs[0].shape[1]
         if pad is not None:
@@ -151,7 +153,8 @@
             self.cout = pad.n_rows if pad.rows is not None else self.cout
             self.cin = pad.n_cols if pad.cols is not None else self.cin
         lib = L.load()
-        nbytes = lib.sgd_packed_weight_bytes(self.cout, self.cin, ksize, prec)
+        nbytes = (lib.sgd_packed_weight_subpixel_bytes(self.cout, self.cin, prec) if subpixel
+                  else lib.sgd_packed_weight_bytes(self.cout, self.cin, ksize, prec))
         self.buf = torch.empty(nbytes // 4, dtype=torch.float32, device=srcs[0].device)
         self.cin_p = self.cout_p = 0
         self.sig = None
@@ -174,7 +177,13 @@
         if self.pad is not None:
             src = self.pad.apply(src).contiguous()
         cin_p, cout_p = C.c_int32(0), C.c_int32(0)
-        if self.scaled:
+        if self.subpixel:
+            self.amax.zero_()
+            L.check(lib.sgd_weight_amax_subpixel(_ptr(src), self.cout, self.cin, _ptr(self.amax), stream), "sgd_weight_amax_subpixel")
+            L.check(lib.sgd_pack_weight_subpixel_scaled(_ptr(src), _ptr(self.buf), self.cout, self.cin, self.prec, _ptr(self.amax),
+                                                        _ptr(self.scale_inv), C.byref(cin_p), C.byref(cout_p), stream),
+                    "sgd_pack_weight_subpixel_scaled")
+        elif self.scaled:
             self.amax.zero_()
             L.check(lib.sgd_weight_amax(_ptr(src), src.numel(), _ptr(self.amax), stream), "sgd_weight_amax")
             if len(self.srcs) == 1 and self.pad is None:
@@ -204,7 +213,7 @@
         if hasattr(pk, "srcs"):
             if len(pk.srcs) != 1 or pk.pad is not None:
                 return None
-            p, t = pk.srcs[0], 0
+            p, t = pk.srcs[0], (L.PACK_SUBPIXEL if pk.subpixel else L.PACK_FORWARD)
             cout, cin = pk.cout, pk.cin
         else:
             if len(pk.deps) != 1:
@@ -262,7 +271,7 @@
             for pk, p, cp, op in self.members:
                 pk.cin_p, pk.cout_p = cp, op
                 pk.sig = ((p.data_ptr(), p._version),)
-                if hasattr(pk, "srcs") and pk.scaled:
+                if hasattr(pk, "srcs") and pk.scaled and not pk.subpixel:
                     AMAX_OF[p.data_ptr()] = (p._version, pk.amax, weakref.ref(p))
         for pk in self.packs:
             pk.refresh(stream)
@@ -537,10 +546,25 @@
     def attention_fn(self):
         return self.lib.sgd_attention_split if self.prec == L.PREC_F16X3 else self.lib.sgd_attention
 
-    def pack(self, names, ksize, pad=None):
-        pk = _Packed([self.m.P(nm) for nm in names], ksize, self.prec, pad)
+    def pack(self, names, ksize, pad=None, subpixel=False):
+        pk = _Packed([self.m.P(nm) for nm in names], ksize, self.prec, pad, subpixel)
         self.packed.append(pk)
         return pk
+
+    def up_conv(self, tag, x0, c0, y, cout, wname, conv, *, stats=False, **kw):
+        assert conv[6] == L.RS_UP2
+        pk = self.pack([wname], 3)
+        q = L.IgemmArgs()
+        q.mode, (q.n, q.hi, q.wi, q.ho, q.wo, q.stride, q.resample) = L.MODE_CONV3, conv
+        q.c0, q.c1, q.cout, q.y_ld, q.prec = c0, kw.get("c1", 0), cout, cout, self.prec
+        q.stats = 1 if stats else 0
+        q.tune = L.TUNE_NO_SUBPIXEL if os.environ.get("SGDM_SUBPIXEL", "1") == "0" else 0
+        if kw.get("res") is not None or not self.lib.sgd_igemm_subpixel_ok(C.byref(q)):
+            return self.igemm(tag, x0, c0, y, cout, pk, conv=conv, stats=stats, **kw)
+        direct = self.igemm(tag, x0, c0, y, cout, pk, conv=conv, launch=False, **kw)
+        self.igemm(tag, x0, c0, y, cout, self.pack([wname], 3, subpixel=True), conv=conv[:6] + (L.RS_UP2_SUBPIXEL,),
+                   stats=stats, **kw)
+        return direct
 
     def padded(self, name, pad):
         src = self.m.P(name)
@@ -601,7 +625,7 @@
         self._late.append((a, pk))
         rows = conv[0] * conv[3] * conv[4] if conv is not None else m
         rows_in = conv[0] * conv[1] * conv[2] if conv is not None else m
-        taps = 9 if conv is not None else 1
+        taps = (4 if conv[6] == L.RS_UP2_SUBPIXEL else 9) if conv is not None else 1
         cin = c0 + c1
         flops = 2.0 * rows * cout * taps * cin
         nbytes = 4.0 * (rows_in * cin + rows * cout * (2 if res is not None else 1) + taps * cin * cout)
@@ -747,9 +771,8 @@
             elif kind == "up":
                 (t, c, hh, ww), = srcs
                 y = self.buf(self.n, hh * 2, ww * 2, c)
-                a = self.igemm(p + ".conv", t, c, y, c, self.pack([p + ".conv.weight"], 3),
-                               conv=(self.n, hh, ww, hh * 2, ww * 2, 1, L.RS_UP2), bias=self.m.P(p + ".conv.bias"),
-                               stats=True)
+                a = self.up_conv(p + ".conv", t, c, y, c, p + ".conv.weight",
+                                 (self.n, hh, ww, hh * 2, ww * 2, 1, L.RS_UP2), bias=self.m.P(p + ".conv.bias"), stats=True)
                 self.tape.append(dict(kind="up", p=p, x=t, y=y, c=c, hw_in=(hh, ww), a=a))
                 srcs = [(y, c, hh * 2, ww * 2)]
         return srcs[0]
@@ -767,9 +790,12 @@
                          p + ".in_layers.0")
         sums1 = self._last_sums
         h1 = self.buf(n, ho, wo, cout)
-        ac1 = self.igemm(p + ".in_layers.2", t0, c0, h1, cout, self.pack([p + ".in_layers.2.weight"], 3), x1=t1,
-                         c1=c1, conv=(n, hh, ww, ho, wo, 1, rs), pro=L.PRO_AFFINE_NC, silu=1, pa=a1, pb=b1,
-                         bias=P(p + ".in_layers.2.bias"), stats=ss)
+        kw1 = dict(x1=t1, c1=c1, pro=L.PRO_AFFINE_NC, silu=1, pa=a1, pb=b1, bias=P(p + ".in_layers.2.bias"), stats=ss)
+        if rs == L.RS_UP2:
+            ac1 = self.up_conv(p + ".in_layers.2", t0, c0, h1, cout, p + ".in_layers.2.weight", (n, hh, ww, ho, wo, 1, rs), **kw1)
+        else:
+            ac1 = self.igemm(p + ".in_layers.2", t0, c0, h1, cout, self.pack([p + ".in_layers.2.weight"], 3),
+                             conv=(n, hh, ww, ho, wo, 1, rs), **kw1)
         film_ptr = self.film.data_ptr() + 4 * self.film_off[p]
         if ss:
             a2, b2 = self.gn(p + ".out_layers.0", [(h1, cout)], ho * wo, p + ".out_layers.0", film=film_ptr,
```

Measured after the change: 2.265 images/s (median of 6 runs). 4.8% higher.
